# i8run/BigDL-1

Hardware: AMD Instinct MI355X
Metric: images/sec (whole node) ResNet-50 ImageNet-shape sync-SGD at 1/2/4/8 MI355X (higher is better)
Workload: dtype bf16; 1 GPU; model=ResNet-50, global_batch=256, per_gpu_batch=256, image_size=224, classes=1000, parallelism=dp1, optimizer=SGD(lr=0.1,m=0.9,nesterov,wd=1e-4)+L2Reg(1e-4), comm_dtype=fp32, device=cuda, syncbn=False, driver=LocalOptimizer

## Files before the change

bigdl-1_amd/bigdl/nn/fusion.py:

```python
from __future__ import annotations

from ..utils import config
from .containers import Sequential, ConcatTable
from .layers.activation import Threshold
from .layers.conv import SpatialConvolution
from .layers.normalization import BatchNormalization, SpatialBatchNormalization
from .layers.table_ops import CAddTable


def _is_relu(m):
    return isinstance(m, Threshold) and m.threshold == 0.0 and m.value == 0.0


from .layers.conv import SpatialShareConvolution

_PLAIN_CONVS = (SpatialConvolution, SpatialShareConvolution)


def _is_nchw_bn(m):
    return isinstance(m, BatchNormalization) and getattr(m, "dataFormat", "NCHW") == "NCHW"


def _relu_fusable_conv(m):
    return type(m) in _PLAIN_CONVS and m.format == "NCHW" and m._bias_folded_into is None


def _fuse_conv_relu(a, b):
    a._fused_relu = True
    b._passthrough = "mask"


def _fuse_graphs(model, convrelu):
    from .graph import Graph
    for g in model.flattened_modules():
        if not isinstance(g, Graph) or not hasattr(g, "forward_order"):
            continue
        g._plans = None
        for n in g.forward_order:
            if (convrelu and _relu_fusable_conv(n.element) and len(n.next_nodes) == 1
                    and _is_relu(n.next_nodes[0].element) and len(n.next_nodes[0].prev_nodes) == 1
                    and not n.element._fused_relu):
                _fuse_conv_relu(n.element, n.next_nodes[0].element)


def _stackable(a, b):
    from .layers.recurrent import Recurrent, LSTM
    return (type(a) is Recurrent and type(b) is Recurrent and type(a.topology) is LSTM and type(b.topology) is LSTM
            and a.topology.p == 0 and b.topology.p == 0 and not a.maskZero and not b.maskZero
            and b.batchNormParams is None and a._stack_next is None and a._stack_prev is None
            and b._stack_next is None and b._stack_prev is None)


def _link_stack(a, b):
    a._stack_next = b
    b._stack_prev = a


def _fuse_lstm_stacks(model):
    from .graph import Graph
    for s in model.flattened_modules():
        if isinstance(s, Sequential):
            mods = s.modules
            for i in range(len(mods) - 1):
                if _stackable(mods[i], mods[i + 1]):
                    _link_stack(mods[i], mods[i + 1])
        elif isinstance(s, Graph) and hasattr(s, "forward_order"):
            for n in s.forward_order:
                if len(n.next_nodes) != 1:
                    continue
                m = n.next_nodes[0]
                if len(m.prev_nodes) == 1 and _stackable(n.element, m.element):
                    _link_stack(n.element, m.element)


def fuse(model, convbn=None, bnrelu=None, convsum=None, bnbwd=None, convrelu=None):
    if not config.get_property("bigdl.fusion"):
        return model
    if getattr(model, "_fused", False):
        return model
    model._fused = True
    convrelu = config.get_property("bigdl.fusion.convrelu") if convrelu is None else convrelu
    convbn = config.get_property("bigdl.fusion.convbn") if convbn is None else convbn
    bnrelu = config.get_property("bigdl.fusion.bnrelu") if bnrelu is None else bnrelu
    convsum = config.get_property("bigdl.fusion.convsum") if convsum is None else convsum
    bnbwd = config.get_property("bigdl.fusion.bnbwd") if bnbwd is None else bnbwd
    tails, heads = [], []
    for s in model.flattened_modules():
        if not isinstance(s, Sequential):
            continue
        mods = s.modules
        for i in range(len(mods) - 1):
            a, b = mods[i], mods[i + 1]
            if convbn and isinstance(a, SpatialConvolution) and type(a) in (SpatialConvolution,) + tuple(
                    SpatialConvolution.__subclasses__()) and a.format == "NCHW" and a.withBias and _is_nchw_bn(b) \
                    and b._bias_producer is None:
                a._bias_folded_into = b
                b._bias_producer = a
            if convrelu and _relu_fusable_conv(a) and _is_relu(b) and not b._passthrough:
                _fuse_conv_relu(a, b)
            if bnrelu and _is_nchw_bn(a) and _is_relu(b):
                a._fused_relu = True
                b._passthrough = True
                c = mods[i + 2] if i + 2 < len(mods) else None
                if bnbwd and isinstance(c, SpatialConvolution) and c.format == "NCHW" and c.nGroup == 1:
                    c._bn_bwd_target = a
                    if type(c) in _PLAIN_CONVS:
                        a._pro_consumer = c
        if not convsum:
            continue
        for i in range(len(mods) - 1):
            ct, add = mods[i], mods[i + 1]
            if not (isinstance(ct, ConcatTable) and len(ct.modules) == 2 and isinstance(add, CAddTable)):
                continue
            br = ct.modules[0]
            if not (isinstance(br, Sequential) and br.modules and _is_nchw_bn(br.modules[-1])):
                continue
            bn = br.modules[-1]
            if bn._fused_relu:
                continue
            relu = mods[i + 2] if i + 2 < len(mods) and _is_relu(mods[i + 2]) else None
            ct._residual = (br, bn, ct.modules[1], relu is not None)
            sc = ct.modules[1]
            if (config.get_property("bigdl.fusion.shortcutbn") and isinstance(sc, Sequential) and len(sc.modules) >= 2
                    and _is_nchw_bn(sc.modules[-1]) and not sc.modules[-1]._fused_relu):
                sc.modules[-1]._defer_ok = True
            add._passthrough = True
            if relu is not None:
                relu._passthrough = True
                tails.append(bn)
            first = br.modules[0]
            if isinstance(first, SpatialConvolution) and len(br.modules) > 1:
                heads.append(first)
                sc = ct.modules[1]
                sc0 = sc.modules[0] if isinstance(sc, Sequential) and sc.modules else None
                if (isinstance(sc0, SpatialConvolution) and type(sc0) in _PLAIN_CONVS and sc0.format == "NCHW"
                        and sc0.kernelW == 1 and sc0.kernelH == 1 and sc0.padW == 0 and sc0.padH == 0
                        and sc0.nGroup == 1 and (sc0.strideW > 1 or sc0.strideH > 1)):
                    sc0._lazy_strided_ok = True
    if bnbwd and tails:
        for h in heads:
            h._tail_candidates = tails
    _fuse_graphs(model, convrelu)
    if config.get_property("bigdl.fusion.lstmstack"):
        _fuse_lstm_stacks(model)
    return model


def mark_input_no_grad(model):
    from .graph import Graph
    todo, seen = [model], set()
    while todo:
        m = todo.pop()
        if id(m) in seen:
            continue
        seen.add(id(m))
        if isinstance(m, Sequential):
            if m.modules:
                todo.append(m.modules[0])
        elif isinstance(m, Graph) and hasattr(m, "forward_order"):
            for n in m.forward_order:
                if not n.prev_nodes:
                    todo.append(n.element)
        elif isinstance(m, SpatialConvolution):
            m._input_grad_needed = False
    return model


def unfuse(model):
    model._fused = False
    for m in model.flattened_modules():
        if hasattr(m, "_plans"):
            m._plans = None
        if hasattr(m, "_plan"):
            m._plan = None
        if isinstance(m, SpatialConvolution):
            m._bias_folded_into = None
            m._fused_relu = False
            m._bn_bwd_target = None
            m._tail_candidates = None
            m._input_grad_needed = True
            m._lazy_strided_ok = False
        if isinstance(m, BatchNormalization):
            m._bias_producer = None
            m._fused_relu = False
            m._defer_ok = False
            m._pro_consumer = None
            m._pending_stats = None
            m._pending_grad = None
        if isinstance(m, Threshold):
            m._passthrough = False
        if isinstance(m, ConcatTable):
            m._residual = None
        if isinstance(m, CAddTable):
            m._passthrough = False
    return model
```

bigdl-1_amd/bigdl/nn/layers/conv.py:

```python
from __future__ import annotations

import math

import torch
import torch.nn.functional as F

from ... import ops
from ...ops.reference import BNGrad, BNOut, StridedGrad, as_dense
from ...utils.engine import Engine
from ...utils import config
from ..abstractnn import AbstractModule, TensorModule, AutogradModule
from ..initialization_method import RandomUniform, Zeros, VariableFormats
from ...utils import acc_float


def same_padding(in_h, in_w, stride_h, stride_w, k_h, k_w, dil_h=1, dil_w=1):
    out_h = math.ceil(in_h / stride_h)
    out_w = math.ceil(in_w / stride_w)
    ekh = (k_h - 1) * dil_h + 1
    ekw = (k_w - 1) * dil_w + 1
    ph = max((out_h - 1) * stride_h + ekh - in_h, 0)
    pw = max((out_w - 1) * stride_w + ekw - in_w, 0)
    return ph // 2, ph - ph // 2, pw // 2, pw - pw // 2, out_h, out_w


def to_device_layout(x: torch.Tensor) -> torch.Tensor:
    if x.is_cuda and x.dim() == 4:
        dt = Engine.compute_dtype()
        if (dt == torch.bfloat16 and x.dtype in (torch.float32, torch.bfloat16) and x.is_contiguous()
                and not x.is_contiguous(memory_format=torch.channels_last)):
            from ...ops import native as N
            if N.has("nchw_to_nhwc_bf16"):
                y = N.native_ops.nchw_to_nhwc_bf16(x)
                if y is not NotImplemented:
                    return y
        if x.dtype != dt and x.is_floating_point():
            x = x.to(dt)
        if not x.is_contiguous(memory_format=torch.channels_last):
            x = x.contiguous(memory_format=torch.channels_last)
    return x


class SpatialConvolution(TensorModule):
    def __init__(self, n_input_plane, n_output_plane, kernel_w, kernel_h, stride_w=1, stride_h=1, pad_w=0,
                 pad_h=0, n_group=1, propagate_back=True, wRegularizer=None, bRegularizer=None, init_weight=None,
                 init_bias=None, init_grad_weight=None, init_grad_bias=None, with_bias=True, data_format="NCHW",
                 bigdl_type="float"):
        super().__init__()
        if n_output_plane % n_group != 0 or n_input_plane % n_group != 0:
            raise ValueError(f"channels must be multiples of group: in {n_input_plane} out {n_output_plane} g {n_group}")
        if not ((pad_w >= 0 and pad_h >= 0) or (pad_w == -1 and pad_h == -1)):
            raise ValueError(f"Illegal padding configuration (padW: {pad_w}, padH: {pad_h})")
        self.nInputPlane, self.nOutputPlane = n_input_plane, n_output_plane
        self.kernelW, self.kernelH = kernel_w, kernel_h
        self.strideW, self.strideH = stride_w, stride_h
        self.padW, self.padH = pad_w, pad_h
        self.nGroup = n_group
        self.propagateBack = propagate_back
        self.withBias = with_bias
        self.format = data_format
        self.dilationW = self.dilationH = 1
        self.wRegularizer, self.bRegularizer = wRegularizer, bRegularizer
        g = n_group
        shape5 = (g, n_output_plane // g, n_input_plane // g, kernel_h, kernel_w)
        phys = (g, n_output_plane // g, kernel_h, kernel_w, n_input_plane // g)
        w = init_weight if init_weight is not None else torch.zeros(shape5)
        self.register_parameter("weight", torch.as_tensor(w, dtype=torch.float32).reshape(shape5), "gradWeight",
                                layout=(phys, (0, 1, 4, 2, 3)))
        if with_bias:
            b = init_bias if init_bias is not None else torch.zeros(n_output_plane)
            self.register_parameter("bias", torch.as_tensor(b, dtype=torch.float32).reshape(n_output_plane), "gradBias")
        else:
            self.bias = None
            self.gradBias = None
        self._has_init_w = init_weight is not None
        self._has_init_b = init_bias is not None
        stdv = 1.0 / math.sqrt(kernel_w * kernel_h * n_input_plane)
        self._init_weight_method = RandomUniform(-stdv, stdv)
        self._init_bias_method = RandomUniform(-stdv, stdv) if with_bias else Zeros()
        self.reset()

    def reset(self):
        if not self._has_init_w:
            self._init_weight_method.init(self.weight, VariableFormats.GP_OUT_IN_KW_KH)
        if self.withBias and not self._has_init_b:
            self._init_bias_method.init(self.bias, VariableFormats.ONE_D)
        self.zeroGradParameters()
        return self

    def _pads(self, x):
        H, W = x.shape[-2], x.shape[-1]
        if self.padW == -1 and self.padH == -1:
            pt, pb, pl, pr, _, _ = same_padding(H, W, self.strideH, self.strideW, self.kernelH, self.kernelW,
                                                self.dilationH, self.dilationW)
            return pt, pb, pl, pr
        return self.padH, self.padH, self.padW, self.padW

    def _w4(self, w):
        g, og, ig, kh, kw = w.shape
        krsc = w.permute(0, 1, 3, 4, 2)
        if krsc.is_contiguous():
            return krsc.reshape(g * og, kh, kw, ig).permute(0, 3, 1, 2)
        return w.reshape(g * og, ig, kh, kw)

    def _prep(self, input):
        x = input
        batched = x.dim() == 4
        if not batched:
            x = x.unsqueeze(0)
        if self.format == "NHWC":
            x = x.permute(0, 3, 1, 2)
        if (self.nInputPlane <= 3 and self.nGroup == 1 and x.is_cuda and x.dim() == 4 and x.is_contiguous()
                and not x.is_contiguous(memory_format=torch.channels_last) and (self.dilationH, self.dilationW) == (1, 1)
                and Engine.compute_dtype() == torch.bfloat16 and x.dtype in (torch.float32, torch.bfloat16)):
            from ...ops import native as N
            y = N.native_ops.nchw_to_nhwc_padded(x, self._pad_slot_()) if N.has("conv2d_forward") else NotImplemented
            x = to_device_layout(x) if y is NotImplemented else y
        else:
            x = to_device_layout(x)
        pt, pb, pl, pr = self._pads(x)
        if pt != pb or pl != pr:
            x = F.pad(x, (pl, pr, pt, pb))
            pad = (0, 0)
        else:
            pad = (pt, pl)
        return x, pad, batched, (pt, pb, pl, pr)

    _bias_folded_into = None
    _fused_relu = False
    _out_target = None

    _grad_residual = None
    _bn_bwd_target = None
    _tail_candidates = None
    _lazy_strided_ok = False

    def _pad_slot_(self):
        s = self.__dict__.get("_pad_slot")
        if s is None:
            s = self.__dict__["_pad_slot"] = [None]
        return s

    def _tail_target(self, x):
        for bn in self._tail_candidates or ():
            y = bn.output
            if (isinstance(y, torch.Tensor) and y.data_ptr() == x.data_ptr() and y.shape == x.shape and bn.train
                    and getattr(bn, "_last_relu", False)
                    and bn._last_input is not None and bn._last_input.shape == x.shape):
                return bn
        return None

    def _stats_consumer(self, x):
        bn = self._bias_folded_into
        if bn is None or not bn.train or not x.is_cuda:
            return None
        if getattr(bn, "_sync", False) and not config.get_property("bigdl.bn.shiftedStats"):
            return None
        if self.format != "NCHW" or not config.get_property("bigdl.fusion.convstats"):
            return None
        return bn

    def _pro_input(self, input):
        if not (isinstance(input, BNOut) and input.relu and self.format == "NCHW" and self.nGroup == 1
                and input.dim() == 4 and input.is_cuda and self.padW >= 0 and self.padH >= 0):
            return None
        return input.x, input.coef

    def updateOutput(self, input):
        pro = self._pro_input(input)
        if pro is not None:
            y = self._pro_forward(pro[0], pro[1])
            if y is not NotImplemented:
                return y
        if isinstance(input, BNOut):
            input = input.dense()
        x, pad, batched, _ = self._prep(input)
        w4 = self._w4(self.cw("weight"))
        b = self.bias if (self.withBias and self._bias_folded_into is None) else None
        bn = self._stats_consumer(x) if batched else None
        y = NotImplemented
        if bn is not None and ops.native_has("conv2d_forward"):
            shift = bn._stat_shift() if config.get_property("bigdl.bn.shiftedStats") else None
            sums = bn._atomic_sums("fwd", self.nOutputPlane, x.device) if shift is not None else None
            r = ops.native_ops.conv2d_forward_stats(x, w4, b, (self.strideH, self.strideW), pad,
                                                (self.dilationH, self.dilationW), self.nGroup,
                                                pad_slot=self._pad_slot_(), shift=shift, sums=sums)
            if r is not NotImplemented:
                y, part, G = r
                bn._pending_stats = (y.data_ptr(), tuple(y.shape), part, G, shift)
        if y is NotImplemented:
            tgt, self._out_target = self._out_target, None
            if tgt is not None and (not batched or self.format != "NCHW"):
                tgt = None
            y = ops.conv2d_forward(x, w4, b, (self.strideH, self.strideW), pad, (self.dilationH, self.dilationW),
                                   self.nGroup, relu=self._fused_relu, out=tgt,
                                   pad_slot=self._pad_slot_() if (self.train or self.nInputPlane <= 3) else None)
        if self.format == "NHWC":
            y = y.permute(0, 2, 3, 1)
        return y if batched else y.squeeze(0)

    def _pro_forward(self, xb, coef):
        if not ops.native_has("conv2d_forward"):
            return NotImplemented
        pt, pb, pl, pr = self._pads(xb)
        if pt != pb or pl != pr:
            return NotImplemented
        pad = (pt, pl)
        w4 = self._w4(self.cw("weight"))
        b = self.bias if (self.withBias and self._bias_folded_into is None) else None
        st, dl = (self.strideH, self.strideW), (self.dilationH, self.dilationW)
        bn = self._stats_consumer(xb)
        if bn is not None:
            shift = bn._stat_shift() if config.get_property("bigdl.bn.shiftedStats") else None
            sums = bn._atomic_sums("fwd", self.nOutputPlane, xb.device) if shift is not None else None
            r = ops.native_ops.conv2d_forward_stats(xb, w4, b, st, pad, dl, self.nGroup, shift=shift, sums=sums,
                                                    pro=coef) if sums is not None else NotImplemented
            if r is not NotImplemented:
                y, part, G = r
                bn._pending_stats = (y.data_ptr(), tuple(y.shape), part, G, shift)
                return y
            if sums is not None:
                bn._drop_sums((None, None, sums[0], sums[1]), 3)
        return ops.native_ops.conv2d_forward(xb, w4, b, st, pad, dl, self.nGroup, relu=self._fused_relu, pro=coef)

    def _backward(self, input, gradOutput, need_input, acc):
        pro = self._pro_input(input)
        if pro is not None:
            r = self._pro_backward(pro[0], pro[1], gradOutput, need_input, acc)
            if r is not NotImplemented:
                return r
        if isinstance(input, BNOut):
            input = input.dense()
        x, pad, batched, pads = self._prep(input)
        if isinstance(gradOutput, BNGrad):
            own = self.withBias and self._bias_folded_into is None and acc
            if not (batched and self.format == "NCHW" and not own and ops.native_has("conv2d_backward")
                    and ops.native_ops.bngrad_consumable(gradOutput, x, self._w4(self.cw("weight")),
                                                          (self.strideH, self.strideW), pad, self.nGroup)):
                gradOutput = gradOutput.dense()
        if isinstance(gradOutput, BNGrad):
            gy = gradOutput
        else:
            gy = gradOutput if batched else gradOutput.unsqueeze(0)
            if self.format == "NHWC":
                gy = gy.permute(0, 3, 1, 2)
            gy = to_device_layout(gy)
        w4 = self._w4(self.cw("weight"))
        gw = self._w4(self.gradWeight) if acc else None
        same_scale = self.scale_b == self.scale_w
        own_bias = self.withBias and self._bias_folded_into is None
        gb = self.gradBias if (acc and own_bias and same_scale) else None
        res = self._grad_residual if need_input else None
        self._grad_residual = None
        pt, pb, pl, pr = pads
        fuse_res = res is not None and pt == pb and pl == pr and self.format == "NCHW" and batched
        if isinstance(res, StridedGrad) and not (fuse_res and gy.is_cuda):
            res = res.dense()
        bn = self._bn_bwd_target
        bn_fuse = None
        if (bn is not None and need_input and res is None and pt == pb and pl == pr and self.format == "NCHW"
                and batched and gy.is_cuda and bn.train and bn._fused_relu
                and bn._coef is not None and bn._last_input is not None
                and config.get_property("bigdl.fusion.bnbwd")):
            C_ = bn._coef.numel() // 2
            bn_fuse = {"x": bn._last_input, "scale": bn._coef[:C_], "shift": bn._coef[C_:], "mean": bn.saveMean,
                       "sums": bn._atomic_sums("bwd", C_, bn.saveMean.device)}
        elif (fuse_res and self._tail_candidates and gy.is_cuda and config.get_property("bigdl.fusion.bnbwd")):
            bn = self._tail_target(x)
            if bn is not None:
                bn_fuse = {"x": bn._last_input, "mean": bn.saveMean, "mask": bn.output,
                           "bits": getattr(bn, "_relu_bits", None),
                           "sums": bn._atomic_sums("bwd", bn.saveMean.numel(), bn.saveMean.device)}
        lazy = (need_input and self._lazy_strided_ok and res is None and bn_fuse is None and batched
                and self.format == "NCHW" and pt == pb and pl == pr and gy.is_cuda)
        if fuse_res and not isinstance(res, StridedGrad):
            res = to_device_layout(res)
        gi = ops.conv2d_backward(gy, x, w4, (self.strideH, self.strideW), pad, (self.dilationH, self.dilationW),
                                 self.nGroup, need_input, gw, gb, self.scale_w if acc else 0.0,
                                 residual=res if fuse_res else None, bn_fuse=bn_fuse,
                                 pad_slot=self._pad_slot_(), lazy_strided=lazy)
        if isinstance(gi, StridedGrad):
            return gi
        if bn_fuse is not None and "partial" in bn_fuse and gi is not None:
            bn._pending_grad = (gi.data_ptr(), bn_fuse["partial"], bn_fuse["G"])
        if acc and own_bias and not same_scale and self.scale_b != 0:
            self.gradBias.add_(acc_float(gy).sum((0, 2, 3)), alpha=self.scale_b)
        if need_input and gi is not None:
            pt, pb, pl, pr = pads
            if pt != pb or pl != pr:
                gi = gi[:, :, pt:gi.shape[2] - pb, pl:gi.shape[3] - pr]
            if self.format == "NHWC":
                gi = gi.permute(0, 2, 3, 1)
            if not batched:
                gi = gi.squeeze(0)
            if res is not None and not fuse_res:
                gi = gi + as_dense(res)
        return gi

    def _pro_backward(self, xb, coef, gradOutput, need_input, acc):
        if not isinstance(gradOutput, torch.Tensor) or gradOutput.dim() != 4 or not gradOutput.is_cuda:
            return NotImplemented
        pt, pb, pl, pr = self._pads(xb)
        if pt != pb or pl != pr:
            return NotImplemented
        pad = (pt, pl)
        gy = to_device_layout(gradOutput)
        w4 = self._w4(self.cw("weight"))
        gw = self._w4(self.gradWeight) if acc else None
        own_bias = self.withBias and self._bias_folded_into is None
        same_scale = self.scale_b == self.scale_w
        gb = self.gradBias if (acc and own_bias and same_scale) else None
        if self._grad_residual is not None and need_input:
            return NotImplemented
        bn = self._bn_bwd_target
# ... 422 lines not shown
```

bigdl-1_amd/bigdl/nn/layers/normalization.py:

```python
from __future__ import annotations

import math

import torch
import torch.nn.functional as F

from ... import ops
from ..abstractnn import TensorModule, AutogradModule
from ..initialization_method import RandomUniform, Zeros, Ones, VariableFormats
from .conv import to_device_layout
from ...utils import acc_float, config


_SYNCBN_COMM = {}


def _syncbn_comm():
    import torch.distributed as dist
    if not config.get_property("bigdl.syncbn.ownComm") or dist.get_world_size() == 1:
        return None
    key = id(dist.distributed_c10d._get_default_group())
    g = _SYNCBN_COMM.get(key)
    if g is None:
        g = _SYNCBN_COMM[key] = dist.new_group(list(range(dist.get_world_size())))
# ... 6 lines not shown
        super().__init__()
        if n_output <= 0:
            raise ValueError("output feature map number must be greater than zero")
        self.nOutput = n_output
        self.eps = eps
        self.momentum = momentum
        self.affine = affine
        self.register_buffer("runningMean", torch.zeros(n_output))
        self.register_buffer("runningVar", torch.ones(n_output))
        self.saveMean = torch.zeros(n_output)
        self.saveStd = torch.zeros(n_output)
        if affine:
            self.register_parameter("weight", torch.zeros(n_output) if init_weight is None else
                                    torch.as_tensor(init_weight, dtype=torch.float32).reshape(n_output))
            self.register_parameter("bias", torch.zeros(n_output) if init_bias is None else
                                    torch.as_tensor(init_bias, dtype=torch.float32).reshape(n_output))
        else:
            self.weight = self.bias = self.gradWeight = self.gradBias = None
        self._has_init_w = init_weight is not None
        self._has_init_b = init_bias is not None
        self._init_weight_method = RandomUniform(0, 1)
        self._init_bias_method = Zeros()
        self._fused_relu = False
        self._defer_ok = False
        self._pro_consumer = None
        self._sync_group = None
        self._sync = False
        self._sync_force = False
        self.reset()

    def reset(self):
        if self.affine:
            if not self._has_init_w:
                self._init_weight_method.init(self.weight, VariableFormats.ONE_D)
            if not self._has_init_b:
                self._init_bias_method.init(self.bias, VariableFormats.ONE_D)
        self.runningMean.zero_()
        self.runningVar.fill_(1.0)
        self.zeroGradParameters()
        return self

    def setParallism(self, parallism: int):
        self._sync = parallism is not None and parallism > 1
        return self

    def set_sync_group(self, group=None, enabled: bool = True, force: bool = False):
        self._sync = enabled
        self._sync_group = group
        self._sync_force = force
        return self

    def _sync_active(self):
        if not self._sync:
            return False
        import torch.distributed as dist
        pg = dist.distributed_c10d.GroupMember.WORLD if dist.is_available() else None
        token = (id(pg), id(self._sync_group), self._sync_force, config.version())
        c = self.__dict__.get("_sa_cache")
        if c is not None and c[0] == token:
            return c[1]
        on = _dist_ready(self._sync_force)
        if on and config.get_property("bigdl.bn.syncOneRankLocal") and self._sync_world() == 1:
            on = False
        self.__dict__["_sa_cache"] = (token, on)
        return on

    def _sync_world(self):
        import torch.distributed as dist
        grp = self._sync_group
        return dist.get_world_size(grp) if grp is not None else dist.get_world_size()

    def _to_nchw_like(self, x):
        return x

    def _shape_in(self, input):
        return input

    _bias_producer = None
    _pending_stats = None
    _coef = None
    _last_input = None
    _pending_grad = None
    _relu_bits = None

    def _atomic_sums(self, kind, C, device):
        if device.type != "cuda" or config.get_property("bigdl.deterministic"):
            return None
        rep = int(config.get_property("bigdl.bn.statReplicas"))
        if self._sync_active() and not (rep > 0 and config.get_property("bigdl.bn.shiftedStats")):
            return None
        if rep > 0 and (self._sync_active() or not config.get_property("bigdl.bn.atomicStats")):
            rep = min(rep, 512)
            if config.get_property("bigdl.bn.foldFinalize"):
                rep = min(rep, max(4, 16384 // max(C, 1)))
            attr = "_rep_" + kind
            sets = self.__dict__.get(attr)
            if sets is None or sets[0].numel() != 2 * rep * C or sets[0].device != device:
                sets = self.__dict__[attr] = [torch.zeros(2 * rep * C, dtype=torch.float32, device=device)
                                              for _ in range(2)]
                self.__dict__["_repi_" + kind] = 0
            return sets[self.__dict__["_repi_" + kind]], rep
        if not config.get_property("bigdl.bn.atomicStats"):
            return None
        attr = "_sums_" + kind
        buf = self.__dict__.get(attr)
        if buf is None or buf.numel() != 2 * C + 1 or buf.device != device:
            buf = self.__dict__[attr] = torch.zeros(2 * C + 1, dtype=torch.float32, device=device)
        return buf

    def _drop_sums(self, pending, g_index):
        if pending is not None and (pending[g_index] == 0 or self._is_rep(pending[g_index - 1])):
            pending[g_index - 1].zero_()

    def _is_rep(self, part):
        return part is not None and any(part is b for a in ("_rep_fwd", "_rep_bwd") for b in (self.__dict__.get(a) or ()))

    def _rep_next(self, kind, part):
        sets = self.__dict__.get("_rep_" + kind)
        if not sets or not config.get_property("bigdl.bn.foldFinalize"):
            return None
        i = self.__dict__["_repi_" + kind]
        return sets[1 - i] if part is sets[i] else None

    def _rep_flip(self, kind, part):
        sets = self.__dict__.get("_rep_" + kind)
        if sets and part is sets[self.__dict__["_repi_" + kind]]:
            self.__dict__["_repi_" + kind] ^= 1

    def _advance_shift(self, mean):
        kb = self.__dict__.get("_kbuf")
        if kb is None or mean is None:
            return
        i = self.__dict__["_kidx"]
        nxt = kb[1 - i]
        if mean is not nxt:
            nxt.copy_(mean.detach().reshape(nxt.shape))
        self.__dict__["_kidx"] = 1 - i

    def _shift_next(self, shift):
        kb = self.__dict__.get("_kbuf")
        if kb is None or shift is not kb[self.__dict__["_kidx"]]:
            return None
        return kb[1 - self.__dict__["_kidx"]]

    def _stat_shift(self, device=None):
        if not (self._sync_active() or (config.get_property("bigdl.bn.foldFinalize") and self.train)):
            return self.runningMean
        kb = self.__dict__.get("_kbuf")
        rm = self.runningMean
        if kb is None or kb[0].shape != rm.shape or kb[0].device != rm.device:
            kb = self.__dict__["_kbuf"] = [rm.detach().to(torch.float32).clone(), torch.empty_like(rm, dtype=torch.float32)]
            self.__dict__["_kidx"] = 0
        return kb[self.__dict__["_kidx"]]

    def _in_bias(self):
        p = self._bias_producer
        if p is None or not getattr(p, "withBias", False):
            return None
        return p.cw("bias", torch.float32)

    def _pro_deferrable(self, x, relu, residual, coef):
        c = self._pro_consumer
        if (c is None or not relu or residual is not None or not x.is_cuda or x.dtype != torch.float32
                or c._bn_bwd_target is not self or not c.train):
            return False
        if not config.get_property("bigdl.fp32.bnPrologue") or not config.get_property("bigdl.fusion.bnbwd"):
            return False
        from ...ops import fp32x3 as F3
        return F3.pro_ok(x, coef)

    def forward_residual(self, x, residual, relu):
        self._residual_mode = True
        self._res_relu = relu
        try:
            self.output = self._forward_impl(x, residual, relu)
        finally:
            self._residual_mode = False
        return self.output

    def updateOutput(self, input):
        return self._forward_impl(input, None, self._fused_relu)

    def _forward_impl(self, input, residual, relu):
        from ...ops.reference import BNOut
        x = input
        if x.dim() == 1:
            x = x.unsqueeze(0)
        x = to_device_layout(x) if x.dim() == 4 else x
        defer = (self.__dict__.pop("_defer_next", False) and residual is None and not relu and x.is_cuda
                 and x.dtype == torch.bfloat16)
        deferred_res = isinstance(residual, BNOut)
        if deferred_res and not self.train:
            residual, deferred_res = residual.dense(), False
        if residual is not None and not deferred_res and residual.dim() == 4:
            residual = to_device_layout(residual)
        pdt = torch.float64 if x.dtype == torch.float64 else torch.float32
        g = self.cw("weight", pdt) if self.affine else None
        b = self.cw("bias", pdt) if self.affine else None
        ib = self._in_bias()
        self._last_relu = relu
        if self.train:
            if self._sync_active():
                y, mean, invstd = self._sync_forward(x, g, b, relu, residual, ib, defer=defer)
            else:
                r = NotImplemented
                C_ = x.shape[1]
                coef = self._coef
                if coef is None or coef.numel() != 2 * C_ or coef.device != x.device:
                    coef = self._coef = torch.empty(2 * C_, dtype=torch.float32, device=x.device)
                ps, self._pending_stats = self._pending_stats, None
                bits = self._tail_bits(x, relu, residual)
                self._relu_bits = None
                if ps is not None and ps[0] == x.data_ptr() and ps[1] == tuple(x.shape):
                    special = defer or deferred_res
                    pdefer = not special and self._pro_deferrable(x, relu, residual, coef)
                    r = ops.native_ops.batchnorm_forward_train_partials(
                        x, ps[2], ps[3], g, b, self.runningMean, self.runningVar, self.momentum, self.eps,
                        relu=relu, residual=residual, in_bias=ib, coef_out=coef, shift=ps[4],
                        bits_out=None if pdefer else bits,
                        rezero=self._is_rep(ps[2]), zero_next=None if special else self._rep_next("fwd", ps[2]),
                        mean_out=self._shift_next(ps[4]), apply=not (defer or pdefer))
                    if r is not NotImplemented and not special:
                        self._rep_flip("fwd", ps[2])
                if r is NotImplemented:
                    if deferred_res:
                        residual = residual.dense()
                    self._drop_sums(ps, 3)
                    r = ops.batchnorm_forward_train(x, g, b, self.runningMean, self.runningVar,
                                                    self.momentum, self.eps, relu=relu, residual=residual,
                                                    in_bias=ib, coef_out=coef, bits_out=bits)
                self._relu_bits = bits
                y, mean, invstd = r
                if y is None:
                    y = BNOut(x, coef, relu=bool(relu))
                self._advance_shift(mean)
                self._last_input = x
            self.saveMean, self.saveStd = mean, invstd
        else:
            y = ops.batchnorm_forward_infer(x, g, b, self.runningMean, self.runningVar, self.eps, relu=False,
                                            in_bias=ib)
            if residual is not None:
                y = y + residual
            if relu:
                y = torch.relu(y)
        return y.reshape(input.shape) if input.dim() == 1 else y

    def _tail_bits(self, x, relu, residual):
        if not (residual is not None and relu and x.is_cuda and x.dim() == 4 and x.shape[1] % 8 == 0
                and getattr(self, "_residual_mode", False)):
            return None
        n = x.numel() // 8
        bits = self._relu_bits
        if bits is None or bits.numel() != n or bits.device != x.device:
            bits = torch.empty(n, dtype=torch.uint8, device=x.device)
        return bits

    def _lazy_grad_ok(self, input, x):
        prod = self._bias_producer
        if prod is None or input is not x or x.dim() != 4 or not x.is_cuda or x.dtype != torch.bfloat16:
            return False
        mode = int(config.get_property("bigdl.fusion.bnprologue"))
        if mode <= 0 or (mode == 1 and x.shape[1] >= getattr(prod, "nInputPlane", 0)):
            return False
        k = (getattr(prod, "kernelH", 0), getattr(prod, "kernelW", 0), getattr(prod, "strideH", 0),
             getattr(prod, "strideW", 0), getattr(prod, "padH", -1), getattr(prod, "padW", -1),
             getattr(prod, "nGroup", 0))
        return (k == (1, 1, 1, 1, 0, 0, 1) and prod.format == "NCHW" and x.shape[1] % 32 == 0
                and x.is_contiguous(memory_format=torch.channels_last))

    def _sync_allreduce(self, t):
        import torch.distributed as dist
        ws = self.__dict__.get("_sync_ws")
        if ws is None or ws[0] is not self._sync_group:
            grp = self._sync_group if self._sync_group is not None else _syncbn_comm()
            ws = self.__dict__["_sync_ws"] = (self._sync_group, dist.get_world_size(grp), grp)
        if ws[1] > 1:
            dist.all_reduce(t, group=ws[2])

    def _sync_ops(self, x):
        from ...ops import native_ops as NO, reference as R
        if (x.is_cuda and x.dtype == torch.bfloat16 and x.dim() == 4 and x.shape[1] % 8 == 0
                and ops.native_has("batchnorm_forward_train")):
            return NO
        return R

    def _sync_forward(self, x, g, b, relu=False, residual=None, in_bias=None, defer=False):
        from ...ops import reference as R
        impl = self._sync_ops(x)
        C_ = x.shape[1]
        coef = self._coef
        if coef is None or coef.numel() != 2 * C_ or coef.device != x.device:
            coef = self._coef = torch.empty(2 * C_, dtype=torch.float32, device=x.device)
        ps, self._pending_stats = self._pending_stats, None
        bits = self._tail_bits(x, relu, residual) if impl is not R else None
        self._relu_bits = None
        r = NotImplemented
        for m in ((impl, R) if impl is not R else (R,)):
            if m is not R and ps is not None and ps[0] == x.data_ptr() and ps[1] == tuple(x.shape) \
                    and ps[4] is not None:
                shift = ps[4]
                sums = m.bn_local_sums(x, shift, ps[2], ps[3], rezero=self._is_rep(ps[2]))
                ps = None
            else:
                shift = self._stat_shift()
                sums = m.bn_local_sums(x, shift)
            if sums is NotImplemented:
                continue
            self._sync_allreduce(sums)
            kb = self.__dict__.get("_kbuf")
            nxt = kb[1 - self.__dict__["_kidx"]] if (kb is not None and shift is kb[self.__dict__["_kidx"]]) else None
            kw = dict(mean_out=nxt) if (m is not R and nxt is not None) else {}
            r = m.bn_forward_from_sums(x, sums, 0, shift, g, b, self.runningMean, self.runningVar, self.momentum,
                                       self.eps, relu=relu, residual=residual, in_bias=in_bias, coef_out=coef,
                                       bits_out=bits if (m is not R and not defer) else None, apply=not defer, **kw)
            if r is NotImplemented and m is not R:
                m = R
                r = R.bn_forward_from_sums(x, sums, 0, shift, g, b, self.runningMean, self.runningVar,
                                           self.momentum, self.eps, relu=relu, residual=residual, in_bias=in_bias,
                                           coef_out=coef, apply=not defer)
            if r is not NotImplemented:
                if r[0] is None:
                    r = (R.BNOut(x, coef, relu=bool(relu)),) + tuple(r[1:])
                self._relu_bits = bits if m is not R else None
                self._sync_path = "native" if m is not R else "reference"
                self._last_input = x
                if nxt is not None:
                    if r[1] is not nxt:
                        nxt.copy_(r[1])
                    self.__dict__["_kidx"] ^= 1
                break
        self._drop_sums(ps, 3)
        return r

    def _bwd(self, input, gradOutput, need_input, acc, want_gres=False):
        x = input if input.dim() > 1 else input.unsqueeze(0)
        gy = gradOutput if gradOutput.dim() > 1 else gradOutput.unsqueeze(0)
        if x.dim() == 4:
            x = to_device_layout(x)
            gy = to_device_layout(gy)
        relu = getattr(self, "_last_relu", self._fused_relu)
        y = self.output if relu else None
        from ...ops.reference import BNOut
        if isinstance(y, BNOut):
            y = None if (self._pending_grad is not None and self._pending_grad[0] == gy.data_ptr()) else y.dense()
        if y is not None and y.dim() == 1:
            y = y.unsqueeze(0)
        g = self.cw("weight", torch.float64 if x.dtype == torch.float64 else torch.float32) if self.affine else None
        prod = self._bias_producer
        cb = prod.gradBias if (acc and prod is not None and getattr(prod, "withBias", False)) else None
        cbs = prod.scale_b if prod is not None else 0.0
        gres = None
        if self._sync_active() and self.train:
            pg = self._pending_grad
            pre_masked = pg is not None and pg[0] == gy.data_ptr()
            gi, cb_done = self._sync_backward(x, gy, g, y, need_input, acc, relu, cb, cbs)
            if cb is not None and gi is not None and not cb_done:
                cb.add_(acc_float(gi).sum([d for d in range(gi.dim()) if d != 1]), alpha=cbs)
            if want_gres:
                gres = gy * (y > 0).to(gy.dtype) if (relu and not pre_masked) else gy
        else:
            same = self.scale_w == self.scale_b
            pg, self._pending_grad = self._pending_grad, None
            if pg is not None and pg[0] == gy.data_ptr() and relu and same:
                gi = ops.native_ops.batchnorm_backward_partials(
                    gy, x, g, self.saveMean, self.saveStd, pg[1], pg[2], need_input=need_input,
                    gg_acc=self.gradWeight if (acc and self.affine) else None,
                    gb_acc=self.gradBias if (acc and self.affine) else None,
                    scale=self.scale_w if acc else 0.0, cbias_acc=cb, cbias_scale=cbs,
                    lazy=self._lazy_grad_ok(input, x), rezero=self._is_rep(pg[1]),
                    zero_next=self._rep_next("bwd", pg[1]))
                if gi is not NotImplemented:
                    self._rep_flip("bwd", pg[1])
                    if gi is not None and input.dim() == 1:
                        gi = gi.reshape(input.shape)
                    return (gi, gy) if want_gres else gi
            self._drop_sums(pg, 2)
            gi, gres = ops.batchnorm_backward(gy, x, g, self.saveMean, self.saveStd, y=y, relu=relu,
                                              need_input=need_input,
                                              gg_acc=self.gradWeight if (acc and self.affine) else None,
                                              gb_acc=self.gradBias if (acc and self.affine and same) else None,
                                              scale=self.scale_w if acc else 0.0, cbias_acc=cb, cbias_scale=cbs,
                                              want_gres=want_gres)
            if acc and self.affine and not same and self.scale_b != 0:
                gf = acc_float(gy) * ((y > 0).float() if relu else 1.0)
                dims = [d for d in range(gf.dim()) if d != 1]
                self.gradBias.add_(gf.sum(dims), alpha=self.scale_b)
        if gi is not None and input.dim() == 1:
            gi = gi.reshape(input.shape)
        if want_gres:
            return gi, gres
        return gi

    def backward_residual(self, input, gradOutput):
        gi, gres = self._bwd(input, gradOutput, True, True, want_gres=True)
        self.gradInput = gi
        for h in self._grad_ready_hooks:
            h(self)
        return gi, gres

    def _sync_backward(self, x, gy, g, y, need_input, acc, relu=None, cb=None, cbs=0.0):
        from ...ops import reference as R
        relu = self._fused_relu if relu is None else relu
        impl = self._sync_ops(x)
        pg, self._pending_grad = self._pending_grad, None
        C = x.shape[1]
        rows = x.numel() // C
        for m in ((impl, R) if impl is not R else (R,)):
            rl = relu
            both = NotImplemented
            if m is not R and pg is not None and pg[0] == gy.data_ptr() and relu:
                both = m.bn_bwd_partials_sums(pg[1], pg[2], C, x.device, rows=rows, rezero=self._is_rep(pg[1]))
                if both is not NotImplemented:
                    rl = False
                    pg = None
            if both is NotImplemented:
                both = m.bn_bwd_local_sums(gy, x, self.saveMean, y=y, relu=rl)
            if both is NotImplemented:
                continue
            loc, glob = both[:2 * C], both[2 * C:]
            self._sync_allreduce(glob)
            kw = dict(need_input=need_input, gg_acc=self.gradWeight if (acc and self.affine) else None,
                      gb_acc=self.gradBias if (acc and self.affine) else None, scale=self.scale_w if acc else 0.0,
                      cbias_acc=cb, cbias_scale=cbs)
            gi = m.bn_backward_from_sums(gy, x, g, self.saveMean, self.saveStd, loc, glob, 0, y=y, relu=rl, **kw)
            if gi is NotImplemented and m is not R:
                m = R
                gi = R.bn_backward_from_sums(gy, x, g, self.saveMean, self.saveStd, loc, glob, 0, y=y, relu=rl, **kw)
            if gi is NotImplemented:
                raise RuntimeError("SyncBN backward: no implementation accepted the all-reduced sums")
            if acc and self.affine and self.scale_b != self.scale_w:
                self.gradBias.add_(loc[:C], alpha=self.scale_b - self.scale_w)
            self._sync_bwd_path = "native" if m is not R else "reference"
            self._drop_sums(pg, 2)
            return gi, cb is not None
        raise RuntimeError("SyncBN backward: no implementation accepted the input")

    def updateGradInput(self, input, gradOutput):
        gi = self._bwd(input, gradOutput, True, True)
        self._gi_done = True
        return gi

    def accGradParameters(self, input, gradOutput):
        if not getattr(self, "_gi_done", False):
            self._bwd(input, gradOutput, False, True)
        self._gi_done = False

    def set_running_mean(self, v):
        self.runningMean.copy_(torch.as_tensor(v))
        return self

    def set_running_std(self, v):
        self.runningVar.copy_(torch.as_tensor(v))
        return self

    def __repr__(self):
        return f"{type(self).__name__}[{self.get_name()}]({self.nOutput}, {self.eps}, {self.momentum}, {self.affine})"


class SpatialBatchNormalization(BatchNormalization):
    def __init__(self, n_output, eps=1e-5, momentum=0.1, affine=True, init_weight=None, init_bias=None,
                 init_grad_weight=None, init_grad_bias=None, data_format="NCHW", bigdl_type="float"):
        super().__init__(n_output, eps, momentum, affine, init_weight, init_bias, init_grad_weight, init_grad_bias)
        self.dataFormat = data_format

    def updateOutput(self, input):
        if self.dataFormat == "NHWC":
            y = super().updateOutput(input.permute(0, 3, 1, 2))
# ... 188 lines not shown
```

bigdl-1_amd/bigdl/nn/layers/pooling.py:

```python
from __future__ import annotations

import math

import torch
import torch.nn.functional as F

from ... import ops
from ..abstractnn import TensorModule, AutogradModule
from .conv import to_device_layout, same_padding
from ...utils import acc_float


def _pool_pad(x, kh, kw, dh, dw, ph, pw):
    if ph == -1 and pw == -1:
        pt, pb, pl, pr, _, _ = same_padding(x.shape[-2], x.shape[-1], dh, dw, kh, kw)
        return pt, pb, pl, pr
    return ph, ph, pw, pw


class SpatialMaxPooling(TensorModule):
    def __init__(self, kw, kh, dw=None, dh=None, pad_w=0, pad_h=0, to_ceil=False, format="NCHW",
                 bigdl_type="float"):
        super().__init__()
        self.kW, self.kH = kw, kh
        self.dW = dw if dw is not None else kw
        self.dH = dh if dh is not None else kh
        self.padW, self.padH = pad_w, pad_h
        self.ceilMode = to_ceil
        self.format = format

    def ceil(self):
        self.ceilMode = True
        return self

    def floor(self):
        self.ceilMode = False
        return self

    def _prep(self, input):
        x = input
        if self.format == "NHWC":
            x = x.permute(0, 3, 1, 2) if x.dim() == 4 else x.permute(2, 0, 1)
        batched = x.dim() == 4
        if not batched:
            x = x.unsqueeze(0)
        x = to_device_layout(x)
        pt, pb, pl, pr = _pool_pad(x, self.kH, self.kW, self.dH, self.dW, self.padH, self.padW)
        if pt != pb or pl != pr:
            x = F.pad(x, (pl, pr, pt, pb), value=float("-inf"))
            pad = (0, 0)
        else:
            pad = (pt, pl)
        return x, pad, batched, (pt, pb, pl, pr)

    def _post(self, y, batched):
        if not batched:
            y = y.squeeze(0)
        if self.format == "NHWC":
            y = y.permute(0, 2, 3, 1) if y.dim() == 4 else y.permute(1, 2, 0)
        return y

    def _int8_forward(self, input):
        from ...ops import native_ops as NO
        if not (input.is_cuda and input.dim() == 4 and self.format == "NCHW" and not self.train):
            return None
        pt, pb, pl, pr = _pool_pad(input, self.kH, self.kW, self.dH, self.dW, self.padH, self.padW)
        if pt != pb or pl != pr:
            return None
        H, W = input.shape[2], input.shape[3]
        P = NO._pool_out(H, self.kH, self.dH, pt, self.ceilMode)
        Q = NO._pool_out(W, self.kW, self.dW, pl, self.ceilMode)
        y = NO.maxpool_i8(input, self.kH, self.kW, self.dH, self.dW, pt, pl, P, Q)
        return None if y is NotImplemented else y

    def updateOutput(self, input):
        if input.dtype == torch.int8 and getattr(input, "_qscale", None) is not None:
            y = self._int8_forward(input)
            if y is not None:
                return y
            from ..quantized.layers import dequant
            input = dequant(input)
        x, pad, batched, _ = self._prep(input)
        y, idx = ops.maxpool2d_forward(x, (self.kH, self.kW), (self.dH, self.dW), pad, self.ceilMode,
                                       need_indices=bool(self.train))
        self._indices = idx
        return self._post(y, batched)

    def updateGradInput(self, input, gradOutput):
        x, pad, batched, pads = self._prep(input)
        gy = gradOutput
        if self.format == "NHWC":
            gy = gy.permute(0, 3, 1, 2) if gy.dim() == 4 else gy.permute(2, 0, 1)
        if not batched:
            gy = gy.unsqueeze(0)
        gy = to_device_layout(gy)
        if self._indices is None:
            _, self._indices = ops.maxpool2d_forward(x, (self.kH, self.kW), (self.dH, self.dW), pad, self.ceilMode)
        gi = ops.maxpool2d_backward(gy, x, self._indices, (self.kH, self.kW), (self.dH, self.dW), pad, self.ceilMode)
        pt, pb, pl, pr = pads
        if pt != pb or pl != pr:
            gi = gi[:, :, pt:gi.shape[2] - pb, pl:gi.shape[3] - pr]
        return self._post(gi, batched)

    def __repr__(self):
        return f"SpatialMaxPooling[{self.get_name()}]({self.kW}, {self.kH}, {self.dW}, {self.dH}, {self.padW}, {self.padH})"


class SpatialAveragePooling(TensorModule):
    def __init__(self, kw, kh, dw=1, dh=1, pad_w=0, pad_h=0, global_pooling=False, ceil_mode=False,
                 count_include_pad=True, divide=True, format="NCHW", bigdl_type="float"):
        super().__init__()
        self.kW, self.kH, self.dW, self.dH = kw, kh, dw, dh
        self.padW, self.padH = pad_w, pad_h
        self.globalPooling = global_pooling
        self.ceilMode = ceil_mode
        self.countIncludePad = count_include_pad
        self.divide = divide
        self.format = format

    def ceil(self):
        self.ceilMode = True
        return self

    def floor(self):
        self.ceilMode = False
        return self

    def _geom(self, x):
        if self.globalPooling:
            return (x.shape[-2], x.shape[-1]), (1, 1), (0, 0)
        return (self.kH, self.kW), (self.dH, self.dW), None

    def _prep(self, input):
        x = input
        if self.format == "NHWC":
            x = x.permute(0, 3, 1, 2) if x.dim() == 4 else x.permute(2, 0, 1)
        batched = x.dim() == 4
        if not batched:
            x = x.unsqueeze(0)
        x = to_device_layout(x)
        k, s, p = self._geom(x)
        pads = (0, 0, 0, 0)
        if p is None:
            pt, pb, pl, pr = _pool_pad(x, k[0], k[1], s[0], s[1], self.padH, self.padW)
            pads = (pt, pb, pl, pr)
            if pt != pb or pl != pr:
                x = F.pad(x, (pl, pr, pt, pb))
                p = (0, 0)
            else:
                p = (pt, pl)
        divisor = None if self.divide else 1
        return x, k, s, p, batched, pads, divisor

    def _post(self, y, batched):
        if not batched:
            y = y.squeeze(0)
        if self.format == "NHWC":
            y = y.permute(0, 2, 3, 1) if y.dim() == 4 else y.permute(1, 2, 0)
        return y

    def updateOutput(self, input):
        x, k, s, p, batched, _, divisor = self._prep(input)
        y = ops.avgpool2d_forward(x, k, s, p, self.ceilMode, self.countIncludePad, divisor)
        return self._post(y, batched)

    def updateGradInput(self, input, gradOutput):
        x, k, s, p, batched, pads, divisor = self._prep(input)
        gy = gradOutput
        if self.format == "NHWC":
            gy = gy.permute(0, 3, 1, 2) if gy.dim() == 4 else gy.permute(2, 0, 1)
        if not batched:
# ... 228 lines not shown
```

bigdl-1_amd/bigdl/ops/csrc/batchnorm.hip:

```cpp
#include "common.h"

struct BnGeom {
  int C, CG, RPI, tpr;
};

__device__ __forceinline__ BnGeom bn_geom(int C) {
  BnGeom g;
  g.C = C;
  g.CG = C >> 3;
  int cg_eff = g.CG < 256 ? g.CG : 256;
  g.RPI = 256 / cg_eff;
  g.tpr = cg_eff;
  return g;
}

__global__ void __launch_bounds__(256) k_bn_stats(const bf16_t* __restrict__ x, long long M, int C,
                                                  long long rows_per_block, float* __restrict__ partial, int G,
                                                  const float* __restrict__ kshift = nullptr) {
  extern __shared__ __attribute__((aligned(16))) float smem[];
  BnGeom g = bn_geom(C);
  const int t = threadIdx.x;
  const int cg_local = t % g.tpr;
  const int r_off = t / g.tpr;
  const long long r0 = (long long)blockIdx.x * rows_per_block;
// ... 300 lines not shown
      b += partial[(size_t)(G + g) * C + c];
    }
  }
  red[0][ty][tx] = a;
  red[1][ty][tx] = b;
  __syncthreads();
  if (ty == 0 && c < C) {
    out[(size_t)blockIdx.y * C + c] = red[0][0][tx] + red[0][1][tx] + red[0][2][tx] + red[0][3][tx];
    out[(size_t)(S + blockIdx.y) * C + c] = red[1][0][tx] + red[1][1][tx] + red[1][2][tx] + red[1][3][tx];
  }
}

static constexpr int kFoldRows = 128;

BIGDL_EXPORT long long bigdl_bn_fold_scratch(int G, int C) {
  if (G <= 512) return 0;
  const int S = (G + kFoldRows - 1) / kFoldRows;
  return 4LL * S * C;
}

static bool maybe_fold(const float* partial, int& G, int C, float* scratch, hipStream_t s) {
  if (G <= 512 || !scratch) return false;
  const int S = (G + kFoldRows - 1) / kFoldRows;
  hipLaunchKernelGGL(k_bn_fold_partials, dim3((C + 63) / 64, S), dim3(256), 0, s, partial, G, C, kFoldRows, S,
                     (double*)scratch);
  G = S;
  return true;
}

BIGDL_EXPORT int bigdl_bn_fwd_train_partials2(const void* x, const void* res, const float* rcoef, void* y, long long M,
                                              int C, const float* gamma, const float* beta, const float* in_bias,
                                              float* run_mean, float* run_var, float momentum, float eps,
                                              float* save_mean, float* save_invstd, const float* partial, int G,
                                              const float* kshift, float* coef, int relu, float* scratch, void* bits,
                                              int rezero, hipStream_t s);

BIGDL_EXPORT int bigdl_bn_fwd_train_partials(const void* x, const void* res, void* y, long long M, int C,
                                             const float* gamma, const float* beta, const float* in_bias,
                                             float* run_mean, float* run_var, float momentum, float eps,
                                             float* save_mean, float* save_invstd, const float* partial, int G,
                                             const float* kshift, float* coef, int relu, float* scratch, void* bits,
                                             int rezero, hipStream_t s) {
  if (!y) return (int)hipErrorInvalidValue;
  return bigdl_bn_fwd_train_partials2(x, res, nullptr, y, M, C, gamma, beta, in_bias, run_mean, run_var, momentum, eps,
                                      save_mean, save_invstd, partial, G, kshift, coef, relu, scratch, bits, rezero, s);
}

BIGDL_EXPORT int bigdl_bn_fwd_train_partials2(const void* x, const void* res, const float* rcoef, void* y, long long M,
                                              int C, const float* gamma, const float* beta, const float* in_bias,
                                              float* run_mean, float* run_var, float momentum, float eps,
                                              float* save_mean, float* save_invstd, const float* partial, int G,
                                              const float* kshift, float* coef, int relu, float* scratch, void* bits,
                                              int rezero, hipStream_t s) {
  if (rcoef && !res) return (int)hipErrorInvalidValue;
  if (C % 8 || M <= 0 || G <= 0 || (bits && !relu) || (rezero && G > 512)) return (int)hipErrorInvalidValue;
  if (!rezero && maybe_fold(partial, G, C, scratch, s))
    hipLaunchKernelGGL(k_bn_finalize<double>, dim3((C + 31) / 32), dim3(32 * kFinRG), 0, s, (const bf16_t*)nullptr, kshift,
                       (const double*)scratch, G, M, C, gamma, beta, in_bias, run_mean, run_var, momentum, eps, save_mean,
                       save_invstd, coef, coef + C);
  else
    hipLaunchKernelGGL(k_bn_finalize<float>, dim3((C + 31) / 32), dim3(32 * kFinRG), 0, s, (const bf16_t*)nullptr, kshift,
                       partial, G, M, C, gamma, beta, in_bias, run_mean, run_var, momentum, eps, save_mean, save_invstd,
                       coef, coef + C, nullptr, rezero ? const_cast<float*>(partial) : nullptr);
  if (y) launch_apply(x, res, y, M, C, coef, relu, bits, s, rcoef);
  BIGDL_CHECK_LAUNCH();
}

BIGDL_EXPORT int bigdl_bn_fwd_infer(const void* x, void* y, long long M, int C, const float* gamma, const float* beta,
                                    const float* run_mean, const float* run_var, const float* in_bias, float eps,
                                    float* coef, int relu, hipStream_t s) {
  if (C % 8 || M <= 0) return (int)hipErrorInvalidValue;
  hipLaunchKernelGGL(k_bn_infer_coef, dim3((C + 255) / 256), dim3(256), 0, s, C, gamma, beta, run_mean, run_var,
                     in_bias, eps, coef, coef + C);
  int grid = apply_grid(M, C);
  if (relu)
    hipLaunchKernelGGL((k_bn_apply<false, true>), dim3(grid), dim3(256), 0, s, (const bf16_t*)x, nullptr, (bf16_t*)y,
                       M, C, coef, coef + C);
  else
    hipLaunchKernelGGL((k_bn_apply<false, false>), dim3(grid), dim3(256), 0, s, (const bf16_t*)x, nullptr,
                       (bf16_t*)y, M, C, coef, coef + C);
  BIGDL_CHECK_LAUNCH();
}

template <bool RELU>
__global__ void __launch_bounds__(256) k_bn_bwd_reduce(const bf16_t* __restrict__ gy, const bf16_t* __restrict__ x,
                                                       const bf16_t* __restrict__ y, long long M, int C,
                                                       long long rows_per_block, const float* __restrict__ mean,
                                                       float* __restrict__ partial, int G) {
  extern __shared__ __attribute__((aligned(16))) float smem[];
  BnGeom g = bn_geom(C);
  const int t = threadIdx.x;
  const int cg_local = t % g.tpr;
  const int r_off = t / g.tpr;
  const long long r0 = (long long)blockIdx.x * rows_per_block;
  long long r1 = r0 + rows_per_block;
  if (r1 > M) r1 = M;
  float* s_a = smem;
  float* s_b = smem + g.RPI * C;
  for (int cg = cg_local; cg < g.CG; cg += g.tpr) {
    if (r_off >= g.RPI) break;
    float mu[8], a[8], b[8];
#pragma unroll
    for (int k = 0; k < 8; ++k) { mu[k] = mean[cg * 8 + k]; a[k] = 0.f; b[k] = 0.f; }
    for (long long r = r0 + r_off; r < r1; r += g.RPI) {
      size_t off = (size_t)r * C + (size_t)cg * 8;
      float gv[8], xv[8];
      load8_nt(gy + off, gv);
      load8_nt(x + off, xv);
      if (RELU) {
        float yv[8];
        load8_nt(y + off, yv);
#pragma unroll
        for (int k = 0; k < 8; ++k) gv[k] = yv[k] > 0.f ? gv[k] : 0.f;
      }
#pragma unroll
      for (int k = 0; k < 8; ++k) {
        a[k] += gv[k];
        b[k] = fmaf(gv[k], xv[k] - mu[k], b[k]);
      }
    }
#pragma unroll
    for (int k = 0; k < 8; ++k) {
      s_a[r_off * C + cg * 8 + k] = a[k];
      s_b[r_off * C + cg * 8 + k] = b[k];
    }
  }
  __syncthreads();
  for (int c = t; c < C; c += 256) {
    float a = 0.f, b = 0.f;
    for (int i = 0; i < g.RPI; ++i) {
      a += s_a[i * C + c];
      b += s_b[i * C + c];
    }
    partial[(size_t)blockIdx.x * C + c] = a;
    partial[(size_t)(G + blockIdx.x) * C + c] = b;
  }
}

template <typename T>
__global__ void __launch_bounds__(32 * kFinRG) k_bn_bwd_finalize(const T* __restrict__ partial, int G, long long M,
                                                          int C, const float* __restrict__ gamma,
                                                          const float* __restrict__ mean,
                                                          const float* __restrict__ invstd,
                                                          float* __restrict__ ggamma, float* __restrict__ gbeta,
                                                          float gscale, float* __restrict__ cbias, float cbscale,
                                                          float* __restrict__ coef, const float* __restrict__ dM = nullptr,
                                                          float* rezero = nullptr) {
  __shared__ double lds[kFinRG][2][33];
  double ad, bd;
  reduce_partials(partial, G, C, blockIdx.x * 32, lds, ad, bd, rezero);
  const int c = blockIdx.x * 32 + (threadIdx.x & 31);
  if ((threadIdx.x >> 5) != 0 || c >= C) return;
  const float a = (float)ad, b = (float)bd;
  float is = invstd[c];
  float dbeta = a;
  float dgamma = b * is;
  if (ggamma) ggamma[c] += gscale * dgamma;
  if (gbeta) gbeta[c] += gscale * dbeta;
  float gm = gamma ? gamma[c] : 1.f;
  float A = gm * is;
  const float Mf = dM ? *dM : (float)M;
  float B = -gm * is * is * dgamma / Mf;
  float Cc = -gm * is * dbeta / Mf - B * mean[c];
  coef[c] = A;
  coef[C + c] = B;
  coef[2 * C + c] = Cc;
  if (cbias) cbias[c] += cbscale * (A * dbeta + B * Mf * mean[c] + Mf * Cc);
}

template <bool RELU, bool GRES, int kApplyUnroll>
__device__ __forceinline__ void bn_bwd_apply_rows(const bf16_t* __restrict__ gy, const bf16_t* __restrict__ x,
                                                  const bf16_t* __restrict__ y, bf16_t* __restrict__ gx,
                                                  bf16_t* __restrict__ gres, long long M, int C, const float* coef) {
  BnGeom g = bn_geom(C);
  const int t = threadIdx.x;
  const int cg_local = t % g.tpr;
  const int r_off = t / g.tpr;
  if (r_off >= g.RPI) return;
  const long long rstride = (long long)gridDim.x * g.RPI;
  for (int cg = cg_local; cg < g.CG; cg += g.tpr) {
    float A[8], B[8], Cc[8];
#pragma unroll
    for (int k = 0; k < 8; ++k) {
      A[k] = coef[cg * 8 + k];
      B[k] = coef[C + cg * 8 + k];
      Cc[k] = coef[2 * C + cg * 8 + k];
    }
    long long r = (long long)blockIdx.x * g.RPI + r_off;
    for (; r < M; r += kApplyUnroll * rstride) {
      bigdl_u32x4 gq[kApplyUnroll], xq[kApplyUnroll], yq[kApplyUnroll];
#pragma unroll
      for (int u = 0; u < kApplyUnroll; ++u) {
        const long long ru = r + u * rstride;
        const size_t off = (size_t)(ru < M ? ru : r) * C + (size_t)cg * 8;
        gq[u] = __builtin_nontemporal_load(reinterpret_cast<const bigdl_u32x4*>(gy + off));
        xq[u] = __builtin_nontemporal_load(reinterpret_cast<const bigdl_u32x4*>(x + off));
        if (RELU) yq[u] = __builtin_nontemporal_load(reinterpret_cast<const bigdl_u32x4*>(y + off));
      }
#pragma unroll
      for (int u = 0; u < kApplyUnroll; ++u) {
        const long long ru = r + u * rstride;
        if (ru >= M) break;
        const size_t off = (size_t)ru * C + (size_t)cg * 8;
        float gv[8], xv[8];
        unpack8(make_uint4(gq[u][0], gq[u][1], gq[u][2], gq[u][3]), gv);
        unpack8(make_uint4(xq[u][0], xq[u][1], xq[u][2], xq[u][3]), xv);
        if (RELU) {
          float yv[8];
          unpack8(make_uint4(yq[u][0], yq[u][1], yq[u][2], yq[u][3]), yv);
#pragma unroll
          for (int k = 0; k < 8; ++k) gv[k] = yv[k] > 0.f ? gv[k] : 0.f;
        }
        if (GRES) store8(gres + off, gv);
#pragma unroll
        for (int k = 0; k < 8; ++k) xv[k] = fmaf(A[k], gv[k], fmaf(B[k], xv[k], Cc[k]));
        store8(gx + off, xv);
      }
    }
  }
}

template <bool RELU, bool GRES, int kApplyUnroll = 4>
__global__ void __launch_bounds__(256) k_bn_bwd_apply(const bf16_t* __restrict__ gy, const bf16_t* __restrict__ x,
                                                      const bf16_t* __restrict__ y, bf16_t* __restrict__ gx,
                                                      bf16_t* __restrict__ gres, long long M, int C,
                                                      const float* __restrict__ coef) {
  bn_bwd_apply_rows<RELU, GRES, kApplyUnroll>(gy, x, y, gx, gres, M, C, coef);
}

BIGDL_EXPORT int bigdl_bn_bwd(const void* gy, const void* x, const void* y, void* gx, void* gres, long long M, int C,
                              const float* gamma, const float* mean, const float* invstd, float* ggamma,
                              float* gbeta, float gscale, float* cbias, float cbscale, float* ws, float* coef,
                              int relu, hipStream_t s) {
  if (C % 8 || M <= 0) return (int)hipErrorInvalidValue;
  int G = bigdl_bn_num_partials(M, C);
  long long rpb = (M + G - 1) / G;
  size_t sm = stats_smem(C);
  if (relu)
    hipLaunchKernelGGL(k_bn_bwd_reduce<true>, dim3(G), dim3(256), sm, s, (const bf16_t*)gy, (const bf16_t*)x,
                       (const bf16_t*)y, M, C, rpb, mean, ws, G);
  else
    hipLaunchKernelGGL(k_bn_bwd_reduce<false>, dim3(G), dim3(256), sm, s, (const bf16_t*)gy, (const bf16_t*)x,
                       (const bf16_t*)y, M, C, rpb, mean, ws, G);
  hipLaunchKernelGGL(k_bn_bwd_finalize<float>, dim3((C + 31) / 32), dim3(32 * kFinRG), 0, s, (const float*)ws, G, M, C, gamma,
                     mean, invstd, ggamma, gbeta, gscale, cbias, cbscale, coef);
  if (gx) {
    int grid = apply_grid(M, C);
    const bf16_t *g_ = (const bf16_t*)gy, *x_ = (const bf16_t*)x, *y_ = (const bf16_t*)y;
    bf16_t *gx_ = (bf16_t*)gx, *gr_ = (bf16_t*)gres;
    if (relu && gres) hipLaunchKernelGGL((k_bn_bwd_apply<true, true>), dim3(grid), dim3(256), 0, s, g_, x_, y_, gx_, gr_, M, C, coef);
    else if (relu) hipLaunchKernelGGL((apply_unroll1() ? k_bn_bwd_apply<true, false, 1> : k_bn_bwd_apply<true, false, 4>), dim3(grid), dim3(256), 0, s, g_, x_, y_, gx_, gr_, M, C, coef);
    else if (gres) hipLaunchKernelGGL((k_bn_bwd_apply<false, true>), dim3(grid), dim3(256), 0, s, g_, x_, y_, gx_, gr_, M, C, coef);
    else hipLaunchKernelGGL((apply_unroll1() ? k_bn_bwd_apply<false, false, 1> : k_bn_bwd_apply<false, false, 4>), dim3(grid), dim3(256), 0, s, g_, x_, y_, gx_, gr_, M, C, coef);
  }
  BIGDL_CHECK_LAUNCH();
}

BIGDL_EXPORT int bigdl_bn_bwd_partials(const void* gm, const void* x, void* gx, long long M, int C, const float* gamma,
                                       const float* mean, const float* invstd, float* ggamma, float* gbeta,
                                       float gscale, float* cbias, float cbscale, const float* partial, int G,
                                       float* coef, float* scratch, int rezero, hipStream_t s) {
  if (C % 8 || M <= 0 || G <= 0 || (rezero && G > 512)) return (int)hipErrorInvalidValue;
  if (!rezero && maybe_fold(partial, G, C, scratch, s))
    hipLaunchKernelGGL(k_bn_bwd_finalize<double>, dim3((C + 31) / 32), dim3(32 * kFinRG), 0, s, (const double*)scratch, G, M,
                       C, gamma, mean, invstd, ggamma, gbeta, gscale, cbias, cbscale, coef);
  else
    hipLaunchKernelGGL(k_bn_bwd_finalize<float>, dim3((C + 31) / 32), dim3(32 * kFinRG), 0, s, partial, G, M, C, gamma, mean,
                       invstd, ggamma, gbeta, gscale, cbias, cbscale, coef, nullptr,
                       rezero ? const_cast<float*>(partial) : nullptr);
  if (gx) {
    int grid = apply_grid(M, C);
    hipLaunchKernelGGL((apply_unroll1() ? k_bn_bwd_apply<false, false, 1> : k_bn_bwd_apply<false, false, 4>), dim3(grid), dim3(256), 0, s, (const bf16_t*)gm,
                       (const bf16_t*)x, (const bf16_t*)nullptr, (bf16_t*)gx, (bf16_t*)nullptr, M, C, coef);
  }
  BIGDL_CHECK_LAUNCH();
}

BIGDL_EXPORT int bigdl_bn_bwd_apply_coef(const void* gm, const void* x, void* gx, long long M, int C,
                                         const float* coef, hipStream_t s) {
  if (C % 8 || M <= 0 || !gm || !x || !gx || !coef) return (int)hipErrorInvalidValue;
  hipLaunchKernelGGL((apply_unroll1() ? k_bn_bwd_apply<false, false, 1> : k_bn_bwd_apply<false, false, 4>),
                     dim3(apply_grid(M, C)), dim3(256), 0, s, (const bf16_t*)gm, (const bf16_t*)x,
                     (const bf16_t*)nullptr, (bf16_t*)gx, (bf16_t*)nullptr, M, C, coef);
  BIGDL_CHECK_LAUNCH();
}

struct BnFwdFin {
  float* sums;
  const float* kshift;
  const float* gamma;
  const float* beta;
  const float* in_bias;
  float* run_mean;
  float* run_var;
  float* save_mean;
  float* save_invstd;
  float* coef;
  double M;
  float momentum, eps;
  const float* dM;
  unsigned* ticket;
  int keep;
  int early;
  const float* rep;
  int R;
  float* zero_next;
};

__device__ __forceinline__ void fin_fwd_sums(const BnFwdFin& f, int C, int c, double& s, double& q) {
  if (f.rep) {
    s = 0.0;
    q = 0.0;
    for (int r = 0; r < f.R; ++r) {
      s += (double)f.rep[(size_t)r * C + c];
      q += (double)f.rep[((size_t)f.R + r) * C + c];
    }
  } else {
    s = (double)f.sums[c];
    q = (double)f.sums[C + c];
  }
}

__device__ __forceinline__ void block_zero(float* p, long long n) {
  for (long long i = (long long)threadIdx.x * 4; i < n; i += (long long)blockDim.x * 4)
    *reinterpret_cast<float4*>(p + i) = make_float4(0.f, 0.f, 0.f, 0.f);
}

__device__ __forceinline__ void fin_fwd_coef(const BnFwdFin& f, int C, int c, float& mean, float& var, float& invstd,
                                             float& sc, float& sh) {
  const double Mg = f.dM ? (double)*f.dM : f.M;
  double s1, s2;
  fin_fwd_sums(f, C, c, s1, s2);
  const double dm = s1 / Mg;
  var = (float)fmax(s2 / Mg - dm * dm, 0.0);
  mean = (f.kshift ? f.kshift[c] : 0.f) + (float)dm;
  invstd = rsqrtf(var + f.eps);
  sc = (f.gamma ? f.gamma[c] : 1.f) * invstd;
  sh = (f.beta ? f.beta[c] : 0.f) - mean * sc;
}

__device__ __forceinline__ bool last_arriver(unsigned* cnt) {
  __shared__ int last;
  __syncthreads();
  if (threadIdx.x == 0) last = atomicAdd(cnt, 1u) == gridDim.x - 1 ? 1 : 0;
  __syncthreads();
  return last != 0;
}

constexpr int kTicketLeaves = 16;
__device__ __forceinline__ bool last_arriver_tree(unsigned* cnt) {
  __shared__ int last;
  __syncthreads();
  if (threadIdx.x == 0) {
    const unsigned nb = gridDim.x, leaf = blockIdx.x % kTicketLeaves;
    const unsigned in_leaf = (nb - leaf + kTicketLeaves - 1) / kTicketLeaves;
    const unsigned leaves = nb < (unsigned)kTicketLeaves ? nb : (unsigned)kTicketLeaves;
    int l = 0;
    if (atomicAdd(&cnt[1 + leaf], 1u) == in_leaf - 1) {
      atomicExch(&cnt[1 + leaf], 0u);
      if (atomicAdd(&cnt[0], 1u) == leaves - 1) {
        atomicExch(&cnt[0], 0u);
        l = 1;
      }
    }
    last = l;
  }
// ... 283 lines not shown
                                         const float* kshift, float* coef, int relu, void* bits, unsigned* ticket,
                                         hipStream_t s) {
  if (C % 8 || M <= 0 || count < 0 || (bits && !relu) || (rcoef && !res) || (!y && (res || bits)))
    return (int)hipErrorInvalidValue;
  if (ticket && C <= 8192 && y && !rcoef) {
    BnFwdFin f{const_cast<float*>(sums), kshift, gamma, beta, in_bias, run_mean, run_var, save_mean, save_invstd, coef,
               (double)count, momentum, eps, count == 0 ? sums + 2 * C : nullptr, ticket, 1,
               (kshift != run_mean && kshift != save_mean) ? 1 : 0};
    const int grid = apply_grid(M, C);
    const bf16_t* xr = (const bf16_t*)x;
    const bf16_t* rr = (const bf16_t*)res;
    bf16_t* yr = (bf16_t*)y;
    uint8_t* br = (uint8_t*)bits;
    if (relu && bits && res) hipLaunchKernelGGL((k_bn_apply_fin<true, true, true>), dim3(grid), dim3(256), 8 * C, s, xr, rr, yr, M, C, f, br);
    else if (relu && bits) hipLaunchKernelGGL((k_bn_apply_fin<false, true, true>), dim3(grid), dim3(256), 8 * C, s, xr, rr, yr, M, C, f, br);
    else if (res && relu) hipLaunchKernelGGL((k_bn_apply_fin<true, true, false>), dim3(grid), dim3(256), 8 * C, s, xr, rr, yr, M, C, f, br);
    else if (res) hipLaunchKernelGGL((k_bn_apply_fin<true, false, false>), dim3(grid), dim3(256), 8 * C, s, xr, rr, yr, M, C, f, br);
    else if (relu) hipLaunchKernelGGL((k_bn_apply_fin<false, true, false>), dim3(grid), dim3(256), 8 * C, s, xr, rr, yr, M, C, f, br);
    else hipLaunchKernelGGL((k_bn_apply_fin<false, false, false>), dim3(grid), dim3(256), 8 * C, s, xr, rr, yr, M, C, f, br);
    BIGDL_CHECK_LAUNCH();
  }
  hipLaunchKernelGGL(k_bn_finalize<float>, dim3((C + 31) / 32), dim3(32 * kFinRG), 0, s, (const bf16_t*)nullptr, kshift, sums,
                     1, count, C, gamma, beta, in_bias, run_mean, run_var, momentum, eps, save_mean, save_invstd, coef,
                     coef + C, count == 0 ? sums + 2 * C : nullptr);
  if (y) launch_apply(x, res, y, M, C, coef, relu, bits, s, rcoef);
  BIGDL_CHECK_LAUNCH();
}

BIGDL_EXPORT int bigdl_bn_bwd_sums(const void* gy, const void* x, const void* y, long long M, int C, const float* mean,
                                   float* ws, float* scratch, float* out, int relu, float cnt, hipStream_t s) {
  if (C % 8 || M <= 0) return (int)hipErrorInvalidValue;
  int G = bigdl_bn_num_partials(M, C);
  long long rpb = (M + G - 1) / G;
  size_t sm = stats_smem(C);
  if (relu)
    hipLaunchKernelGGL(k_bn_bwd_reduce<true>, dim3(G), dim3(256), sm, s, (const bf16_t*)gy, (const bf16_t*)x,
                       (const bf16_t*)y, M, C, rpb, mean, ws, G);
  else
    hipLaunchKernelGGL(k_bn_bwd_reduce<false>, dim3(G), dim3(256), sm, s, (const bf16_t*)gy, (const bf16_t*)x,
                       (const bf16_t*)y, M, C, rpb, mean, ws, G);
  sum_rows(ws, G, C, scratch, out, s, out + 2 * C, cnt);
  BIGDL_CHECK_LAUNCH();
}

__global__ void __launch_bounds__(256) k_bn_cbias_sync(const float* __restrict__ local_sums,
                                                       const float* __restrict__ coef, const float* __restrict__ mean,
                                                       long long M, int C, float* __restrict__ cbias, float cbscale) {
  const int c = blockIdx.x * 256 + threadIdx.x;
  if (c >= C) return;
  const float A = coef[c], B = coef[C + c], Cc = coef[2 * C + c];
  cbias[c] += cbscale * (A * local_sums[c] + (float)M * (B * mean[c] + Cc));
}

BIGDL_EXPORT int bigdl_bn_bwd_apply_sums(const void* gy, const void* x, const void* y, void* gx, long long M,
                                         long long count, int C, const float* gamma, const float* mean,
                                         const float* invstd, float* ggamma, float* gbeta, float gscale,
                                         const float* local_sums, const float* global_sums, float* coef,
                                         float* coef_scratch, int relu, float* cbias, float cbscale, unsigned* ticket,
                                         hipStream_t s) {
  if (C % 8 || M <= 0 || count < 0) return (int)hipErrorInvalidValue;
  const float* dM = count == 0 ? global_sums + 2 * C : nullptr;
  if (ticket && !relu && C <= 4096) {
    BnBwdFin f{const_cast<float*>(global_sums), gamma, mean, invstd, ggamma, gbeta, gscale, cbias, cbscale, nullptr,
               (float)count, local_sums, (float)M, dM, ticket, 1, 1};
    const int grid = gx ? apply_grid(M, C) : 1;
    hipLaunchKernelGGL(k_bn_bwd_apply_fin, dim3(grid), dim3(256), gx ? 12 * C : 0, s, (const bf16_t*)gy,
                       (const bf16_t*)x, (bf16_t*)gx, M, C, f);
    BIGDL_CHECK_LAUNCH();
  }
  if (ggamma || gbeta)
    hipLaunchKernelGGL(k_bn_bwd_finalize<float>, dim3((C + 31) / 32), dim3(32 * kFinRG), 0, s, local_sums, 1, count, C, gamma,
                       mean, invstd, ggamma, gbeta, gscale, (float*)nullptr, 0.f, coef_scratch, dM);
  hipLaunchKernelGGL(k_bn_bwd_finalize<float>, dim3((C + 31) / 32), dim3(32 * kFinRG), 0, s, global_sums, 1, count, C, gamma,
                     mean, invstd, (float*)nullptr, (float*)nullptr, 0.f, (float*)nullptr, 0.f, coef, dM);
  if (cbias)
    hipLaunchKernelGGL(k_bn_cbias_sync, dim3((C + 255) / 256), dim3(256), 0, s, local_sums, coef, mean, M, C, cbias,
                       cbscale);
  if (gx) {
    int grid = apply_grid(M, C);
    const bf16_t *g_ = (const bf16_t*)gy, *x_ = (const bf16_t*)x, *y_ = (const bf16_t*)y;
    bf16_t* gx_ = (bf16_t*)gx;
    if (relu)
      hipLaunchKernelGGL((apply_unroll1() ? k_bn_bwd_apply<true, false, 1> : k_bn_bwd_apply<true, false, 4>), dim3(grid), dim3(256), 0, s, g_, x_, y_, gx_, (bf16_t*)nullptr, M, C,
                         coef);
    else
      hipLaunchKernelGGL((apply_unroll1() ? k_bn_bwd_apply<false, false, 1> : k_bn_bwd_apply<false, false, 4>), dim3(grid), dim3(256), 0, s, g_, x_, y_, gx_, (bf16_t*)nullptr, M,
                         C, coef);
  }
  BIGDL_CHECK_LAUNCH();
}

__device__ __forceinline__ void ld8f(const float* __restrict__ p, float (&v)[8]) {
  const float4 a = *reinterpret_cast<const float4*>(p), b = *reinterpret_cast<const float4*>(p + 4);
  v[0] = a.x; v[1] = a.y; v[2] = a.z; v[3] = a.w; v[4] = b.x; v[5] = b.y; v[6] = b.z; v[7] = b.w;
}
__device__ __forceinline__ void st8f(float* __restrict__ p, const float (&v)[8]) {
  *reinterpret_cast<float4*>(p) = make_float4(v[0], v[1], v[2], v[3]);
  *reinterpret_cast<float4*>(p + 4) = make_float4(v[4], v[5], v[6], v[7]);
}

template <int MODE, bool RELU>
__global__ void __launch_bounds__(256) k_bn32_reduce(const float* __restrict__ x, const float* __restrict__ gy,
                                                     const float* __restrict__ y, long long M, int C,
                                                     long long rows_per_block, const float* __restrict__ ref,
                                                     float* __restrict__ partial, int G,
                                                     const uint8_t* __restrict__ mbits = nullptr) {
  extern __shared__ __attribute__((aligned(16))) float smem[];
  BnGeom g = bn_geom(C);
  const int t = threadIdx.x;
  const int cg_local = t % g.tpr;
  const int r_off = t / g.tpr;
  const long long r0 = (long long)blockIdx.x * rows_per_block;
  long long r1 = r0 + rows_per_block;
  if (r1 > M) r1 = M;
  float* s_a = smem;
  float* s_b = smem + g.RPI * C;
  for (int cg = cg_local; cg < g.CG; cg += g.tpr) {
    float K[8], a[8], b[8];
#pragma unroll
    for (int k = 0; k < 8; ++k) { K[k] = ref[cg * 8 + k]; a[k] = 0.f; b[k] = 0.f; }
    if (r_off < g.RPI) {
      for (long long r = r0 + r_off; r < r1; r += g.RPI) {
        const size_t off = (size_t)r * C + (size_t)cg * 8;
        float xv[8];
        ld8f(x + off, xv);
        if (MODE == 0) {
#pragma unroll
          for (int k = 0; k < 8; ++k) {
            const float d = xv[k] - K[k];
            a[k] += d;
            b[k] = fmaf(d, d, b[k]);
          }
        } else {
          float gv[8];
          ld8f(gy + off, gv);
          if (RELU) {
            if (mbits) {
              const unsigned mb = mbits[(size_t)r * (C >> 3) + cg];
#pragma unroll
              for (int k = 0; k < 8; ++k) gv[k] = (mb >> k) & 1u ? gv[k] : 0.f;
            } else {
              float yv[8];
              ld8f(y + off, yv);
#pragma unroll
              for (int k = 0; k < 8; ++k) gv[k] = yv[k] > 0.f ? gv[k] : 0.f;
            }
          }
#pragma unroll
          for (int k = 0; k < 8; ++k) {
            a[k] += gv[k];
            b[k] = fmaf(gv[k], xv[k] - K[k], b[k]);
          }
        }
      }
#pragma unroll
      for (int k = 0; k < 8; ++k) {
        s_a[r_off * C + cg * 8 + k] = a[k];
        s_b[r_off * C + cg * 8 + k] = b[k];
      }
    }
  }
  __syncthreads();
  for (int c = t; c < C; c += 256) {
    float a = 0.f, b = 0.f;
    for (int i = 0; i < g.RPI; ++i) {
      a += s_a[i * C + c];
      b += s_b[i * C + c];
    }
    partial[(size_t)blockIdx.x * C + c] = a;
    partial[(size_t)(G + blockIdx.x) * C + c] = b;
// ... 230 lines not shown
```

bigdl-1_amd/bigdl/ops/csrc/pooling.hip:

```cpp
#include "common.h"

struct PoolGeom {
  int N, H, W, C, P, Q, kh, kw, sh, sw, ph, pw;
};

__device__ __forceinline__ void pld8(const bf16_t* p, float* o) { load8(p, o); }
__device__ __forceinline__ void pld8(const float* p, float* o) {
  const float4 a = *reinterpret_cast<const float4*>(p), b = *reinterpret_cast<const float4*>(p + 4);
  o[0] = a.x; o[1] = a.y; o[2] = a.z; o[3] = a.w; o[4] = b.x; o[5] = b.y; o[6] = b.z; o[7] = b.w;
}
__device__ __forceinline__ void pst8(bf16_t* p, const float* o) { store8(p, o); }
__device__ __forceinline__ void pst8(float* p, const float* o) {
  *reinterpret_cast<float4*>(p) = make_float4(o[0], o[1], o[2], o[3]);
  *reinterpret_cast<float4*>(p + 4) = make_float4(o[4], o[5], o[6], o[7]);
}

template <typename IT, typename T = bf16_t>
__global__ void __launch_bounds__(256) k_maxpool_fwd(const T* __restrict__ x, T* __restrict__ y,
                                                     int8_t* __restrict__ idx, PoolGeom g) {
  const int CG = g.C >> 3;
  const IT total = (IT)g.N * g.P * g.Q * CG;
  for (IT t = blockIdx.x * (IT)blockDim.x + threadIdx.x; t < total; t += (IT)gridDim.x * blockDim.x) {
    const int cg = (int)(t % CG);
    IT pix = t / CG;
    const int q = (int)(pix % g.Q);
    pix /= g.Q;
    const int p = (int)(pix % g.P);
    const int n = (int)(pix / g.P);
    float best[8];
    int arg[8];
#pragma unroll
    for (int e = 0; e < 8; ++e) { best[e] = -INFINITY; arg[e] = 0; }
    const int h0 = p * g.sh - g.ph, w0 = q * g.sw - g.pw;
    for (int i = 0; i < g.kh; ++i) {
      const int h = h0 + i;
      if ((unsigned)h >= (unsigned)g.H) continue;
      for (int j = 0; j < g.kw; ++j) {
        const int w = w0 + j;
        if ((unsigned)w >= (unsigned)g.W) continue;
        float v[8];
        pld8(x + (((size_t)n * g.H + h) * g.W + w) * g.C + cg * 8, v);
#pragma unroll
        for (int e = 0; e < 8; ++e) {
          if (v[e] > best[e] || v[e] != v[e]) {
            best[e] = v[e];
            arg[e] = i * g.kw + j;
          }
        }
      }
    }
    const size_t o = (((size_t)n * g.P + p) * g.Q + q) * g.C + cg * 8;
    pst8(y + o, best);
    if (!idx) continue;
    uint32_t lo = 0, hi = 0;
#pragma unroll
    for (int e = 0; e < 4; ++e) lo |= (uint32_t)(arg[e] & 0xFF) << (8 * e);
#pragma unroll
    for (int e = 0; e < 4; ++e) hi |= (uint32_t)(arg[4 + e] & 0xFF) << (8 * e);
    *reinterpret_cast<uint2*>(idx + o) = make_uint2(lo, hi);
  }
}

template <typename IT, typename T = bf16_t>
__global__ void __launch_bounds__(256) k_maxpool_fwd_k3s2(const T* __restrict__ x, T* __restrict__ y,
                                                          int8_t* __restrict__ idx, PoolGeom g) {
  const int CG = g.C >> 3;
  const IT total = (IT)g.N * g.P * g.Q * CG;
  for (IT t = blockIdx.x * (IT)blockDim.x + threadIdx.x; t < total; t += (IT)gridDim.x * blockDim.x) {
    const int cg = (int)(t % CG);
    IT pix = t / CG;
    const int q = (int)(pix % g.Q);
    pix /= g.Q;
    const int p = (int)(pix % g.P);
    const int n = (int)(pix / g.P);
    const int h0 = p * 2 - g.ph, w0 = q * 2 - g.pw;
    const int hc = min(max(h0 + 1, 0), g.H - 1), wc = min(max(w0 + 1, 0), g.W - 1);
    float v[9][8];
    bool ok[9];
#pragma unroll
    for (int i = 0; i < 3; ++i)
#pragma unroll
      for (int j = 0; j < 3; ++j) {
        const int h = h0 + i, w = w0 + j;
        ok[3 * i + j] = (unsigned)h < (unsigned)g.H && (unsigned)w < (unsigned)g.W;
        const int hh = ok[3 * i + j] ? h : hc, ww = ok[3 * i + j] ? w : wc;
        pld8(x + (((size_t)n * g.H + hh) * g.W + ww) * g.C + cg * 8, v[3 * i + j]);
      }
    float best[8];
    int arg[8];
#pragma unroll
    for (int e = 0; e < 8; ++e) { best[e] = -INFINITY; arg[e] = 0; }
#pragma unroll
    for (int k = 0; k < 9; ++k)
#pragma unroll
      for (int e = 0; e < 8; ++e)
        if (ok[k] && (v[k][e] > best[e] || v[k][e] != v[k][e])) {
          best[e] = v[k][e];
          arg[e] = k;
        }
    const size_t o = (((size_t)n * g.P + p) * g.Q + q) * g.C + cg * 8;
    pst8(y + o, best);
    if (!idx) continue;
    uint32_t lo = 0, hi = 0;
#pragma unroll
    for (int e = 0; e < 4; ++e) lo |= (uint32_t)(arg[e] & 0xFF) << (8 * e);
#pragma unroll
    for (int e = 0; e < 4; ++e) hi |= (uint32_t)(arg[4 + e] & 0xFF) << (8 * e);
    *reinterpret_cast<uint2*>(idx + o) = make_uint2(lo, hi);
  }
}

template <typename IT, typename T = bf16_t>
__global__ void __launch_bounds__(256) k_maxpool_bwd(const T* __restrict__ gy, const int8_t* __restrict__ idx,
                                                     T* __restrict__ gx, PoolGeom g) {
  const int CG = g.C >> 3;
  const IT total = (IT)g.N * g.H * g.W * CG;
  for (IT t = blockIdx.x * (IT)blockDim.x + threadIdx.x; t < total; t += (IT)gridDim.x * blockDim.x) {
    const int cg = (int)(t % CG);
    IT pix = t / CG;
    const int w = (int)(pix % g.W);
    pix /= g.W;
    const int h = (int)(pix % g.H);
    const int n = (int)(pix / g.H);
    float acc[8];
#pragma unroll
    for (int e = 0; e < 8; ++e) acc[e] = 0.f;
    const int hp = h + g.ph, wp = w + g.pw;
    int p_lo = hp - g.kh + 1;
    p_lo = p_lo <= 0 ? 0 : (p_lo + g.sh - 1) / g.sh;
    int p_hi = hp / g.sh;
    if (p_hi > g.P - 1) p_hi = g.P - 1;
    int q_lo = wp - g.kw + 1;
    q_lo = q_lo <= 0 ? 0 : (q_lo + g.sw - 1) / g.sw;
    int q_hi = wp / g.sw;
    if (q_hi > g.Q - 1) q_hi = g.Q - 1;
    for (int p = p_lo; p <= p_hi; ++p) {
      const int i = hp - p * g.sh;
      for (int q = q_lo; q <= q_hi; ++q) {
        const int j = wp - q * g.sw;
        const int8_t me = (int8_t)(i * g.kw + j);
        const size_t o = (((size_t)n * g.P + p) * g.Q + q) * g.C + cg * 8;
        const uint2 a = *reinterpret_cast<const uint2*>(idx + o);
        float gv[8];
        pld8(gy + o, gv);
        const uint32_t aw[2] = {a.x, a.y};
#pragma unroll
        for (int e = 0; e < 8; ++e) {
          const int8_t ae = (int8_t)((aw[e >> 2] >> (8 * (e & 3))) & 0xFF);
          if (ae == me) acc[e] += gv[e];
        }
      }
    }
    pst8(gx + (((size_t)n * g.H + h) * g.W + w) * g.C + cg * 8, acc);
  }
}

template <typename IT, typename T = bf16_t>
__global__ void __launch_bounds__(256) k_maxpool_bwd_k3s2(const T* __restrict__ gy, const int8_t* __restrict__ idx,
                                                          T* __restrict__ gx, PoolGeom g) {
  const int CG = g.C >> 3;
  const IT total = (IT)g.N * g.H * g.W * CG;
  for (IT t = blockIdx.x * (IT)blockDim.x + threadIdx.x; t < total; t += (IT)gridDim.x * blockDim.x) {
    const int cg = (int)(t % CG);
    IT pix = t / CG;
    const int w = (int)(pix % g.W);
    pix /= g.W;
    const int h = (int)(pix % g.H);
    const int n = (int)(pix / g.H);
    const int hp = h + g.ph, wp = w + g.pw;
    const int pa = hp / 2 - 1, qa = wp / 2 - 1;
    uint2 a[4];
    float gv[4][8];
    bool ok[4];
    int8_t me[4];
#pragma unroll
    for (int u = 0; u < 2; ++u)
#pragma unroll
      for (int v2 = 0; v2 < 2; ++v2) {
        const int p = pa + u, q = qa + v2, k = 2 * u + v2;
        const int i = hp - 2 * p, j = wp - 2 * q;
        ok[k] = p >= 0 && p < g.P && q >= 0 && q < g.Q && i <= 2 && j <= 2;
        me[k] = (int8_t)(i * 3 + j);
        const int pp = ok[k] ? p : 0, qq = ok[k] ? q : 0;
        const size_t o = (((size_t)n * g.P + pp) * g.Q + qq) * g.C + cg * 8;
// ... 97 lines not shown
#pragma unroll
          for (int e = 0; e < 8; ++e) best[j][e] = (rm[e] > best[j][e] || rm[e] != rm[e]) ? rm[e] : best[j][e];
        }
      }
    }
#pragma unroll
    for (int j = 0; j < MP_ROWS; ++j)
      if (j < np) store8(y + (((size_t)n * g.P + p0 + j) * g.Q + q) * g.C + cg * 8, best[j]);
  }
}

template <typename T = bf16_t>
__global__ void __launch_bounds__(256) k_maxpool_bwd_c1(const T* __restrict__ gy, const int8_t* __restrict__ idx,
                                                        T* __restrict__ gx, PoolGeom g, long long total) {
  for (long long t = blockIdx.x * (long long)blockDim.x + threadIdx.x; t < total; t += (long long)gridDim.x * blockDim.x) {
    const int c = (int)(t % g.C);
    long long pix = t / g.C;
    const int w = (int)(pix % g.W);
    pix /= g.W;
    const int h = (int)(pix % g.H);
    const int n = (int)(pix / g.H);
    const int hp = h + g.ph, wp = w + g.pw;
    int p_lo = hp - g.kh + 1;
    p_lo = p_lo <= 0 ? 0 : (p_lo + g.sh - 1) / g.sh;
    const int p_hi = min(hp / g.sh, g.P - 1);
    int q_lo = wp - g.kw + 1;
    q_lo = q_lo <= 0 ? 0 : (q_lo + g.sw - 1) / g.sw;
    const int q_hi = min(wp / g.sw, g.Q - 1);
    float acc = 0.f;
    for (int p = p_lo; p <= p_hi; ++p)
      for (int q = q_lo; q <= q_hi; ++q) {
        const size_t o = (((size_t)n * g.P + p) * g.Q + q) * g.C + c;
        if (idx[o] == (int8_t)((hp - p * g.sh) * g.kw + (wp - q * g.sw))) acc += pld1(gy + o);
      }
    pst1(gx + t, acc);
  }
}

static PoolGeom make_geom(int N, int H, int W, int C, int P, int Q, int kh, int kw, int sh, int sw, int ph, int pw) {
  PoolGeom g;
  g.N = N; g.H = H; g.W = W; g.C = C; g.P = P; g.Q = Q;
  g.kh = kh; g.kw = kw; g.sh = sh; g.sw = sw; g.ph = ph; g.pw = pw;
  return g;
}

BIGDL_EXPORT int bigdl_maxpool_fwd(const void* x, void* y, void* idx, int N, int H, int W, int C, int P, int Q, int kh,
                                   int kw, int sh, int sw, int ph, int pw, hipStream_t s) {
  if (kh * kw > 127 || N <= 0 || P <= 0 || Q <= 0 || C <= 0) return (int)hipErrorInvalidValue;
  PoolGeom g = make_geom(N, H, W, C, P, Q, kh, kw, sh, sw, ph, pw);
  if (C % 8) {
    const long long te = (long long)N * P * Q * C;
    hipLaunchKernelGGL(k_maxpool_fwd_c1<bf16_t>, dim3(bigdl_grid(te, 256, 16384)), dim3(256), 0, s, (const bf16_t*)x, (bf16_t*)y,
                       (int8_t*)idx, g, te);
    BIGDL_CHECK_LAUNCH();
  }
  const bool k3s2 = kh == 3 && kw == 3 && sh == 2 && sw == 2 && ph <= 1 && pw <= 1;
  if (!idx && k3s2 && (long long)N * P * Q * (C / 8) < 0x7fffffffLL) {
    const long long total = (long long)N * P * Q * (C / 8);
    hipLaunchKernelGGL(k_maxpool_fwd_k3s2<uint32_t>, dim3(bigdl_grid(total, 256, 16384)), dim3(256), 0, s,
                       (const bf16_t*)x, (bf16_t*)y, (int8_t*)nullptr, g);
    BIGDL_CHECK_LAUNCH();
  }
  if (!idx) {
    const long long rows = (long long)N * ((P + MP_ROWS - 1) / MP_ROWS) * Q * (C / 8);
    if (rows < 0x7fffffffLL - 65536LL * 256)
      hipLaunchKernelGGL(k_maxpool_fwd_rows<uint32_t>, dim3(bigdl_grid(rows, 256, 16384)), dim3(256), 0, s,
                         (const bf16_t*)x, (bf16_t*)y, g);
    else
      hipLaunchKernelGGL(k_maxpool_fwd_rows<long long>, dim3(bigdl_grid(rows, 256, 16384)), dim3(256), 0, s,
                         (const bf16_t*)x, (bf16_t*)y, g);
    BIGDL_CHECK_LAUNCH();
  }
  const long long total = (long long)N * P * Q * (C / 8);
  const int grid = bigdl_grid(total, 256, 16384);
  if (total < 0x7fffffffLL) {
    if (k3s2) hipLaunchKernelGGL(k_maxpool_fwd_k3s2<uint32_t>, dim3(grid), dim3(256), 0, s, (const bf16_t*)x, (bf16_t*)y, (int8_t*)idx, g);
    else hipLaunchKernelGGL(k_maxpool_fwd<uint32_t>, dim3(grid), dim3(256), 0, s, (const bf16_t*)x, (bf16_t*)y, (int8_t*)idx, g);
  } else {
    hipLaunchKernelGGL(k_maxpool_fwd<long long>, dim3(grid), dim3(256), 0, s, (const bf16_t*)x, (bf16_t*)y, (int8_t*)idx, g);
  }
  BIGDL_CHECK_LAUNCH();
}

BIGDL_EXPORT int bigdl_maxpool_bwd(const void* gy, const void* idx, void* gx, int N, int H, int W, int C, int P, int Q,
                                   int kh, int kw, int sh, int sw, int ph, int pw, hipStream_t s) {
  if (kh * kw > 127 || N <= 0 || C <= 0) return (int)hipErrorInvalidValue;
  PoolGeom g = make_geom(N, H, W, C, P, Q, kh, kw, sh, sw, ph, pw);
  if (C % 8) {
    const long long te = (long long)N * H * W * C;
    hipLaunchKernelGGL(k_maxpool_bwd_c1<bf16_t>, dim3(bigdl_grid(te, 256, 16384)), dim3(256), 0, s, (const bf16_t*)gy,
                       (const int8_t*)idx, (bf16_t*)gx, g, te);
    BIGDL_CHECK_LAUNCH();
  }
  const long long total = (long long)N * H * W * (C / 8);
  const int grid = bigdl_grid(total, 256, 16384);
  const bool k3s2 = kh == 3 && kw == 3 && sh == 2 && sw == 2 && ph <= 1 && pw <= 1;
  if (total < 0x7fffffffLL && k3s2)
    hipLaunchKernelGGL(k_maxpool_bwd_k3s2<uint32_t>, dim3(grid), dim3(256), 0, s, (const bf16_t*)gy, (const int8_t*)idx,
                       (bf16_t*)gx, g);
  else if (total < 0x7fffffffLL)
    hipLaunchKernelGGL(k_maxpool_bwd<uint32_t>, dim3(grid), dim3(256), 0, s, (const bf16_t*)gy, (const int8_t*)idx,
                       (bf16_t*)gx, g);
  else
    hipLaunchKernelGGL(k_maxpool_bwd<long long>, dim3(grid), dim3(256), 0, s, (const bf16_t*)gy, (const int8_t*)idx,
                       (bf16_t*)gx, g);
  BIGDL_CHECK_LAUNCH();
}

__device__ __forceinline__ float avg_count(const PoolGeom& g, int p, int q, int cip, int divisor) {
  if (divisor > 0) return (float)divisor;
  int hs = p * g.sh - g.ph, ws = q * g.sw - g.pw;
  int he = min(hs + g.kh, g.H + g.ph), we = min(ws + g.kw, g.W + g.pw);
  if (cip) return (float)((he - hs) * (we - ws));
  hs = max(hs, 0); ws = max(ws, 0);
  he = min(he, g.H); we = min(we, g.W);
  return (float)((he - hs) * (we - ws));
}

template <typename IT, typename T = bf16_t>
__global__ void __launch_bounds__(256) k_avgpool_fwd(const T* __restrict__ x, T* __restrict__ y, PoolGeom g,
                                                     int cip, int divisor) {
  const int CG = g.C >> 3;
  const IT total = (IT)g.N * g.P * g.Q * CG;
  for (IT t = blockIdx.x * (IT)blockDim.x + threadIdx.x; t < total; t += (IT)gridDim.x * blockDim.x) {
    const int cg = (int)(t % CG);
    IT pix = t / CG;
    const int q = (int)(pix % g.Q);
    pix /= g.Q;
    const int p = (int)(pix % g.P);
    const int n = (int)(pix / g.P);
    float acc[8] = {0.f, 0.f, 0.f, 0.f, 0.f, 0.f, 0.f, 0.f};
    const int h0 = p * g.sh - g.ph, w0 = q * g.sw - g.pw;
    const int hb = max(h0, 0), he = min(h0 + g.kh, g.H), wb = max(w0, 0), we = min(w0 + g.kw, g.W);
    for (int h = hb; h < he; ++h)
      for (int w = wb; w < we; ++w) {
        float v[8];
        pld8(x + (((size_t)n * g.H + h) * g.W + w) * g.C + cg * 8, v);
#pragma unroll
        for (int e = 0; e < 8; ++e) acc[e] += v[e];
      }
    const float inv = 1.f / fmaxf(avg_count(g, p, q, cip, divisor), 1.f);
#pragma unroll
    for (int e = 0; e < 8; ++e) acc[e] *= inv;
    pst8(y + (((size_t)n * g.P + p) * g.Q + q) * g.C + cg * 8, acc);
  }
}

template <typename IT, typename T = bf16_t>
__global__ void __launch_bounds__(256) k_avgpool_bwd(const T* __restrict__ gy, T* __restrict__ gx, PoolGeom g,
                                                     int cip, int divisor) {
  const int CG = g.C >> 3;
  const IT total = (IT)g.N * g.H * g.W * CG;
  for (IT t = blockIdx.x * (IT)blockDim.x + threadIdx.x; t < total; t += (IT)gridDim.x * blockDim.x) {
    const int cg = (int)(t % CG);
    IT pix = t / CG;
    const int w = (int)(pix % g.W);
    pix /= g.W;
    const int h = (int)(pix % g.H);
    const int n = (int)(pix / g.H);
    const int hp = h + g.ph, wp = w + g.pw;
    const int p_lo = hp < g.kh ? 0 : (hp - g.kh) / g.sh + 1, p_hi = min(hp / g.sh, g.P - 1);
    const int q_lo = wp < g.kw ? 0 : (wp - g.kw) / g.sw + 1, q_hi = min(wp / g.sw, g.Q - 1);
    float acc[8] = {0.f, 0.f, 0.f, 0.f, 0.f, 0.f, 0.f, 0.f};
    for (int p = p_lo; p <= p_hi; ++p)
      for (int q = q_lo; q <= q_hi; ++q) {
        float v[8];
// ... 121 lines not shown
```

bigdl-1_amd/bigdl/ops/native_ops.py:

```python
from __future__ import annotations

import contextlib
import ctypes as C
from typing import Optional

import torch

from . import native as N
from . import reference as R_
from . import fp32x3 as F3
from ..utils import config
from .native import register, ptr, stream_ptr, check
from .lars_table import LarsTable

_bf16 = torch.bfloat16
_f32 = torch.float32


def _al16(t: Optional[torch.Tensor]) -> bool:
    return t is None or t.data_ptr() % 16 == 0


def _dense(t: torch.Tensor) -> bool:
    if t.dim() == 4:
# ... 380 lines not shown
    y = torch.empty_like(x) if apply else None
    check(_lib().bigdl_bn_fwd_train_sums(ptr(x), ptr(residual), ptr(rcoef), ptr(y), _ll(M), _ll(count), C.c_int(C_), ptr(gamma),
                                         ptr(beta), ptr(in_bias), ptr(running_mean), ptr(running_var), _f(momentum),
                                         _f(eps), ptr(mean), ptr(invstd), ptr(sums), ptr(shift), ptr(coef),
                                         C.c_int(1 if relu else 0), ptr(bits_out if relu else None),
                                         ptr(_ticket(x.device)), _s()),
          "bn_fwd_train_sums")
    return y, mean, invstd


def bn_bwd_local_sums(gy, x, save_mean, y=None, relu=False):
    rc = _rows_c(x)
    if rc is None:
        return NotImplemented
    M, C_ = rc
    if not _bn_ok(x, C_) or gy.dtype != _bf16 or gy.shape != x.shape or gy.stride() != x.stride() or not _al16(gy):
        return NotImplemented
    if relu and (y is None or y.dtype != _bf16 or y.stride() != x.stride() or not _al16(y)):
        return NotImplemented
    lib = _lib()
    G = lib.bigdl_bn_num_partials(_ll(M), C.c_int(C_))
    ws = torch.empty(2 * G * C_, dtype=_f32, device=x.device)
    out = torch.empty(4 * C_ + 1, dtype=_f32, device=x.device)
    check(lib.bigdl_bn_bwd_sums(ptr(gy), ptr(x), ptr(y if relu else None), _ll(M), C.c_int(C_), ptr(save_mean), ptr(ws),
                                ptr(_fold_scratch(G, C_, x.device)), ptr(out), C.c_int(1 if relu else 0), _f(M), _s()),
          "bn_bwd_sums")
    return out


def bn_bwd_partials_sums(partial, G, C_, dev, rows=None, rezero=False):
    if partial is None or partial.dtype != _f32 or partial.numel() != 2 * G * C_ or rows is None:
        return NotImplemented
    out = torch.empty(4 * C_ + 1, dtype=_f32, device=dev)
    check(_lib().bigdl_bn_partials_sums2(ptr(partial), C.c_int(G), C.c_int(C_), ptr(_fold_scratch(G, C_, dev)),
                                         ptr(out), ptr(out[2 * C_:]), _f(rows), C.c_int(1 if rezero else 0), _s()), "bn_partials_sums2")
    return out


def bn_backward_from_sums(gy, x, gamma, save_mean, save_invstd, local_sums, global_sums, count, y=None, relu=False,
                          need_input=True, gg_acc=None, gb_acc=None, scale=1.0, cbias_acc=None, cbias_scale=1.0):
    rc = _rows_c(x)
    if rc is None:
        return NotImplemented
    M, C_ = rc
    if not all(_f32vec(t, C_) for t in (gamma, save_mean, save_invstd, gg_acc, gb_acc, cbias_acc)):
        return NotImplemented
    coef = torch.empty(3 * C_, dtype=_f32, device=x.device)
    scratch = torch.empty(3 * C_, dtype=_f32, device=x.device)
    gx = torch.empty_like(x) if need_input else None
    check(_lib().bigdl_bn_bwd_apply_sums(ptr(gy), ptr(x), ptr(y if relu else None), ptr(gx), _ll(M), _ll(count),
                                         C.c_int(C_), ptr(gamma), ptr(save_mean), ptr(save_invstd),
                                         ptr(gg_acc if scale != 0 else None), ptr(gb_acc if scale != 0 else None),
                                         _f(scale), ptr(local_sums), ptr(global_sums), ptr(coef), ptr(scratch),
                                         C.c_int(1 if relu else 0), ptr(cbias_acc if cbias_scale != 0 else None),
                                         _f(cbias_scale), ptr(_ticket(x.device)), _s()), "bn_bwd_apply_sums")
    return gx


@register("batchnorm_forward_infer")
def batchnorm_forward_infer(x, gamma, beta, running_mean, running_var, eps, relu=False, in_bias=None):
    rc = _rows_c(x)
    if rc is None:
        return NotImplemented
    M, C_ = rc
    if _bn32_ok(x, C_) and all(_f32vec(t, C_) for t in (gamma, beta, running_mean, running_var, in_bias)):
        coef = torch.empty(2 * C_, dtype=_f32, device=x.device)
        y = torch.empty_like(x)
        check(_lib().bigdl_bn32_fwd_infer(ptr(x), ptr(y), _ll(M), C.c_int(C_), ptr(gamma), ptr(beta),
                                          ptr(running_mean), ptr(running_var), ptr(in_bias), _f(eps), ptr(coef),
                                          C.c_int(1 if relu else 0), _s()), "bn32_fwd_infer")
        return y
    if not _bn_ok(x, C_) or not all(_f32vec(t, C_) for t in (gamma, beta, running_mean, running_var, in_bias)):
        return NotImplemented
    coef = torch.empty(2 * C_, dtype=_f32, device=x.device)
    y = torch.empty_like(x)
    check(_lib().bigdl_bn_fwd_infer(ptr(x), ptr(y), _ll(M), C.c_int(C_), ptr(gamma), ptr(beta), ptr(running_mean),
                                    ptr(running_var), ptr(in_bias), _f(eps), ptr(coef), C.c_int(1 if relu else 0),
                                    _s()), "bn_fwd_infer")
    return y


@register("batchnorm_backward")
def batchnorm_backward(gy, x, gamma, save_mean, save_invstd, y=None, relu=False, need_input=True, gg_acc=None,
                       gb_acc=None, scale=1.0, cbias_acc=None, cbias_scale=1.0, want_gres=False):
    rc = _rows_c(x)
    if rc is None:
        return NotImplemented
    M, C_ = rc
    mb = F3.producer_bits(y) if relu else None
    if (_bn32_ok(x, C_, gy, y if relu and mb is None else None) and (y is not None or not relu)
            and all(_f32vec(t, C_) for t in (gamma, save_mean, save_invstd, gg_acc, gb_acc, cbias_acc))):
        G = _lib().bigdl_bn_num_partials(_ll(M), C.c_int(C_))
        ws = torch.empty(2 * G * C_, dtype=_f32, device=x.device)
        coef = torch.empty(3 * C_, dtype=_f32, device=x.device)
        gx = torch.empty_like(x) if need_input else None
        gres = torch.empty_like(x) if want_gres else None
        sp = F3.split_buffer(M, C_, x.device) if need_input else None
        check(_lib().bigdl_bn32_bwd(ptr(gy), ptr(x), ptr(y if relu else None), ptr(gx), ptr(gres), _ll(M), C.c_int(C_),
                                    ptr(gamma), ptr(save_mean), ptr(save_invstd), ptr(gg_acc), ptr(gb_acc), _f(scale),
                                    ptr(cbias_acc), _f(cbias_scale), ptr(ws), ptr(coef), C.c_int(1 if relu else 0),
                                    ptr(sp), ptr(mb), _s()), "bn32_bwd")
        F3.note_split(gx, sp)
        return gx, gres
    if not _bn_ok(x, C_) or gy.dtype != _bf16 or gy.shape != x.shape or gy.stride() != x.stride() or not _al16(gy):
        return NotImplemented
    if relu and (y is None or y.dtype != _bf16 or y.stride() != x.stride() or not _al16(y)):
        return NotImplemented
    if not all(_f32vec(t, C_) for t in (gamma, save_mean, save_invstd, gg_acc, gb_acc, cbias_acc)):
        return NotImplemented
    lib = _lib()
    G = lib.bigdl_bn_num_partials(_ll(M), C.c_int(C_))
    ws = torch.empty(2 * G * C_, dtype=_f32, device=x.device)
    coef = torch.empty(3 * C_, dtype=_f32, device=x.device)
    gx = torch.empty_like(x) if need_input else None
    gres = torch.empty_like(x) if want_gres else None
    check(lib.bigdl_bn_bwd(ptr(gy), ptr(x), ptr(y if relu else None), ptr(gx), ptr(gres), _ll(M), C.c_int(C_),
                           ptr(gamma), ptr(save_mean), ptr(save_invstd), ptr(gg_acc), ptr(gb_acc), _f(scale),
                           ptr(cbias_acc), _f(cbias_scale), ptr(ws), ptr(coef), C.c_int(1 if relu else 0), _s()),
          "bn_bwd")
    return gx, gres


def _targets_i32(target_1b, B):
    t = target_1b.reshape(-1)
    if t.numel() != B:
        return None
    return t.to(torch.int32).contiguous()


@register("cross_entropy_fused")
def cross_entropy_fused(x, target_1b, weights=None, size_average=True, padding_value=-1):
    if x.dim() != 2 or not x.is_contiguous() or x.dtype not in (_bf16, _f32):
        return NotImplemented
    B, K = x.shape
    tf = target_1b.reshape(-1) if target_1b.dtype == _f32 and target_1b.device == x.device else None
    if tf is not None and (tf.numel() != B or not tf.is_contiguous() or not hasattr(_lib(), "bigdl_cross_entropy_ft")):
        tf = None
    t = None if tf is not None else _targets_i32(target_1b.to(x.device), B)
    if tf is None and t is None:
        return NotImplemented
    w = None
    if weights is not None:
        w = weights.to(x.device, _f32).contiguous()
        if w.numel() != K:
            return NotImplemented
    ws = torch.empty(3 * B, dtype=_f32, device=x.device)
    out = torch.empty(2, dtype=_f32, device=x.device)
    gx = torch.empty_like(x)
    fn = _lib().bigdl_cross_entropy_ft if tf is not None else _lib().bigdl_cross_entropy
    check(fn(ptr(x), ptr(tf if tf is not None else t), ptr(w), ptr(gx), _ll(B), C.c_int(K), C.c_int(int(padding_value)),
             C.c_int(1 if size_average else 0), C.c_int(1 if x.dtype == _bf16 else 0),
             ptr(ws), ptr(out), _s()), "cross_entropy")
    return out[0], gx


@register("log_softmax_forward")
def log_softmax_forward(x):
    if not x.is_contiguous() or x.dtype not in (_bf16, _f32) or x.dim() < 1 or x.numel() == 0:
        return NotImplemented
    K = x.shape[-1]
    rows = x.numel() // K
    y = torch.empty_like(x)
    check(_lib().bigdl_logsoftmax(ptr(x), ptr(None), ptr(y), _ll(rows), C.c_int(K), C.c_int(0),
                                  C.c_int(1 if x.dtype == _bf16 else 0), _s()), "logsoftmax")
    return y


@register("log_softmax_backward")
def log_softmax_backward(gy, y):
    if not (gy.is_contiguous() and y.is_contiguous()) or gy.dtype != y.dtype or y.dtype not in (_bf16, _f32) \
            or gy.shape != y.shape:
# ... 1331 lines not shown
    check(_lib().bigdl_gemm_i8_ex(ptr(qa), ptr(qb), C.c_int(M), C.c_int(N), C.c_int(Kp), None, C.c_float(sa0), ptr(sb),
                                  ptr(b), ptr(out), C.c_int(1 if out_dtype == _bf16 else 0), C.c_int(1 if relu else 0),
                                  C.c_float(out_scale if out_scale is not None else 0.0),
                                  C.c_int(1 if (out_scale is not None and out_u8) else 0), C.c_int(splits), ptr(work),
                                  _s()), "gemm_i8_ex")
    if out_scale is not None:
        _tag(out, out_scale, out_u8)
        out._qtail = False
    return out


@register("image_crop_flip_norm")
def image_crop_flip_norm(src, oy, ox, flip, out_h, out_w, mean, std, to_rgb, out_dtype=torch.float32):
    if src.dim() != 4 or src.dtype not in (torch.uint8, _f32) or not src.is_contiguous():
        return NotImplemented
    if out_dtype not in (_f32, _bf16):
        return NotImplemented
    B, H, W, Cc = src.shape
    if Cc > 4:
        return NotImplemented
    oy_c, ox_c, fl_c = (torch.as_tensor(v).reshape(-1).cpu().int() for v in (oy, ox, flip))
    if len(oy_c) != B or len(ox_c) != B or len(fl_c) != B:
        return NotImplemented
    if int(oy_c.max()) + out_h > H or int(ox_c.max()) + out_w > W or int(oy_c.min()) < 0 or int(ox_c.min()) < 0:
        raise ValueError("crop window outside the image")
    dev = src.device
    oy_d, ox_d, fl_d = (t.to(dev, non_blocking=True) for t in (oy_c, ox_c, fl_c))
    mean_f = (C.c_float * 4)(*[float(v) for v in list(mean)[:Cc]])
    std_f = (C.c_float * 4)(*[float(v) for v in list(std)[:Cc]])
    out = torch.empty((B, Cc, out_h, out_w), dtype=out_dtype, device=dev, memory_format=torch.channels_last)
    check(_lib().bigdl_image_crop_flip_norm(ptr(src), C.c_int(1 if src.dtype == torch.uint8 else 0), C.c_int(B),
                                            C.c_int(H), C.c_int(W), C.c_int(Cc), ptr(oy_d), ptr(ox_d), ptr(fl_d),
                                            C.c_int(out_h), C.c_int(out_w), mean_f, std_f,
                                            C.c_int(1 if to_rgb else 0), ptr(out),
                                            C.c_int(1 if out_dtype == _bf16 else 0), _s()), "image_crop_flip_norm")
    return out


def _pool_out(size, k, s, p, ceil_mode):
    if ceil_mode:
        o = -(-(size + 2 * p - k) // s) + 1
        if (o - 1) * s >= size + p:
            o -= 1
    else:
        o = (size + 2 * p - k) // s + 1
    return o


class _Int8Idx:
    __slots__ = ("t",)

    def __init__(self, t):
        self.t = t


@register("maxpool2d_forward")
def maxpool2d_forward(x, k, s, p, ceil_mode, need_indices=True):
    if (x.dim() == 4 and x.dtype == _f32 and x.is_contiguous(memory_format=torch.channels_last)
            and k[0] * k[1] <= 127 and p[0] * 2 <= k[0] and p[1] * 2 <= k[1]):
        N_, C_, H, W = x.shape
        P = _pool_out(H, k[0], s[0], p[0], ceil_mode)
        Q = _pool_out(W, k[1], s[1], p[1], ceil_mode)
        if P > 0 and Q > 0:
            y = torch.empty((N_, C_, P, Q), dtype=_f32, device=x.device, memory_format=torch.channels_last)
            idx = torch.empty((N_, P, Q, C_), dtype=torch.int8, device=x.device) if need_indices else None
            check(_lib().bigdl_maxpool32_fwd(ptr(x), ptr(y), ptr(idx), N_, H, W, C_, P, Q, k[0], k[1], s[0], s[1],
                                             p[0], p[1], _s()), "maxpool32_fwd")
            return y, (_Int8Idx(idx) if need_indices else None)
    if x.dim() != 4 or x.dtype != _bf16 or not x.is_contiguous(memory_format=torch.channels_last) or not _al16(x):
        return NotImplemented
    N_, C_, H, W = x.shape
    if k[0] * k[1] > 127 or p[0] * 2 > k[0] or p[1] * 2 > k[1] or (C_ % 8 and not x.is_contiguous(
            memory_format=torch.channels_last)):
        return NotImplemented
    P = _pool_out(H, k[0], s[0], p[0], ceil_mode)
    Q = _pool_out(W, k[1], s[1], p[1], ceil_mode)
    y = torch.empty((N_, C_, P, Q), dtype=_bf16, device=x.device, memory_format=torch.channels_last)
    idx = torch.empty((N_, P, Q, C_), dtype=torch.int8, device=x.device) if need_indices else None
    check(_lib().bigdl_maxpool_fwd(ptr(x), ptr(y), ptr(idx), N_, H, W, C_, P, Q, k[0], k[1], s[0], s[1], p[0], p[1],
                                   _s()), "maxpool_fwd")
    return y, (_Int8Idx(idx) if need_indices else None)


@register("maxpool2d_backward")
def maxpool2d_backward(gy, x, idx, k, s, p, ceil_mode):
    if not isinstance(idx, _Int8Idx):
        return NotImplemented
    N_, C_, H, W = x.shape
    P, Q = gy.shape[2], gy.shape[3]
    if x.dtype == _f32:
        gy = gy.float().contiguous(memory_format=torch.channels_last)
        gx = torch.empty((N_, C_, H, W), dtype=_f32, device=x.device, memory_format=torch.channels_last)
        check(_lib().bigdl_maxpool32_bwd(ptr(gy), ptr(idx.t), ptr(gx), N_, H, W, C_, P, Q, k[0], k[1], s[0], s[1],
                                         p[0], p[1], _s()), "maxpool32_bwd")
        return gx
    if gy.dtype != _bf16:
        gy = gy.to(_bf16)
    gy = gy.contiguous(memory_format=torch.channels_last)
    gx = torch.empty((N_, C_, H, W), dtype=_bf16, device=x.device, memory_format=torch.channels_last)
    check(_lib().bigdl_maxpool_bwd(ptr(gy), ptr(idx.t), ptr(gx), N_, H, W, C_, P, Q, k[0], k[1], s[0], s[1], p[0],
                                   p[1], _s()), "maxpool_bwd")
    return gx


def _lrn_ok(x, size):
    return (x.dim() == 4 and x.dtype in (_bf16, _f32) and x.is_contiguous(memory_format=torch.channels_last)
            and _al16(x) and x.shape[1] % 8 == 0 and size % 2 == 1 and x.numel() > 0)


@register("lrn_forward")
def lrn_forward(x, size, alpha, beta, k):
    if x.dim() == 4 and x.dtype == _f32 and not x.is_contiguous(memory_format=torch.channels_last):
        x = x.contiguous(memory_format=torch.channels_last)
    if not _lrn_ok(x, size) or size > 17:
        return NotImplemented
    y = torch.empty_like(x, memory_format=torch.channels_last)
    n, c, h, w = x.shape
    fn = _lib().bigdl_lrn_fwd_f32 if x.dtype == _f32 else _lib().bigdl_lrn_fwd
    check(fn(ptr(x), ptr(y), _ll(n * h * w), c, size, C.c_float(alpha), C.c_float(beta), C.c_float(k), _s()),
          "lrn_fwd")
    return y


@register("lrn_backward")
def lrn_backward(gy, x, size, alpha, beta, k):
    if x.dim() == 4 and x.dtype == _f32 and not x.is_contiguous(memory_format=torch.channels_last):
        x = x.contiguous(memory_format=torch.channels_last)
    if not _lrn_ok(x, size) or size > 9:
        return NotImplemented
    gy = gy.to(x.dtype).contiguous(memory_format=torch.channels_last)
    if gy.shape != x.shape or not _al16(gy):
        return NotImplemented
    gx = torch.empty_like(x, memory_format=torch.channels_last)
    n, c, h, w = x.shape
    fn = _lib().bigdl_lrn_bwd_f32 if x.dtype == _f32 else _lib().bigdl_lrn_bwd
    check(fn(ptr(x), ptr(gy), ptr(gx), _ll(n * h * w), c, size, C.c_float(alpha), C.c_float(beta), C.c_float(k),
             _s()), "lrn_bwd")
    return gx


class _DropMask:
    __slots__ = ("seed", "cl", "shape", "dev")

    def __init__(self, seed, cl, shape, dev=None):
        self.seed, self.cl, self.shape, self.dev = seed, cl, shape, dev


_DEV_SEED = {}


def _device_seed(device) -> torch.Tensor:
    t = _DEV_SEED.get(device)
    if t is None:
        t = torch.tensor([int(torch.randint(0, 2 ** 62, (1,)))], dtype=torch.int64, device=device)
        _DEV_SEED[device] = t
    return t


def _dense_layout(t):
    if t.is_contiguous():
        return False
    if t.dim() == 4 and t.is_contiguous(memory_format=torch.channels_last):
        return True
    return None


# ... 1228 lines not shown
```

bigdl-1_amd/bigdl/ops/reference.py:

```python
from __future__ import annotations

import ctypes
import math
from typing import Optional, Tuple

import torch
import torch.nn.functional as F
from ..utils import acc_float

aten = torch.ops.aten


def zero_fill(t: torch.Tensor):
    return t.zero_()


def cast_copy(dst: torch.Tensor, src: torch.Tensor):
    dst.copy_(src.reshape(dst.shape) if src.shape != dst.shape else src)
    return dst


def relu_forward(x: torch.Tensor, threshold: float = 0.0, value: float = 0.0, inplace=False):
    if threshold == 0.0 and value == 0.0:
        return torch.relu_(x) if inplace else torch.relu(x)
    y = torch.where(x > threshold, x, torch.full_like(x, value))
    if inplace:
        x.copy_(y)
        return x
    return y


def relu_backward(gy: torch.Tensor, y_or_x: torch.Tensor, threshold: float = 0.0):
    return gy * (y_or_x > threshold).to(gy.dtype)


def conv2d_forward(x, w4, b, stride, pad, dilation=(1, 1), groups=1, relu=False, out=None, res=None, pad_slot=None):
    y = F.conv2d(x, w4.to(x.dtype), None if b is None else b.to(x.dtype), stride, pad, dilation, groups)
    if res is not None:
        y = y + res.to(y.dtype)
    if relu:
        y = torch.relu(y)
    if out is not None:
        out.copy_(y)
        return out
    return y


def conv2d_backward(gy, x, w4, stride, pad, dilation=(1, 1), groups=1, need_input=True, gw_acc=None,
                    gb_acc=None, scale=1.0, residual=None, bn_fuse=None, pad_slot=None, lazy_strided=False):
    gy = gy.to(x.dtype)
    need_w = gw_acc is not None and scale != 0
    need_b = gb_acc is not None and scale != 0
    gi, gw, gb = aten.convolution_backward(gy, x, w4.to(x.dtype), [w4.shape[0]] if need_b else None,
                                           list(stride), list(pad), list(dilation), False, [0, 0], groups,
                                           [need_input, need_w, need_b])
    if need_w:
        gw_acc.add_(acc_float(gw), alpha=scale)
    if need_b:
        gb_acc.add_(acc_float(gb), alpha=scale)
    if residual is not None and gi is not None:
        gi = gi + as_dense(residual).to(gi.dtype)
    return gi


class StridedGrad:
    __slots__ = ("t", "stride", "shape")

    def __init__(self, t, stride, shape):
        self.t, self.stride, self.shape = t, tuple(stride), tuple(shape)

    def dense(self):
        fmt = torch.channels_last if self.t.is_contiguous(memory_format=torch.channels_last) else \
            torch.contiguous_format
        out = torch.empty(self.shape, dtype=self.t.dtype, device=self.t.device, memory_format=fmt).zero_()
        out[:, :, ::self.stride[0], ::self.stride[1]] = self.t
        return out


class BNOut:
    __slots__ = ("x", "coef", "shape", "relu")

    def __init__(self, x, coef, relu=False):
        self.x, self.coef, self.shape, self.relu = x, coef, tuple(x.shape), relu

    @property
    def dtype(self):
        return self.x.dtype

    @property
    def is_cuda(self):
        return self.x.is_cuda

    @property
    def device(self):
        return self.x.device

    def dim(self):
        return self.x.dim()

    def dense(self):
        C = self.shape[1]
        sc = self.coef[:C].view(1, C, *([1] * (self.x.dim() - 2)))
        sh = self.coef[C:2 * C].view(1, C, *([1] * (self.x.dim() - 2)))
        y = torch.addcmul(sh, self.x.float(), sc)
        if self.relu:
            y = torch.relu(y)
        return y.to(self.x.dtype).contiguous(memory_format=torch.channels_last) if self.x.dim() == 4 \
            else y.to(self.x.dtype)


class BNGrad:
    __slots__ = ("g", "x", "coef", "shape")

    def __init__(self, g, x, coef):
        self.g, self.x, self.coef, self.shape = g, x, coef, tuple(x.shape)

    @property
    def dtype(self):
        return self.g.dtype

    @property
    def is_cuda(self):
        return self.g.is_cuda

    def dense(self):
        from . import native as N
        if self.g.is_cuda and N.has("batchnorm_backward"):
            M, C = self.g.numel() // self.shape[1], self.shape[1]
            gx = torch.empty_like(self.g)
            N.check(N.lib().bigdl_bn_bwd_apply_coef(N.ptr(self.g), N.ptr(self.x), N.ptr(gx), ctypes.c_longlong(M),
                                                    ctypes.c_int(C), N.ptr(self.coef),
                                                    ctypes.c_void_p(N.stream_ptr())), "bn_bwd_apply_coef")
            return gx
        C = self.shape[1]
        sh = [1, C] + [1] * (len(self.shape) - 2)
        a, b, c = (self.coef[i * C:(i + 1) * C].view(sh) for i in range(3))
        return (a * self.g.float() + b * self.x.float() + c).to(self.g.dtype)


def as_dense(g):
    return g.dense() if isinstance(g, (StridedGrad, BNGrad)) else g


def conv_transpose2d_forward(x, w4, b, stride, pad, adj, dilation=(1, 1), groups=1):
    return F.conv_transpose2d(x, w4.to(x.dtype), None if b is None else b.to(x.dtype), stride, pad, adj, groups,
                              dilation)


def _resize_axis(n_in, n_out, align, device):
    scale = (n_in - 1) / (n_out - 1) if (align and n_out > 1) else n_in / n_out
    src = torch.arange(n_out, dtype=torch.float32, device=device) * torch.tensor(scale, dtype=torch.float32)
    lo = src.to(torch.int64).clamp_max(n_in - 1)
    hi = (lo + 1).clamp_max(n_in - 1)
    return lo, hi, src - lo.to(torch.float32)


def resize_bilinear(x, oh, ow, align=False):
    y0, y1, ly = _resize_axis(x.shape[2], oh, align, x.device)
    x0, x1, lx = _resize_axis(x.shape[3], ow, align, x.device)
    xf = x if x.dtype == torch.float64 else x.float()
    top, bot = xf.index_select(2, y0), xf.index_select(2, y1)
    lx_, ly_ = lx.to(xf.dtype).view(1, 1, 1, -1), ly.to(xf.dtype).view(1, 1, -1, 1)
    t = top.index_select(3, x0) + (top.index_select(3, x1) - top.index_select(3, x0)) * lx_
    b = bot.index_select(3, x0) + (bot.index_select(3, x1) - bot.index_select(3, x0)) * lx_
    return (t + (b - t) * ly_).to(x.dtype)


def batchnorm_forward_train(x, gamma, beta, running_mean, running_var, momentum, eps, relu=False, residual=None,
                            in_bias=None, coef_out=None, bits_out=None):
    C = x.shape[1]
    dims = [d for d in range(x.dim()) if d != 1]
    xf = acc_float(x)
    n = x.numel() // C
    mean = xf.mean(dim=dims)
    var = xf.var(dim=dims, unbiased=False)
    invstd = torch.rsqrt(var + eps)
    if running_mean is not None:
        with torch.no_grad():
            unbiased = var * (n / max(n - 1, 1))
            true_mean = mean if in_bias is None else mean + acc_float(in_bias)
            running_mean.mul_(1 - momentum).add_(true_mean, alpha=momentum)
            running_var.mul_(1 - momentum).add_(unbiased, alpha=momentum)
    shape = [1, C] + [1] * (x.dim() - 2)
    g = acc_float(gamma).view(shape) if gamma is not None else 1.0
    bb = acc_float(beta).view(shape) if beta is not None else 0.0
    if coef_out is not None:
        sc = invstd * (acc_float(gamma) if gamma is not None else 1.0)
        coef_out[:C].copy_(sc)
        coef_out[C:2 * C].copy_((acc_float(beta) if beta is not None else 0.0) - mean * sc)
    y = (xf - mean.view(shape)) * invstd.view(shape) * g + bb
    if residual is not None:
        y = y + acc_float(residual)
    if relu:
        y = torch.relu(y)
    y = y.to(x.dtype)
    if bits_out is not None and relu and x.dim() == 4 and C % 8 == 0:
        pos = (y.permute(0, 2, 3, 1).reshape(-1, 8) > 0).to(torch.int32)
        w = (2 ** torch.arange(8, device=y.device, dtype=torch.int32)).view(1, 8)
        bits_out.copy_((pos * w).sum(1).to(torch.uint8))
    return y, mean, invstd


def batchnorm_forward_infer(x, gamma, beta, running_mean, running_var, eps, relu=False, in_bias=None):
    C = x.shape[1]
    shape = [1, C] + [1] * (x.dim() - 2)
    invstd = torch.rsqrt(acc_float(running_var) + eps)
    scale = invstd * (acc_float(gamma) if gamma is not None else 1.0)
    rm = acc_float(running_mean) - (acc_float(in_bias) if in_bias is not None else 0.0)
    shift = (acc_float(beta) if beta is not None else 0.0) - rm * scale
    y = acc_float(x) * scale.view(shape) + shift.view(shape)
    if relu:
        y = torch.relu(y)
    return y.to(x.dtype)


def batchnorm_backward(gy, x, gamma, save_mean, save_invstd, y=None, relu=False, need_input=True, gg_acc=None,
                       gb_acc=None, scale=1.0, cbias_acc=None, cbias_scale=1.0, want_gres=False):
    C = x.shape[1]
    dims = [d for d in range(x.dim()) if d != 1]
    shape = [1, C] + [1] * (x.dim() - 2)
    g = acc_float(gy)
    if relu:
        g = g * (y > 0).float()
    xhat = (acc_float(x) - save_mean.view(shape)) * save_invstd.view(shape)
    dbeta = g.sum(dim=dims)
    dgamma = (g * xhat).sum(dim=dims)
    gi = None
    if need_input or cbias_acc is not None:
        n = x.numel() // C
        gam = acc_float(gamma).view(shape) if gamma is not None else 1.0
        gif = (gam * save_invstd.view(shape) / n) * (n * g - dbeta.view(shape) - xhat * dgamma.view(shape))
        if cbias_acc is not None and cbias_scale != 0:
            cbias_acc.add_(gif.sum(dim=dims), alpha=cbias_scale)
        gi = gif.to(x.dtype) if need_input else None
    if gg_acc is not None and scale != 0:
        gg_acc.add_(dgamma, alpha=scale)
    if gb_acc is not None and scale != 0:
        gb_acc.add_(dbeta, alpha=scale)
    return gi, (g.to(gy.dtype) if want_gres else None)


def _bn_dims(x):
    return [d for d in range(x.dim()) if d != 1], [1, x.shape[1]] + [1] * (x.dim() - 2)


def bn_local_sums(x, shift, partial=None, G=0, rezero=False):
    C = x.shape[1]
    dims, shape = _bn_dims(x)
    if partial is not None:
        p = partial.view(2, G, C).sum(1)
        out = torch.cat([p.reshape(-1), p.new_tensor([float(x.numel() // C)])])
        if rezero:
            partial.zero_()
        return out
    xf = acc_float(x).double() - acc_float(shift).double().view(shape)
    out = torch.cat([xf.sum(dims), (xf * xf).sum(dims), xf.new_tensor([float(x.numel() // C)])])
    return out.to(acc_float(x).dtype if acc_float(x).dtype != torch.float64 else torch.float64)


def bn_forward_from_sums(x, sums, count, shift, gamma, beta, running_mean, running_var, momentum, eps, relu=False,
                         residual=None, in_bias=None, coef_out=None, bits_out=None, apply=True):
    C = x.shape[1]
    dims, shape = _bn_dims(x)
    n = sums[2 * C].double() if count == 0 else torch.tensor(float(count), dtype=torch.float64, device=x.device)
    dm = sums[:C].double() / n
    var = (sums[C:2 * C].double() / n - dm * dm).clamp_min(0)
    fd = acc_float(x).dtype
    mean = (acc_float(shift).double() + dm).to(fd)
    var = var.to(fd)
    invstd = torch.rsqrt(var + eps)
    if running_mean is not None:
        with torch.no_grad():
            unb = (var.double() * n / (n - 1).clamp_min(1)).to(fd)
            tm = mean if in_bias is None else mean + acc_float(in_bias)
            running_mean.mul_(1 - momentum).add_(tm, alpha=momentum)
            running_var.mul_(1 - momentum).add_(unb, alpha=momentum)
    sc = invstd * (acc_float(gamma) if gamma is not None else 1.0)
    sh = (acc_float(beta) if beta is not None else 0.0) - mean * sc
    if coef_out is not None:
        coef_out[:C].copy_(sc)
        coef_out[C:2 * C].copy_(sh)
    if not apply:
        return None, mean, invstd
    y = acc_float(x) * sc.view(shape) + sh.view(shape)
    if isinstance(residual, BNOut):
        residual = residual.dense()
    if residual is not None:
        y = y + acc_float(residual)
    if relu:
        y = torch.relu(y)
    return y.to(x.dtype), mean, invstd


def bn_bwd_local_sums(gy, x, save_mean, y=None, relu=False):
    C = x.shape[1]
    dims, shape = _bn_dims(x)
    g = acc_float(gy)
    if relu:
        g = g * (y > 0).float()
    xc = acc_float(x) - save_mean.view(shape)
    loc = torch.cat([g.sum(dims), (g * xc).sum(dims)])
    return torch.cat([loc, loc, loc.new_tensor([float(x.numel() // C)])])


def bn_bwd_partials_sums(partial, G, C_, dev, rows=None, rezero=False):
    p = partial.view(2, G, C_).sum(1).reshape(-1)
    out = torch.cat([p, p, p.new_tensor([float(rows)])])
    if rezero:
        partial.zero_()
    return out


def bn_backward_from_sums(gy, x, gamma, save_mean, save_invstd, local_sums, global_sums, count, y=None, relu=False,
                          need_input=True, gg_acc=None, gb_acc=None, scale=1.0, cbias_acc=None, cbias_scale=1.0):
    C = x.shape[1]
    dims, shape = _bn_dims(x)
    n = global_sums[2 * C] if count == 0 else torch.tensor(float(count), device=x.device)
    is_ = save_invstd
    if gg_acc is not None and scale != 0:
        gg_acc.add_(local_sums[C:2 * C] * is_, alpha=scale)
    if gb_acc is not None and scale != 0:
        gb_acc.add_(local_sums[:C], alpha=scale)
    gm = acc_float(gamma) if gamma is not None else torch.ones_like(is_)
    db, dgc = global_sums[:C], global_sums[C:2 * C]
    A = gm * is_
    B = -gm * is_ * is_ * (dgc * is_) / n
    Cc = -gm * is_ * db / n - B * save_mean
    if cbias_acc is not None and cbias_scale != 0:
        m_loc = float(x.numel() // C)
        cbias_acc.add_(A * local_sums[:C] + m_loc * (B * save_mean + Cc), alpha=cbias_scale)
    if not need_input:
        return None
    g = acc_float(gy)
    if relu:
        g = g * (y > 0).float()
    gx = A.view(shape) * g + B.view(shape) * acc_float(x) + Cc.view(shape)
    return gx.to(x.dtype)


def maxpool2d_forward(x, k, s, p, ceil_mode, need_indices=True):
    if not need_indices:
        return F.max_pool2d(x, k, s, p, 1, ceil_mode), None
    y, idx = F.max_pool2d(x, k, s, p, 1, ceil_mode, return_indices=True)
    return y, idx


def maxpool2d_backward(gy, x, idx, k, s, p, ceil_mode):
    if hasattr(idx, "t") and not isinstance(idx, torch.Tensor):
        _, idx = maxpool2d_forward(x, k, s, p, ceil_mode)
    return aten.max_pool2d_with_indices_backward(gy, x, list(k), list(s), list(p), [1, 1], ceil_mode, idx)


def avgpool2d_forward(x, k, s, p, ceil_mode, count_include_pad, divisor=None):
    return F.avg_pool2d(x, k, s, p, ceil_mode, count_include_pad, divisor)


def avgpool2d_backward(gy, x, k, s, p, ceil_mode, count_include_pad, divisor=None):
    if (x.dim() == 4 and tuple(k) == tuple(x.shape[-2:]) and tuple(p) == (0, 0) and tuple(gy.shape[-2:]) == (1, 1)):
        fmt = torch.channels_last if x.is_contiguous(memory_format=torch.channels_last) and not x.is_contiguous() \
            else torch.contiguous_format
        g = torch.div(gy, float(divisor or x.shape[-2] * x.shape[-1]))
        return g.expand(x.shape).contiguous(memory_format=fmt)
    return aten.avg_pool2d_backward(gy, x, list(k), list(s), list(p), ceil_mode, count_include_pad, divisor)


def linear_forward(x, w, b):
    y = x @ w.to(x.dtype).t()
    if b is not None:
        y = y + b.to(y.dtype)
    return y


def linear_backward(gy, x, w, need_input=True, gw_acc=None, gb_acc=None, scale=1.0):
    gi = gy @ w.to(gy.dtype) if need_input else None
    if gw_acc is not None and scale != 0:
        gw_acc.add_(acc_float(gy).t() @ acc_float(x), alpha=scale)
    if gb_acc is not None and scale != 0:
        gb_acc.add_(acc_float(gy).sum(0), alpha=scale)
    return gi


def log_softmax_forward(x):
    return torch.log_softmax(acc_float(x), dim=-1).to(x.dtype)


def log_softmax_backward(gy, y):
    gyf = acc_float(gy)
    return (gyf - torch.exp(acc_float(y)) * gyf.sum(-1, keepdim=True)).to(y.dtype)


def softmax_forward(x):
    return torch.softmax(acc_float(x), dim=-1).to(x.dtype)


def softmax_backward(gy, y):
    gyf, yf = acc_float(gy), acc_float(y)
    return (yf * (gyf - (gyf * yf).sum(-1, keepdim=True))).to(y.dtype)


def class_nll_forward(logp, target_1b, weights=None, size_average=True, padding_value=-1):
    if logp.dim() == 1:
        logp = logp.unsqueeze(0)
        target_1b = target_1b.reshape(1)
    t = target_1b.long().reshape(-1)
    valid = t != padding_value
    idx = torch.where(valid, t - 1, torch.zeros_like(t))
    picked = acc_float(logp).gather(1, idx.unsqueeze(1)).squeeze(1)
    w = acc_float(weights)[idx] if weights is not None else torch.ones_like(picked)
    w = w * acc_float(valid)
    total = -(picked * w).sum()
    if size_average:
        denom = w.sum()
        total = total / torch.clamp(denom, min=1e-12) if weights is not None else total / torch.clamp(acc_float(valid).sum(), min=1)
    return total


def class_nll_backward(logp, target_1b, weights=None, size_average=True, padding_value=-1):
    squeeze = logp.dim() == 1
    lp = logp.unsqueeze(0) if squeeze else logp
    t = target_1b.long().reshape(-1)
    valid = t != padding_value
    idx = torch.where(valid, t - 1, torch.zeros_like(t))
    w = acc_float(weights)[idx] if weights is not None else torch.ones(t.shape[0], device=lp.device)
    w = w * acc_float(valid)
    if size_average:
        denom = w.sum() if weights is not None else acc_float(valid).sum()
        w = w / torch.clamp(denom, min=1e-12 if weights is not None else 1)
    g = torch.zeros(lp.shape, dtype=torch.float32, device=lp.device)
    g.scatter_(1, idx.unsqueeze(1), (-w).unsqueeze(1))
    g = g.to(logp.dtype)
    return g.squeeze(0) if squeeze else g


def cross_entropy_fused(x, target_1b, weights=None, size_average=True, padding_value=-1):
    logp = torch.log_softmax(acc_float(x), dim=-1)
# ... 299 lines not shown
```

bigdl-1_amd/bigdl/utils/config.py:

```python
from __future__ import annotations

import os
import threading

_lock = threading.Lock()

_REGISTRY = {
    "bigdl.localMode": (bool, False, "run without a process group"),
    "bigdl.coreNumber": (int, 0, "host threads for CPU ops (0 = auto)"),
    "bigdl.engineType": (str, "hip", "kept for compatibility: 'mklblas'/'mkldnn' map to the native engine"),
    "bigdl.multiModels": (bool, False, "compat flag (one replica per GPU here)"),
    "bigdl.utils.Engine.defaultPoolSize": (int, 0, "host pool size"),
    "bigdl.check.singleton": (bool, False, "compat"),
    "bigdl.failure.retryTimes": (int, 5, "optimizer retry budget"),
    "bigdl.graph.capture": (bool, False, "LocalOptimizer on a GPU: capture the training step into a HIP graph"),
    "bigdl.comm.timeout": (float, 600.0, "collective watchdog: seconds before a hung RCCL/gloo collective raises"),
    "bigdl.failure.retryTimeInterval": (int, 120, "retry window seconds"),
    "bigdl.failure.resume": (bool, False, "resume from the latest checkpoint at optimize() start (automatic after a launcher restart)"),
    "bigdl.embedding.syncCheck": (bool, False, "check LookupTable ids synchronously after every GPU lookup (debug; default: the out-of-range flag is read back asynchronously and raised at the next lookup)"),
    "bigdl.straggler.window": (int, 20, "iterations between straggler checks (all-gather of per-rank step times)"),
    "bigdl.straggler.factor": (float, 1.5, "a rank is slow when its step time exceeds factor x the kthLargest threshold"),
    "bigdl.Parameter.syncPoolSize": (int, 4, "compat"),
    "bigdl.Parameter.computePoolSize": (int, 0, "compat"),
    "bigdl.parallelOptimizer.parameterBlocks": (int, 10, "number of gradient buckets for overlap mode"),
    "bigdl.compute.dtype": (str, "auto", "auto (bf16 on a GPU, fp32 on the host) | fp32 | bf16 compute dtype"),
    "bigdl.comm.dtype": (str, "fp32", "fp32 | bf16 | bf16_truncate wire format for gradient reduction"),
    "bigdl.comm.bucketMB": (float, 32.0, "gradient bucket size for RCCL collectives"),
    "bigdl.comm.overlap": (bool, True, "overlap gradient reduce-scatter with backward"),
    "bigdl.comm.sharded": (bool, True, "reduce-scatter + sharded update + all-gather (ZeRO-1)"),
    "bigdl.comm.channels": (int, 0, "RCCL channel cap (NCCL_MIN/MAX_NCHANNELS, set by the launcher before any GPU call; 0 = RCCL default): bounds the CUs collectives take from compute"),
    "bigdl.comm.streamPriority": (int, -1, "priority of the comm-side stream that runs the shard update + all-gather (-1 = high, 0 = normal)"),
    "bigdl.comm.aliasWorld1": (bool, True, "sharded mode with one rank: the shard tensors alias the parameter arena and the identity reduce-scatter / all-gather are skipped"),
    "bigdl.comm.earlyUpdate": (bool, True, "sharded mode on a GPU: issue each bucket's shard update + all-gather on the comm-side stream as soon as its reduce-scatter is launched (overlaps the rest of backward)"),
    "bigdl.metrics.jsonPath": (str, "", "per-rank JSON metrics stream: one line per iteration to <path>.rank<r>.jsonl ('' = off)"),
    "bigdl.metrics.deviceTimers": (bool, False, "time the distributed phases with HIP events (adds no host sync)"),
    "bigdl.bn.atomicStats": (bool, False, "conv epilogues ADD the BN statistics into a [2C] buffer with fp32 atomics and the BN runs as ONE finalize+apply launch (forward and backward); off (or bigdl.deterministic) = per-tile partial rows + fold/finalize kernels, bit-reproducible. Off by default: the same-address atomics from thousands of tiles cost more conv time than the fold launches they remove (25.04 vs 23.09 ms/step, profiles/r4_bn_atomic_ab.txt)"),
    "bigdl.syncbn.ownComm": (bool, True, "SyncBN statistics all-reduces run over a communicator of their own (own RCCL stream), not the one the gradient buckets use"),
    "bigdl.bn.statReplicas": (int, 32, "R > 0 (with atomicStats off): conv epilogues ADD the BN statistics into R replicas (tile tm → replica tm % R) of a zeroed buffer — R-fold less same-address atomic contention than atomicStats, and the BN finalizes from R rows with no fold pass; 0 = per-tile partial rows. Default 32: 22.50 vs 22.94 ms/step (profiles/r4_bn_replicas_ab.txt)"),
    "bigdl.bn.foldFinalize": (bool, False, "training BN from a conv's replicated statistics in ONE launch per pass: every apply block reduces the replicas itself (no finalize kernel), block 0 updates the running statistics and clears the other of two alternating replica sets; the statistics shift is the previous step's batch mean (a two-buffer ring), so no block reads what block 0 writes. Off: 22.45 vs 21.05 ms/step — re-reducing the R·C replica rows in each of ~1000 apply blocks costs more than the finalize launches it removes (profiles/r5_bn_fold_ab.txt)"),
    "bigdl.bn.syncOneRankLocal": (bool, True, "a SyncBN whose sync group has ONE rank (also the forced world-size-1 rehearsal) runs the local BN kernels: the all-reduce is the identity there, so the compaction of the statistics replicas and the one-launch global finalize+apply are skipped; False rehearses the multi-rank kernels at one rank"),
    "bigdl.bn.shiftedStats": (bool, True, "conv-epilogue BN statistics as Σ(y−K), Σ(y−K)² with K = the BN running mean"),
    "bigdl.checkpoint.async": (bool, True, "trigger-driven checkpoints: host snapshot on the training thread, serialise + write on a writer thread"),
    "bigdl.predict.compiled": (bool, True, "LocalPredictor / Predictor / PredictionService on a GPU: lower the model through the IR (BN fold, conv+sum+ReLU), plan each batch shape once and replay its forward as a HIP graph (the reference's predictors always convert, LocalPredictor.scala:66)"),
    "bigdl.compile.lower": (bool, True, "nn.compiled.compile (inference phase): lower the model through the IR first (utils/intermediate.ConversionUtils: BN folded into convs / Linears, conv+sum+ReLU epilogues)"),
    "bigdl.roctx": (bool, False, "emit roctx ranges around forward / backward / reduce-scatter / update / all-gather"),
    "bigdl.native.require": (bool, True, "fail loudly on a GPU if the HIP extension is missing"),
    "bigdl.native.strict": (bool, False, "raise instead of warning when a device-tensor op falls back to the torch reference"),
    "bigdl.step.overlapMinMs": (float, 8.0, "enable the high-priority step stream and async wgrad once the measured step period is at least this long (GPU-bound steps; launch-bound ones lose to the extra host work)"),
    "bigdl.step.maxInflight": (int, 2, "GPU training iterations the host may queue ahead of the device (0 = unbounded): a host far ahead of a GPU-bound step piles up cross-stream events and fresh allocations (blocks still read by the wgrad side stream cannot be recycled) and was measured to stall for seconds (profiles/r6_fp32_runahead.txt)"),
    "bigdl.step.highPriority": (bool, True, "run each GPU training iteration on a high-priority HIP stream (the critical path outranks side-stream wgrad work)"),
    "bigdl.fp32.native": (bool, True, "fp32 compute on a GPU: convolutions and Linear run the bf16x3 split on the MFMA kernels (ops/fp32x3.py; ≤2^-16 relative per product) instead of torch/MIOpen fp32"),
    "bigdl.fp32.twoPart": (bool, True, "fp32 compute: activation splits stored as [hi | lo] and read by the conv kernels as [hi | hi | lo] (ConvParams::cdup); false = the three-part [hi | hi | lo] buffers"),
    "bigdl.fp32.producerSplit": (bool, True, "fp32 compute: the BN apply passes also write the [hi | lo] split of their output for the consuming conv (forward input, backward dY), so the conv skips its own split pass"),
    "bigdl.fp32.bnPrologue": (bool, True, "fp32 compute: a training BN + ReLU whose only consumer is a conv hands its output over deferred (ops.reference.BNOut); the conv applies relu(x·scale + shift) in its forward B-operand and weight-gradient X-operand prologues (conv_x3 / conv_wgrad PRO) and its dgrad epilogue recomputes the ReLU mask — the BN output is never written or read"),
    "bigdl.fp32.stemC4": (bool, True, "fp32 compute: a conv with ≤ 4 input channels (the RGB stem) reads a 4-channel NHWC copy of its input and gathers 8 taps × 4 channels per k-tile (conv_x3.hip MODE 2, conv_wgrad.hip C4 F32): 224 reduction indices for the 7×7 stem instead of the space-to-depth image's 512"),
    "bigdl.fp32.direct": (bool, True, "fp32 compute: convolutions with C % 32 == 0 read the fp32 activations and gradients directly (csrc/conv_x3.hip: hi / lo split while reading the MFMA fragments; conv_wgrad.hip F32: split between load and LDS store) — no [hi | lo] split is materialised and the BN passes write fp32 only"),
    "bigdl.fp32.convStats": (bool, True, "fp32 compute: a conv followed by a training BN adds the BN statistics into the BN's replicated buffer from its fp32 epilogue (the BN skips its statistics pass)"),
    "bigdl.compile.trainAutotune": (bool, True, "training compile phase: the first GPU training iteration records its conv launches (forward, backward-data, weight-gradient) and pins the fastest kernel candidate per geometry"),
    "bigdl.compile.autotune": (bool, True, "nn.compiled.compile on a GPU (inference): time every implicit-GEMM conv tile candidate per conv geometry and pin the fastest (kernel selection)"),
    "bigdl.conv.asyncWgrad": (bool, True, "inside optimizer steps run conv backward-weight kernels on a second HIP stream, overlapping the backward-data / BatchNorm chain"),
    "bigdl.deterministic": (bool, False, "bit-reproducible kernels: single-writer reductions instead of split-K float atomics (slower wgrad / embedding backward)"),
    "bigdl.native.enable": (bool, True, "False routes device tensors to the torch reference ops (debug/A-B only)"),
    "bigdl.profile.sync": (bool, False, "synchronize the device around per-module timers"),
    "bigdl.profile.deviceTimers": (bool, False, "per-module HIP-event forward/backward timers (resolved lazily by getDeviceTimes)"),
    "bigdl.optim.foldRegularizers": (bool, True, "apply pure-L2 layer regularizers inside the fused SGD update"),
    "bigdl.lars.fused": (bool, True, "LarsSGD methods with device weights run as one LarsPlan (layer-norm kernels + one fused update, no host sync) under the LocalOptimizer and in replicated mode; sharded mode always uses the plan"),
    "bigdl.int8.calibration": (str, "p99.999", "static int8 activation scale rule of quantize() after calcScales: max (max|x|, the reference's) or p99.9 / p99.99 / p99.999 (that percentile of |x|)"),
    "bigdl.int8.unsignedActivations": (bool, True, "a quantised conv whose ReLU is fused writes its non-negative int8 output as unsigned 8-bit (offset -128, scale clip/255); the consumer corrects the offset with per-tap weight sums"),
    "bigdl.int8.foldBN": (bool, True, "quantize() folds evaluation BatchNorms into the preceding convolution before quantising its weights (the reference's int8 conv + BN fusion)"),
    "bigdl.int8.residual": (bool, True, "quantize() turns ConcatTable(branch, shortcut) + CAddTable + ReLU blocks into int8 residual blocks (conv + sum epilogue, int8 block outputs chained to the next block)"),
    "bigdl.int8.quantizeLinear": (bool, True, "quantize() converts Linear layers too (int8 GEMM, per-row dynamic input scales); False keeps them in the compute dtype"),
    "bigdl.fusion": (bool, True, "enable layer fusion"),
    "bigdl.fusion.convbn": (bool, True, "fold BN into conv for inference"),
    "bigdl.fusion.bnrelu": (bool, True, "fuse BN + ReLU"),
    "bigdl.fusion.convrelu": (bool, True, "fuse conv + ReLU"),
    "bigdl.fusion.lstmstack": (bool, True, "run two stacked Recurrent(LSTM) layers on the layer wavefront"),
    "bigdl.fusion.convsum": (bool, True, "fuse residual add"),
    "bigdl.fusion.convstats": (bool, True, "conv epilogue emits the following training BN's statistics"),
    "bigdl.fusion.shortcutbn": (bool, True, "a ResNet block's conv->BN shortcut hands its BN output to the fused tail deferred (input + coefficients), applied inside the tail's pass"),
    "bigdl.fusion.bnbwd": (bool, True, "dgrad epilogue applies the producing BN's ReLU mask and its backward reductions"),
    "bigdl.fusion.bnprologue": (int, 0, "a BN whose producer is a 1x1 stride-1 conv hands it the input gradient "
                                         "deferred (A*g + B*x + C applied in the conv's dgrad / wgrad operand loads): "
                                         "0 off, 1 when the BN is narrower than the conv input, 2 always "
                                         "(profiles/r3_bn_prologue_ab.txt)"),
    "bigdl.utils.LoggerFilter.disable": (bool, False, "disable log redirect"),
    "bigdl.utils.LoggerFilter.logFile": (str, "bigdl.log", "log file"),
    "bigdl.utils.LoggerFilter.enableSparkLog": (bool, True, "compat"),
}

_overrides: dict = {}
_listeners: dict = {}


def on_change(key: str, fn):
    _listeners.setdefault(key, []).append(fn)


def _env_name(key: str) -> str:
    return "BIGDL_" + key.replace("bigdl.", "", 1).replace(".", "_").upper()


def _coerce(typ, v):
    if typ is bool:
        if isinstance(v, bool):
            return v
        return str(v).strip().lower() in ("1", "true", "yes", "on")
    return typ(v)


def get_property(key: str, default=None):
    with _lock:
        if key in _overrides:
            return _overrides[key]
    typ, dflt, _ = _REGISTRY.get(key, (str, default, ""))
    env = os.environ.get(_env_name(key))
    if env is not None:
        return _coerce(typ, env)
    sysprop = os.environ.get(key)
    if sysprop is not None:
        return _coerce(typ, sysprop)
    return dflt if default is None else default


_VERSION = [0]


def version() -> int:
    return _VERSION[0]


def set_property(key: str, value):
    typ = _REGISTRY.get(key, (type(value), None, ""))[0]
    with _lock:
        _overrides[key] = _coerce(typ, value)
        _VERSION[0] += 1
    for fn in _listeners.get(key, ()):
        fn(get_property(key))


def clear_property(key: str):
    with _lock:
        _overrides.pop(key, None)
        _VERSION[0] += 1
    for fn in _listeners.get(key, ()):
        fn(get_property(key))


def describe() -> dict:
    return {k: get_property(k) for k in _REGISTRY}
```

Baseline: 12360 images/sec.

## Fuse stem BN+ReLU into max-pool forward and pool-gradient gather into BN backward

Adds a bnpool fusion for the ResNet stem: a training BN+ReLU that feeds a 3x3 stride-2 max-pool hands over its input and coefficients deferred. The pool kernel applies BN and ReLU to its window taps on load, and the BN backward gathers the pool gradient through int8 argmax indices, so the dense BN output and dense pool gradient are never materialised. The BN backward can also take the ReLU mask from the coefficients or bit-packed masks instead of the dense output. This targets memory traffic at the largest activation in the network, at the cost of extra index arithmetic and new kernels with many fallback conditions.

```diff
diff --git a/bigdl-1_amd/bigdl/nn/fusion.py b/bigdl-1_amd/bigdl/nn/fusion.py
--- a/bigdl-1_amd/bigdl/nn/fusion.py
+++ b/bigdl-1_amd/bigdl/nn/fusion.py
@@ -5,6 +5,7 @@
 from .layers.activation import Threshold
 from .layers.conv import SpatialConvolution
 from .layers.normalization import BatchNormalization, SpatialBatchNormalization
+from .layers.pooling import SpatialMaxPooling
 from .layers.table_ops import CAddTable
 
 
@@ -73,7 +74,7 @@
                     _link_stack(n.element, m.element)
 
 
-def fuse(model, convbn=None, bnrelu=None, convsum=None, bnbwd=None, convrelu=None):
+def fuse(model, convbn=None, bnrelu=None, convsum=None, bnbwd=None, convrelu=None, bnpool=None):
     if not config.get_property("bigdl.fusion"):
         return model
     if getattr(model, "_fused", False):
@@ -84,6 +85,7 @@
     bnrelu = config.get_property("bigdl.fusion.bnrelu") if bnrelu is None else bnrelu
     convsum = config.get_property("bigdl.fusion.convsum") if convsum is None else convsum
     bnbwd = config.get_property("bigdl.fusion.bnbwd") if bnbwd is None else bnbwd
+    bnpool = config.get_property("bigdl.fusion.bnpool") if bnpool is None else bnpool
     tails, heads = [], []
     for s in model.flattened_modules():
         if not isinstance(s, Sequential):
@@ -106,6 +108,10 @@
                     c._bn_bwd_target = a
                     if type(c) in _PLAIN_CONVS:
                         a._pro_consumer = c
+                if (bnpool and type(c) is SpatialMaxPooling and c._bnpool_ok() and a._pool_consumer is None
+                        and c._bn_producer is None):
+                    a._pool_consumer = c
+                    c._bn_producer = a
         if not convsum:
             continue
         for i in range(len(mods) - 1):
@@ -185,8 +191,12 @@
             m._fused_relu = False
             m._defer_ok = False
             m._pro_consumer = None
+            m._pool_consumer = None
             m._pending_stats = None
             m._pending_grad = None
+        if isinstance(m, SpatialMaxPooling):
+            m._bn_producer = None
+            m._bn_in = None
         if isinstance(m, Threshold):
             m._passthrough = False
         if isinstance(m, ConcatTable):
diff --git a/bigdl-1_amd/bigdl/nn/layers/conv.py b/bigdl-1_amd/bigdl/nn/layers/conv.py
--- a/bigdl-1_amd/bigdl/nn/layers/conv.py
+++ b/bigdl-1_amd/bigdl/nn/layers/conv.py
@@ -6,7 +6,7 @@
 import torch.nn.functional as F
 
 from ... import ops
-from ...ops.reference import BNGrad, BNOut, StridedGrad, as_dense
+from ...ops.reference import BNGrad, BNOut, DeferredBN, StridedGrad, as_dense
 from ...utils.engine import Engine
 from ...utils import config
 from ..abstractnn import AbstractModule, TensorModule, AutogradModule
@@ -172,7 +172,7 @@
             y = self._pro_forward(pro[0], pro[1])
             if y is not NotImplemented:
                 return y
-        if isinstance(input, BNOut):
+        if isinstance(input, DeferredBN):
             input = input.dense()
         x, pad, batched, _ = self._prep(input)
         w4 = self._w4(self.cw("weight"))
@@ -229,7 +229,7 @@
             r = self._pro_backward(pro[0], pro[1], gradOutput, need_input, acc)
             if r is not NotImplemented:
                 return r
-        if isinstance(input, BNOut):
+        if isinstance(input, DeferredBN):
             input = input.dense()
         x, pad, batched, pads = self._prep(input)
         if isinstance(gradOutput, BNGrad):
diff --git a/bigdl-1_amd/bigdl/nn/layers/normalization.py b/bigdl-1_amd/bigdl/nn/layers/normalization.py
--- a/bigdl-1_amd/bigdl/nn/layers/normalization.py
+++ b/bigdl-1_amd/bigdl/nn/layers/normalization.py
@@ -112,6 +112,8 @@
     _last_input = None
     _pending_grad = None
     _relu_bits = None
+    _pool_consumer = None
+    _last_res = False
 
     def _atomic_sums(self, kind, C, device):
         if device.type != "cuda" or config.get_property("bigdl.deterministic"):
@@ -199,6 +201,13 @@
         from ...ops import fp32x3 as F3
         return F3.pro_ok(x, coef)
 
+    def _pool_deferrable(self, x, relu, residual):
+        c = self._pool_consumer
+        return (c is not None and relu and residual is None and x.is_cuda and x.dtype == torch.bfloat16
+                and x.dim() == 4 and x.shape[1] % 8 == 0 and x.is_contiguous(memory_format=torch.channels_last)
+                and c._bn_producer is self and c.train and c._bnpool_ok()
+                and bool(config.get_property("bigdl.fusion.bnpool")) and ops.native_has("maxpool2d_forward"))
+
     def forward_residual(self, x, residual, relu):
         self._residual_mode = True
         self._res_relu = relu
@@ -212,7 +221,7 @@
         return self._forward_impl(input, None, self._fused_relu)
 
     def _forward_impl(self, input, residual, relu):
-        from ...ops.reference import BNOut
+        from ...ops.reference import BNOut, BNPoolOut
         x = input
         if x.dim() == 1:
             x = x.unsqueeze(0)
@@ -229,6 +238,7 @@
         b = self.cw("bias", pdt) if self.affine else None
         ib = self._in_bias()
         self._last_relu = relu
+        self._last_res = residual is not None
         if self.train:
             if self._sync_active():
                 y, mean, invstd = self._sync_forward(x, g, b, relu, residual, ib, defer=defer)
@@ -241,15 +251,17 @@
                 ps, self._pending_stats = self._pending_stats, None
                 bits = self._tail_bits(x, relu, residual)
                 self._relu_bits = None
+                pooldefer = False
                 if ps is not None and ps[0] == x.data_ptr() and ps[1] == tuple(x.shape):
-                    special = defer or deferred_res
+                    pooldefer = not (defer or deferred_res) and self._pool_deferrable(x, relu, residual)
+                    special = defer or deferred_res or pooldefer
                     pdefer = not special and self._pro_deferrable(x, relu, residual, coef)
                     r = ops.native_ops.batchnorm_forward_train_partials(
                         x, ps[2], ps[3], g, b, self.runningMean, self.runningVar, self.momentum, self.eps,
                         relu=relu, residual=residual, in_bias=ib, coef_out=coef, shift=ps[4],
-                        bits_out=None if pdefer else bits,
+                        bits_out=None if (pdefer or pooldefer) else bits,
                         rezero=self._is_rep(ps[2]), zero_next=None if special else self._rep_next("fwd", ps[2]),
-                        mean_out=self._shift_next(ps[4]), apply=not (defer or pdefer))
+                        mean_out=self._shift_next(ps[4]), apply=not (defer or pdefer or pooldefer))
                     if r is not NotImplemented and not special:
                         self._rep_flip("fwd", ps[2])
                 if r is NotImplemented:
@@ -262,7 +274,7 @@
                 self._relu_bits = bits
                 y, mean, invstd = r
                 if y is None:
-                    y = BNOut(x, coef, relu=bool(relu))
+                    y = BNPoolOut(x, coef, relu=True) if pooldefer else BNOut(x, coef, relu=bool(relu))
                 self._advance_shift(mean)
                 self._last_input = x
             self.saveMean, self.saveStd = mean, invstd
@@ -362,7 +374,57 @@
         self._drop_sums(ps, 3)
         return r
 
+    def _bwd_pool(self, input, pg, need_input, acc):
+        out = self.output
+        if (pg.src is not out or not self.train or self._sync_active() or self.scale_w != self.scale_b
+                or input.dim() != 4 or not getattr(self, "_last_relu", False) or self._last_res):
+            return NotImplemented
+        x = to_device_layout(input)
+        if x is not out.x and x.data_ptr() != out.x.data_ptr():
+            return NotImplemented
+        impl = ops.native_ops if (x.is_cuda and ops.native_has("batchnorm_backward")) else ops.reference
+        if x.is_cuda and impl is ops.reference:
+            return NotImplemented
+        g = self.cw("weight", torch.float64 if x.dtype == torch.float64 else torch.float32) if self.affine else None
+        prod = self._bias_producer
+        cb = prod.gradBias if (acc and prod is not None and getattr(prod, "withBias", False)) else None
+        cbs = prod.scale_b if prod is not None else 0.0
+        self._drop_sums(self._pending_grad, 2)
+        self._pending_grad = None
+        return impl.batchnorm_backward_pool(pg, x, g, self.saveMean, self.saveStd, fcoef=out.coef,
+                                            need_input=need_input,
+                                            gg_acc=self.gradWeight if (acc and self.affine) else None,
+                                            gb_acc=self.gradBias if (acc and self.affine) else None,
+                                            scale=self.scale_w if acc else 0.0, cbias_acc=cb, cbias_scale=cbs)
+
+    def _same_input(self, x):
+        li = self._last_input
+        return li is not None and (li is x or (li.data_ptr() == x.data_ptr() and li.shape == x.shape
+                                               and li.stride() == x.stride()))
+
+    def _mask_source(self, x, y, relu):
+        from ...ops.reference import DeferredBN as BNOut
+        if not (relu and self.train and x.is_cuda and x.dtype == torch.bfloat16 and x.dim() == 4
+                and x.shape[1] % 8 == 0 and self._same_input(x) and ops.native_has("batchnorm_backward")):
+            return (y.dense() if isinstance(y, BNOut) else y), None, None
+        C_ = x.shape[1]
+        if not self._last_res:
+            coef = y.coef if isinstance(y, BNOut) else self._coef
+            if coef is not None and coef.numel() == 2 * C_ and coef.device == x.device:
+                return None, coef, None
+        elif not isinstance(y, BNOut):
+            bits = self._relu_bits
+            if bits is not None and bits.numel() == x.numel() // 8 and bits.device == x.device:
+                return None, None, bits
+        return (y.dense() if isinstance(y, BNOut) else y), None, None
+
     def _bwd(self, input, gradOutput, need_input, acc, want_gres=False):
+        from ...ops.reference import PoolGrad
+        if isinstance(gradOutput, PoolGrad):
+            gi = self._bwd_pool(input, gradOutput, need_input, acc)
+            if gi is not NotImplemented:
+                return (gi, None) if want_gres else gi
+            gradOutput = gradOutput.dense()
         x = input if input.dim() > 1 else input.unsqueeze(0)
         gy = gradOutput if gradOutput.dim() > 1 else gradOutput.unsqueeze(0)
         if x.dim() == 4:
@@ -370,10 +432,13 @@
             gy = to_device_layout(gy)
         relu = getattr(self, "_last_relu", self._fused_relu)
         y = self.output if relu else None
-        from ...ops.reference import BNOut
+        from ...ops.reference import DeferredBN as BNOut
         if isinstance(y, BNOut):
-            y = None if (self._pending_grad is not None and self._pending_grad[0] == gy.data_ptr()) else y.dense()
-        if y is not None and y.dim() == 1:
+            if self._pending_grad is not None and self._pending_grad[0] == gy.data_ptr():
+                y = None
+            elif self._sync_active() and self.train:
+                y = y.dense()
+        if isinstance(y, torch.Tensor) and y.dim() == 1:
             y = y.unsqueeze(0)
         g = self.cw("weight", torch.float64 if x.dtype == torch.float64 else torch.float32) if self.affine else None
         prod = self._bias_producer
@@ -405,14 +470,16 @@
                         gi = gi.reshape(input.shape)
                     return (gi, gy) if want_gres else gi
             self._drop_sums(pg, 2)
+            y, fcoef, mbits = self._mask_source(x, y, relu)
+            mkw = {} if (fcoef is None and mbits is None) else dict(fcoef=fcoef, mask_bits=mbits)
             gi, gres = ops.batchnorm_backward(gy, x, g, self.saveMean, self.saveStd, y=y, relu=relu,
-                                              need_input=need_input,
+                                              need_input=need_input, **mkw,
                                               gg_acc=self.gradWeight if (acc and self.affine) else None,
                                               gb_acc=self.gradBias if (acc and self.affine and same) else None,
                                               scale=self.scale_w if acc else 0.0, cbias_acc=cb, cbias_scale=cbs,
                                               want_gres=want_gres)
             if acc and self.affine and not same and self.scale_b != 0:
-                gf = acc_float(gy) * ((y > 0).float() if relu else 1.0)
+                gf = acc_float(gy) * (ops.reference.relu_mask(x, y, fcoef, mbits).float() if relu else 1.0)
                 dims = [d for d in range(gf.dim()) if d != 1]
                 self.gradBias.add_(gf.sum(dims), alpha=self.scale_b)
         if gi is not None and input.dim() == 1:
diff --git a/bigdl-1_amd/bigdl/nn/layers/pooling.py b/bigdl-1_amd/bigdl/nn/layers/pooling.py
--- a/bigdl-1_amd/bigdl/nn/layers/pooling.py
+++ b/bigdl-1_amd/bigdl/nn/layers/pooling.py
@@ -73,7 +73,37 @@
         y = NO.maxpool_i8(input, self.kH, self.kW, self.dH, self.dW, pt, pl, P, Q)
         return None if y is NotImplemented else y
 
+    _bn_producer = None
+    _bn_in = None
+
+    def _bnpool_ok(self):
+        return (self.format == "NCHW" and not self.ceilMode and (self.kW, self.kH, self.dW, self.dH) == (3, 3, 2, 2)
+                and self.padW in (0, 1) and self.padH in (0, 1))
+
+    def _bnpool_forward(self, bnout):
+        if not (self._bnpool_ok() and bnout.dim() == 4 and self.train):
+            return None
+        k, s, p = (self.kH, self.kW), (self.dH, self.dW), (self.padH, self.padW)
+        if bnout.is_cuda:
+            if not ops.native_has("maxpool2d_forward"):
+                return None
+            r = ops.native_ops.bn_maxpool_forward(bnout, k, s, p, False, need_indices=True)
+        else:
+            r = ops.reference.bn_maxpool_forward(bnout, k, s, p, False, need_indices=True)
+        if r is NotImplemented:
+            return None
+        self._indices = r[1]
+        self._bn_in = bnout
+        return r[0]
+
     def updateOutput(self, input):
+        from ...ops.reference import DeferredBN
+        self._bn_in = None
+        if isinstance(input, DeferredBN):
+            y = self._bnpool_forward(input)
+            if y is not None:
+                return y
+            input = input.dense()
         if input.dtype == torch.int8 and getattr(input, "_qscale", None) is not None:
             y = self._int8_forward(input)
             if y is not None:
@@ -87,6 +117,16 @@
         return self._post(y, batched)
 
     def updateGradInput(self, input, gradOutput):
+        from ...ops.reference import DeferredBN, PoolGrad, as_dense
+        gradOutput = as_dense(gradOutput)
+        if isinstance(input, DeferredBN):
+            if input is self._bn_in and self._indices is not None:
+                gy = to_device_layout(gradOutput)
+                if gy.dtype != input.dtype:
+                    gy = gy.to(input.dtype)
+                return PoolGrad(gy, self._indices, (self.kH, self.kW), (self.dH, self.dW), (self.padH, self.padW),
+                                input)
+            input = input.dense()
         x, pad, batched, pads = self._prep(input)
         gy = gradOutput
         if self.format == "NHWC":
diff --git a/bigdl-1_amd/bigdl/ops/csrc/batchnorm.hip b/bigdl-1_amd/bigdl/ops/csrc/batchnorm.hip
--- a/bigdl-1_amd/bigdl/ops/csrc/batchnorm.hip
+++ b/bigdl-1_amd/bigdl/ops/csrc/batchnorm.hip
@@ -406,11 +406,103 @@
   BIGDL_CHECK_LAUNCH();
 }
 
-template <bool RELU>
+enum { kMaskNone = 0, kMaskY = 1, kMaskCoef = 2, kMaskBits = 3 };
+
+struct BnPoolSrc {
+  const int8_t* idx;
+  int H, W, P, Q, ph, pw;
+};
+
+template <int MASK, bool GATHER>
+struct BnBwdRow {
+  static constexpr int NG = GATHER ? 4 : 1;
+  bigdl_u32x4 g[NG], xq, yq;
+  uint2 a[NG];
+  uint32_t me;
+  uint32_t bits;
+
+  __device__ __forceinline__ void issue(const bf16_t* __restrict__ gy, const bf16_t* __restrict__ x,
+                                        const void* __restrict__ msk, const BnPoolSrc& ps, long long r, int C,
+                                        int cg) {
+    const size_t off = (size_t)r * C + (size_t)cg * 8;
+    xq = __builtin_nontemporal_load(reinterpret_cast<const bigdl_u32x4*>(x + off));
+    if (MASK == kMaskY)
+      yq = __builtin_nontemporal_load(reinterpret_cast<const bigdl_u32x4*>(static_cast<const bf16_t*>(msk) + off));
+    if (MASK == kMaskBits) bits = static_cast<const uint8_t*>(msk)[off >> 3];
+    if (!GATHER) {
+      g[0] = __builtin_nontemporal_load(reinterpret_cast<const bigdl_u32x4*>(gy + off));
+      return;
+    }
+    const unsigned ru = (unsigned)r, HW = (unsigned)ps.H * (unsigned)ps.W;
+    const unsigned n = ru / HW, rem = ru - n * HW;
+    const int h = (int)(rem / (unsigned)ps.W), w = (int)(rem - (unsigned)h * (unsigned)ps.W);
+    const int hp = h + ps.ph, wp = w + ps.pw;
+    const int pa = hp / 2 - 1, qa = wp / 2 - 1;
+    me = 0;
+#pragma unroll
+    for (int u = 0; u < 2; ++u)
+#pragma unroll
+      for (int v2 = 0; v2 < 2; ++v2) {
+        const int p = pa + u, q = qa + v2, k = 2 * u + v2;
+        const int i = hp - 2 * p, j = wp - 2 * q;
+        const bool ok = p >= 0 && p < ps.P && q >= 0 && q < ps.Q && i <= 2 && j <= 2;
+        me |= (ok ? (uint32_t)(i * 3 + j) : 0xFFu) << (8 * k);
+        const int pp = ok ? p : 0, qq = ok ? q : 0;
+        const size_t o = (((size_t)n * ps.P + pp) * ps.Q + qq) * C + (size_t)cg * 8;
+        a[k] = *reinterpret_cast<const uint2*>(ps.idx + o);
+        g[k] = *reinterpret_cast<const bigdl_u32x4*>(gy + o);
+      }
+  }
+
+  __device__ __forceinline__ void get(const float* fsc, const float* fsh, float* gv, float* xv) const {
+    unpack8(make_uint4(xq[0], xq[1], xq[2], xq[3]), xv);
+    if (!GATHER) {
+      unpack8(make_uint4(g[0][0], g[0][1], g[0][2], g[0][3]), gv);
+    } else {
+#pragma unroll
+      for (int e = 0; e < 8; ++e) gv[e] = 0.f;
+#pragma unroll
+      for (int k = 0; k < NG; ++k) {
+        float t[8];
+        unpack8(make_uint4(g[k][0], g[k][1], g[k][2], g[k][3]), t);
+        const uint32_t aw[2] = {a[k].x, a[k].y};
+        const uint32_t mk = (me >> (8 * k)) & 0xFFu;
+#pragma unroll
+        for (int e = 0; e < 8; ++e)
+          if (((aw[e >> 2] >> (8 * (e & 3))) & 0xFFu) == mk) gv[e] += t[e];
+      }
+    }
+    if (MASK == kMaskY) {
+      float yv[8];
+      unpack8(make_uint4(yq[0], yq[1], yq[2], yq[3]), yv);
+#pragma unroll
+      for (int k = 0; k < 8; ++k) gv[k] = yv[k] > 0.f ? gv[k] : 0.f;
+    }
+    if (MASK == kMaskCoef) {
+#pragma unroll
+      for (int k = 0; k < 8; ++k) gv[k] = fmaf(xv[k], fsc[k], fsh[k]) > 0.f ? gv[k] : 0.f;
+    }
+    if (MASK == kMaskBits) {
+#pragma unroll
+      for (int k = 0; k < 8; ++k) gv[k] = ((bits >> k) & 1u) ? gv[k] : 0.f;
+    }
+  }
+};
+
+template <int MASK>
+__device__ __forceinline__ void bn_bwd_fcoef(const void* msk, int C, int cg, float* fsc, float* fsh) {
+#pragma unroll
+  for (int k = 0; k < 8; ++k) {
+    fsc[k] = MASK == kMaskCoef ? static_cast<const float*>(msk)[cg * 8 + k] : 0.f;
+    fsh[k] = MASK == kMaskCoef ? static_cast<const float*>(msk)[C + cg * 8 + k] : 0.f;
+  }
+}
+
+template <int MASK, bool GATHER = false>
 __global__ void __launch_bounds__(256) k_bn_bwd_reduce(const bf16_t* __restrict__ gy, const bf16_t* __restrict__ x,
-                                                       const bf16_t* __restrict__ y, long long M, int C,
+                                                       const void* __restrict__ msk, long long M, int C,
                                                        long long rows_per_block, const float* __restrict__ mean,
-                                                       float* __restrict__ partial, int G) {
+                                                       float* __restrict__ partial, int G, BnPoolSrc ps = BnPoolSrc()) {
   extern __shared__ __attribute__((aligned(16))) float smem[];
   BnGeom g = bn_geom(C);
   const int t = threadIdx.x;
@@ -421,26 +513,30 @@
   if (r1 > M) r1 = M;
   float* s_a = smem;
   float* s_b = smem + g.RPI * C;
+  constexpr int U = GATHER ? 4 : 1;
   for (int cg = cg_local; cg < g.CG; cg += g.tpr) {
     if (r_off >= g.RPI) break;
-    float mu[8], a[8], b[8];
+    float mu[8], a[8], b[8], fsc[8], fsh[8];
 #pragma unroll
     for (int k = 0; k < 8; ++k) { mu[k] = mean[cg * 8 + k]; a[k] = 0.f; b[k] = 0.f; }
-    for (long long r = r0 + r_off; r < r1; r += g.RPI) {
-      size_t off = (size_t)r * C + (size_t)cg * 8;
-      float gv[8], xv[8];
-      load8_nt(gy + off, gv);
-      load8_nt(x + off, xv);
-      if (RELU) {
-        float yv[8];
-        load8_nt(y + off, yv);
-#pragma unroll
-        for (int k = 0; k < 8; ++k) gv[k] = yv[k] > 0.f ? gv[k] : 0.f;
+    bn_bwd_fcoef<MASK>(msk, C, cg, fsc, fsh);
+    for (long long r = r0 + r_off; r < r1; r += (long long)U * g.RPI) {
+      BnBwdRow<MASK, GATHER> row[U];
+#pragma unroll
+      for (int u = 0; u < U; ++u) {
+        const long long ru = r + (long long)u * g.RPI;
+        row[u].issue(gy, x, msk, ps, ru < r1 ? ru : r, C, cg);
       }
 #pragma unroll
-      for (int k = 0; k < 8; ++k) {
-        a[k] += gv[k];
-        b[k] = fmaf(gv[k], xv[k] - mu[k], b[k]);
+      for (int u = 0; u < U; ++u) {
+        if (r + (long long)u * g.RPI >= r1) break;
+        float gv[8], xv[8];
+        row[u].get(fsc, fsh, gv, xv);
+#pragma unroll
+        for (int k = 0; k < 8; ++k) {
+          a[k] += gv[k];
+          b[k] = fmaf(gv[k], xv[k] - mu[k], b[k]);
+        }
       }
     }
 #pragma unroll
@@ -492,10 +588,11 @@
   if (cbias) cbias[c] += cbscale * (A * dbeta + B * Mf * mean[c] + Mf * Cc);
 }
 
-template <bool RELU, bool GRES, int kApplyUnroll>
+template <int MASK, bool GRES, int kApplyUnroll, bool GATHER = false>
 __device__ __forceinline__ void bn_bwd_apply_rows(const bf16_t* __restrict__ gy, const bf16_t* __restrict__ x,
-                                                  const bf16_t* __restrict__ y, bf16_t* __restrict__ gx,
-                                                  bf16_t* __restrict__ gres, long long M, int C, const float* coef) {
+                                                  const void* __restrict__ msk, bf16_t* __restrict__ gx,
+                                                  bf16_t* __restrict__ gres, long long M, int C, const float* coef,
+                                                  const BnPoolSrc& ps = BnPoolSrc()) {
   BnGeom g = bn_geom(C);
   const int t = threadIdx.x;
   const int cg_local = t % g.tpr;
@@ -503,23 +600,21 @@
   if (r_off >= g.RPI) return;
   const long long rstride = (long long)gridDim.x * g.RPI;
   for (int cg = cg_local; cg < g.CG; cg += g.tpr) {
-    float A[8], B[8], Cc[8];
+    float A[8], B[8], Cc[8], fsc[8], fsh[8];
 #pragma unroll
     for (int k = 0; k < 8; ++k) {
       A[k] = coef[cg * 8 + k];
       B[k] = coef[C + cg * 8 + k];
       Cc[k] = coef[2 * C + cg * 8 + k];
     }
+    bn_bwd_fcoef<MASK>(msk, C, cg, fsc, fsh);
     long long r = (long long)blockIdx.x * g.RPI + r_off;
     for (; r < M; r += kApplyUnroll * rstride) {
-      bigdl_u32x4 gq[kApplyUnroll], xq[kApplyUnroll], yq[kApplyUnroll];
+      BnBwdRow<MASK, GATHER> row[kApplyUnroll];
 #pragma unroll
       for (int u = 0; u < kApplyUnroll; ++u) {
         const long long ru = r + u * rstride;
-        const size_t off = (size_t)(ru < M ? ru : r) * C + (size_t)cg * 8;
-        gq[u] = __builtin_nontemporal_load(reinterpret_cast<const bigdl_u32x4*>(gy + off));
-        xq[u] = __builtin_nontemporal_load(reinterpret_cast<const bigdl_u32x4*>(x + off));
-        if (RELU) yq[u] = __builtin_nontemporal_load(reinterpret_cast<const bigdl_u32x4*>(y + off));
+        row[u].issue(gy, x, msk, ps, ru < M ? ru : r, C, cg);
       }
 #pragma unroll
       for (int u = 0; u < kApplyUnroll; ++u) {
@@ -527,14 +622,7 @@
         if (ru >= M) break;
         const size_t off = (size_t)ru * C + (size_t)cg * 8;
         float gv[8], xv[8];
-        unpack8(make_uint4(gq[u][0], gq[u][1], gq[u][2], gq[u][3]), gv);
-        unpack8(make_uint4(xq[u][0], xq[u][1], xq[u][2], xq[u][3]), xv);
-        if (RELU) {
-          float yv[8];
-          unpack8(make_uint4(yq[u][0], yq[u][1], yq[u][2], yq[u][3]), yv);
-#pragma unroll
-          for (int k = 0; k < 8; ++k) gv[k] = yv[k] > 0.f ? gv[k] : 0.f;
-        }
+        row[u].get(fsc, fsh, gv, xv);
         if (GRES) store8(gres + off, gv);
 #pragma unroll
         for (int k = 0; k < 8; ++k) xv[k] = fmaf(A[k], gv[k], fmaf(B[k], xv[k], Cc[k]));
@@ -544,12 +632,12 @@
   }
 }
 
-template <bool RELU, bool GRES, int kApplyUnroll = 4>
+template <int MASK, bool GRES, int kApplyUnroll = 4, bool GATHER = false>
 __global__ void __launch_bounds__(256) k_bn_bwd_apply(const bf16_t* __restrict__ gy, const bf16_t* __restrict__ x,
-                                                      const bf16_t* __restrict__ y, bf16_t* __restrict__ gx,
+                                                      const void* __restrict__ msk, bf16_t* __restrict__ gx,
                                                       bf16_t* __restrict__ gres, long long M, int C,
-                                                      const float* __restrict__ coef) {
-  bn_bwd_apply_rows<RELU, GRES, kApplyUnroll>(gy, x, y, gx, gres, M, C, coef);
+                                                      const float* __restrict__ coef, BnPoolSrc ps = BnPoolSrc()) {
+  bn_bwd_apply_rows<MASK, GRES, kApplyUnroll, GATHER>(gy, x, msk, gx, gres, M, C, coef, ps);
 }
 
 BIGDL_EXPORT int bigdl_bn_bwd(const void* gy, const void* x, const void* y, void* gx, void* gres, long long M, int C,
@@ -572,11 +660,75 @@
     int grid = apply_grid(M, C);
     const bf16_t *g_ = (const bf16_t*)gy, *x_ = (const bf16_t*)x, *y_ = (const bf16_t*)y;
     bf16_t *gx_ = (bf16_t*)gx, *gr_ = (bf16_t*)gres;
-    if (relu && gres) hipLaunchKernelGGL((k_bn_bwd_apply<true, true>), dim3(grid), dim3(256), 0, s, g_, x_, y_, gx_, gr_, M, C, coef);
-    else if (relu) hipLaunchKernelGGL((apply_unroll1() ? k_bn_bwd_apply<true, false, 1> : k_bn_bwd_apply<true, false, 4>), dim3(grid), dim3(256), 0, s, g_, x_, y_, gx_, gr_, M, C, coef);
-    else if (gres) hipLaunchKernelGGL((k_bn_bwd_apply<false, true>), dim3(grid), dim3(256), 0, s, g_, x_, y_, gx_, gr_, M, C, coef);
-    else hipLaunchKernelGGL((apply_unroll1() ? k_bn_bwd_apply<false, false, 1> : k_bn_bwd_apply<false, false, 4>), dim3(grid), dim3(256), 0, s, g_, x_, y_, gx_, gr_, M, C, coef);
-  }
+    if (relu && gres) hipLaunchKernelGGL((k_bn_bwd_apply<true, true>), dim3(grid), dim3(256), 0, s, g_, x_, y_, gx_, gr_, M, C, coef, BnPoolSrc());
+    else if (relu) hipLaunchKernelGGL((apply_unroll1() ? k_bn_bwd_apply<true, false, 1> : k_bn_bwd_apply<true, false, 4>), dim3(grid), dim3(256), 0, s, g_, x_, y_, gx_, gr_, M, C, coef, BnPoolSrc());
+    else if (gres) hipLaunchKernelGGL((k_bn_bwd_apply<false, true>), dim3(grid), dim3(256), 0, s, g_, x_, y_, gx_, gr_, M, C, coef, BnPoolSrc());
+    else hipLaunchKernelGGL((apply_unroll1() ? k_bn_bwd_apply<false, false, 1> : k_bn_bwd_apply<false, false, 4>), dim3(grid), dim3(256), 0, s, g_, x_, y_, gx_, gr_, M, C, coef, BnPoolSrc());
+  }
+  BIGDL_CHECK_LAUNCH();
+}
+
+template <int MASK, bool GATHER, bool GRES>
+static void launch_bwd_src(const void* gy, const void* x, const void* msk, void* gx, void* gres, long long M, int C,
+                           const float* gamma, const float* mean, const float* invstd, float* ggamma, float* gbeta,
+                           float gscale, float* cbias, float cbscale, float* ws, float* coef, const BnPoolSrc& ps,
+                           hipStream_t s) {
+  const int G = bigdl_bn_num_partials(M, C);
+  const long long rpb = (M + G - 1) / G;
+  hipLaunchKernelGGL((k_bn_bwd_reduce<MASK, GATHER>), dim3(G), dim3(256), stats_smem(C), s, (const bf16_t*)gy,
+                     (const bf16_t*)x, msk, M, C, rpb, mean, ws, G, ps);
+  hipLaunchKernelGGL(k_bn_bwd_finalize<float>, dim3((C + 31) / 32), dim3(32 * kFinRG), 0, s, (const float*)ws, G, M, C,
+                     gamma, mean, invstd, ggamma, gbeta, gscale, cbias, cbscale, coef);
+  if (!gx) return;
+  constexpr int U = GATHER ? 2 : 4;
+  hipLaunchKernelGGL((k_bn_bwd_apply<MASK, GRES, U, GATHER>), dim3(apply_grid(M, C)), dim3(256), 0, s,
+                     (const bf16_t*)gy, (const bf16_t*)x, msk, (bf16_t*)gx, (bf16_t*)gres, M, C, coef, ps);
+}
+
+static bool al16(const void* p) { return ((uintptr_t)p & 15) == 0; }
+
+BIGDL_EXPORT int bigdl_bn_bwd_mask(const void* gy, const void* x, const void* mask, int mask_kind, void* gx, void* gres,
+                                   long long M, int C, const float* gamma, const float* mean, const float* invstd,
+                                   float* ggamma, float* gbeta, float gscale, float* cbias, float cbscale, float* ws,
+                                   float* coef, hipStream_t s) {
+  if (C % 8 || M <= 0 || !gy || !x || !mask || !mean || !invstd || !ws || !coef) return (int)hipErrorInvalidValue;
+  if ((mask_kind != kMaskCoef && mask_kind != kMaskBits) || (gres && !gx)) return (int)hipErrorInvalidValue;
+  if (!al16(gy) || !al16(x) || !al16(gx) || !al16(gres) || stats_smem(C) > 64 * 1024) return (int)hipErrorInvalidValue;
+  const BnPoolSrc ps = BnPoolSrc();
+#define BIGDL_BWD_SRC(MK, GR) \
+  launch_bwd_src<MK, false, GR>(gy, x, mask, gx, gres, M, C, gamma, mean, invstd, ggamma, gbeta, gscale, cbias, \
+                                cbscale, ws, coef, ps, s)
+  if (mask_kind == kMaskCoef) {
+    if (gres) BIGDL_BWD_SRC(kMaskCoef, true);
+    else BIGDL_BWD_SRC(kMaskCoef, false);
+  } else {
+    if (gres) BIGDL_BWD_SRC(kMaskBits, true);
+    else BIGDL_BWD_SRC(kMaskBits, false);
+  }
+#undef BIGDL_BWD_SRC
+  BIGDL_CHECK_LAUNCH();
+}
+
+BIGDL_EXPORT int bigdl_bn_bwd_pool(const void* gp, const void* idx, const void* x, const float* fcoef, void* gx, int N,
+                                   int H, int W, int C, int P, int Q, int ph, int pw, const float* gamma,
+                                   const float* mean, const float* invstd, float* ggamma, float* gbeta, float gscale,
+                                   float* cbias, float cbscale, float* ws, float* coef, hipStream_t s) {
+  if (C <= 0 || C % 8 || N <= 0 || H <= 0 || W <= 0 || P <= 0 || Q <= 0 || ph < 0 || ph > 1 || pw < 0 || pw > 1)
+    return (int)hipErrorInvalidValue;
+  if (!gp || !idx || !x || !mean || !invstd || !ws || !coef) return (int)hipErrorInvalidValue;
+  const long long M = (long long)N * H * W;
+  if (M >= 0x7fffffffLL || (long long)H * W >= 0x7fffffffLL) return (int)hipErrorInvalidValue;
+  if (!al16(gp) || !al16(x) || !al16(gx) || ((uintptr_t)idx & 7) || stats_smem(C) > 64 * 1024)
+    return (int)hipErrorInvalidValue;
+  BnPoolSrc ps;
+  ps.idx = (const int8_t*)idx;
+  ps.H = H; ps.W = W; ps.P = P; ps.Q = Q; ps.ph = ph; ps.pw = pw;
+  if (fcoef)
+    launch_bwd_src<kMaskCoef, true, false>(gp, x, fcoef, gx, nullptr, M, C, gamma, mean, invstd, ggamma, gbeta, gscale,
+                                           cbias, cbscale, ws, coef, ps, s);
+  else
+    launch_bwd_src<kMaskNone, true, false>(gp, x, nullptr, gx, nullptr, M, C, gamma, mean, invstd, ggamma, gbeta,
+                                           gscale, cbias, cbscale, ws, coef, ps, s);
   BIGDL_CHECK_LAUNCH();
 }
 
@@ -595,7 +747,7 @@
   if (gx) {
     int grid = apply_grid(M, C);
     hipLaunchKernelGGL((apply_unroll1() ? k_bn_bwd_apply<false, false, 1> : k_bn_bwd_apply<false, false, 4>), dim3(grid), dim3(256), 0, s, (const bf16_t*)gm,
-                       (const bf16_t*)x, (const bf16_t*)nullptr, (bf16_t*)gx, (bf16_t*)nullptr, M, C, coef);
+                       (const bf16_t*)x, (const bf16_t*)nullptr, (bf16_t*)gx, (bf16_t*)nullptr, M, C, coef, BnPoolSrc());
   }
   BIGDL_CHECK_LAUNCH();
 }
@@ -605,7 +757,7 @@
   if (C % 8 || M <= 0 || !gm || !x || !gx || !coef) return (int)hipErrorInvalidValue;
   hipLaunchKernelGGL((apply_unroll1() ? k_bn_bwd_apply<false, false, 1> : k_bn_bwd_apply<false, false, 4>),
                      dim3(apply_grid(M, C)), dim3(256), 0, s, (const bf16_t*)gm, (const bf16_t*)x,
-                     (const bf16_t*)nullptr, (bf16_t*)gx, (bf16_t*)nullptr, M, C, coef);
+                     (const bf16_t*)nullptr, (bf16_t*)gx, (bf16_t*)nullptr, M, C, coef, BnPoolSrc());
   BIGDL_CHECK_LAUNCH();
 }
 
@@ -1055,10 +1207,10 @@
     bf16_t* gx_ = (bf16_t*)gx;
     if (relu)
       hipLaunchKernelGGL((apply_unroll1() ? k_bn_bwd_apply<true, false, 1> : k_bn_bwd_apply<true, false, 4>), dim3(grid), dim3(256), 0, s, g_, x_, y_, gx_, (bf16_t*)nullptr, M, C,
-                         coef);
+                         coef, BnPoolSrc());
     else
       hipLaunchKernelGGL((apply_unroll1() ? k_bn_bwd_apply<false, false, 1> : k_bn_bwd_apply<false, false, 4>), dim3(grid), dim3(256), 0, s, g_, x_, y_, gx_, (bf16_t*)nullptr, M,
-                         C, coef);
+                         C, coef, BnPoolSrc());
   }
   BIGDL_CHECK_LAUNCH();
 }
diff --git a/bigdl-1_amd/bigdl/ops/csrc/pooling.hip b/bigdl-1_amd/bigdl/ops/csrc/pooling.hip
--- a/bigdl-1_amd/bigdl/ops/csrc/pooling.hip
+++ b/bigdl-1_amd/bigdl/ops/csrc/pooling.hip
@@ -100,6 +100,67 @@
         }
     const size_t o = (((size_t)n * g.P + p) * g.Q + q) * g.C + cg * 8;
     pst8(y + o, best);
+    if (!idx) continue;
+    uint32_t lo = 0, hi = 0;
+#pragma unroll
+    for (int e = 0; e < 4; ++e) lo |= (uint32_t)(arg[e] & 0xFF) << (8 * e);
+#pragma unroll
+    for (int e = 0; e < 4; ++e) hi |= (uint32_t)(arg[4 + e] & 0xFF) << (8 * e);
+    *reinterpret_cast<uint2*>(idx + o) = make_uint2(lo, hi);
+  }
+}
+
+template <typename IT, bool RELU>
+__global__ void __launch_bounds__(256) k_bn_maxpool_fwd_k3s2(const bf16_t* __restrict__ x,
+                                                             const float* __restrict__ coef,
+                                                             bf16_t* __restrict__ y, int8_t* __restrict__ idx,
+                                                             PoolGeom g) {
+  const int CG = g.C >> 3;
+  const IT total = (IT)g.N * g.P * g.Q * CG;
+  for (IT t = blockIdx.x * (IT)blockDim.x + threadIdx.x; t < total; t += (IT)gridDim.x * blockDim.x) {
+    const int cg = (int)(t % CG);
+    IT pix = t / CG;
+    const int q = (int)(pix % g.Q);
+    pix /= g.Q;
+    const int p = (int)(pix % g.P);
+    const int n = (int)(pix / g.P);
+    const int h0 = p * 2 - g.ph, w0 = q * 2 - g.pw;
+    const int hc = min(max(h0 + 1, 0), g.H - 1), wc = min(max(w0 + 1, 0), g.W - 1);
+    uint4 raw[9];
+    bool ok[9];
+#pragma unroll
+    for (int i = 0; i < 3; ++i)
+#pragma unroll
+      for (int j = 0; j < 3; ++j) {
+        const int h = h0 + i, w = w0 + j;
+        ok[3 * i + j] = (unsigned)h < (unsigned)g.H && (unsigned)w < (unsigned)g.W;
+        const int hh = ok[3 * i + j] ? h : hc, ww = ok[3 * i + j] ? w : wc;
+        raw[3 * i + j] = *reinterpret_cast<const uint4*>(x + (((size_t)n * g.H + hh) * g.W + ww) * g.C + cg * 8);
+      }
+    float sc[8], sh[8];
+    pld8(coef + cg * 8, sc);
+    pld8(coef + g.C + cg * 8, sh);
+    float best[8];
+    int arg[8];
+#pragma unroll
+    for (int e = 0; e < 8; ++e) { best[e] = -INFINITY; arg[e] = 0; }
+#pragma unroll
+    for (int k = 0; k < 9; ++k) {
+      float v[8];
+      unpack8(raw[k], v);
+#pragma unroll
+      for (int e = 0; e < 8; ++e) {
+        float o = fmaf(v[e], sc[e], sh[e]);
+        if (RELU) o = fmaxf(o, 0.f);
+        o = bf2f(f2bf(o));
+        if (ok[k] && (o > best[e] || o != o)) {
+          best[e] = o;
+          arg[e] = k;
+        }
+      }
+    }
+    const size_t o = (((size_t)n * g.P + p) * g.Q + q) * g.C + cg * 8;
+    store8(y + o, best);
     if (!idx) continue;
     uint32_t lo = 0, hi = 0;
 #pragma unroll
@@ -363,6 +424,28 @@
   BIGDL_CHECK_LAUNCH();
 }
 
+BIGDL_EXPORT int bigdl_bn_maxpool_fwd(const void* x, const float* coef, void* y, void* idx, int N, int H, int W, int C,
+                                      int P, int Q, int kh, int kw, int sh, int sw, int ph, int pw, int relu,
+                                      hipStream_t s) {
+  if (!x || !coef || !y || N <= 0 || H <= 0 || W <= 0 || P <= 0 || Q <= 0 || C <= 0 || C % 8)
+    return (int)hipErrorInvalidValue;
+  if (kh != 3 || kw != 3 || sh != 2 || sw != 2 || ph < 0 || pw < 0 || ph > 1 || pw > 1) return (int)hipErrorInvalidValue;
+  if (2 * (P - 1) - ph >= H || 2 * (Q - 1) - pw >= W) return (int)hipErrorInvalidValue;
+  if (((uintptr_t)x & 15) || ((uintptr_t)y & 15) || ((uintptr_t)coef & 15) || ((uintptr_t)idx & 7))
+    return (int)hipErrorInvalidValue;
+  const long long total = (long long)N * P * Q * (C / 8);
+  if (total >= 0x7fffffffLL || (long long)N * H * W * (C / 8) >= 0x7fffffffLL) return (int)hipErrorInvalidValue;
+  PoolGeom g = make_geom(N, H, W, C, P, Q, kh, kw, sh, sw, ph, pw);
+  const int grid = bigdl_grid(total, 256, 16384);
+  if (relu)
+    hipLaunchKernelGGL((k_bn_maxpool_fwd_k3s2<uint32_t, true>), dim3(grid), dim3(256), 0, s, (const bf16_t*)x, coef,
+                       (bf16_t*)y, (int8_t*)idx, g);
+  else
+    hipLaunchKernelGGL((k_bn_maxpool_fwd_k3s2<uint32_t, false>), dim3(grid), dim3(256), 0, s, (const bf16_t*)x, coef,
+                       (bf16_t*)y, (int8_t*)idx, g);
+  BIGDL_CHECK_LAUNCH();
+}
+
 BIGDL_EXPORT int bigdl_maxpool_bwd(const void* gy, const void* idx, void* gx, int N, int H, int W, int C, int P, int Q,
                                    int kh, int kw, int sh, int sw, int ph, int pw, hipStream_t s) {
   if (kh * kw > 127 || N <= 0 || C <= 0) return (int)hipErrorInvalidValue;
diff --git a/bigdl-1_amd/bigdl/ops/native_ops.py b/bigdl-1_amd/bigdl/ops/native_ops.py
--- a/bigdl-1_amd/bigdl/ops/native_ops.py
+++ b/bigdl-1_amd/bigdl/ops/native_ops.py
@@ -486,11 +486,35 @@
 
 @register("batchnorm_backward")
 def batchnorm_backward(gy, x, gamma, save_mean, save_invstd, y=None, relu=False, need_input=True, gg_acc=None,
-                       gb_acc=None, scale=1.0, cbias_acc=None, cbias_scale=1.0, want_gres=False):
+                       gb_acc=None, scale=1.0, cbias_acc=None, cbias_scale=1.0, want_gres=False, fcoef=None,
+                       mask_bits=None):
     rc = _rows_c(x)
     if rc is None:
         return NotImplemented
     M, C_ = rc
+    if relu and y is None and (fcoef is not None or mask_bits is not None):
+        if fcoef is not None:
+            kind, msk = 2, fcoef
+            ok = _f32vec(fcoef, 2 * C_)
+        else:
+            kind, msk = 3, mask_bits
+            ok = _bits_ok(mask_bits, M, C_, True) is not None
+        if not (ok and _bn_ok(x, C_) and gy.dtype == _bf16 and gy.shape == x.shape and gy.stride() == x.stride()
+                and _al16(gy) and all(_f32vec(t, C_) for t in (gamma, save_mean, save_invstd, gg_acc, gb_acc,
+                                                               cbias_acc))):
+            return NotImplemented
+        lib = _lib()
+        G = lib.bigdl_bn_num_partials(_ll(M), C.c_int(C_))
+        ws = torch.empty(2 * G * C_, dtype=_f32, device=x.device)
+        coef = torch.empty(3 * C_, dtype=_f32, device=x.device)
+        gx = torch.empty_like(x) if need_input else None
+        gres = torch.empty_like(x) if (want_gres and need_input) else None
+        check(lib.bigdl_bn_bwd_mask(ptr(gy), ptr(x), ptr(msk), C.c_int(kind), ptr(gx), ptr(gres), _ll(M), C.c_int(C_),
+                                    ptr(gamma), ptr(save_mean), ptr(save_invstd), ptr(gg_acc), ptr(gb_acc), _f(scale),
+                                    ptr(cbias_acc), _f(cbias_scale), ptr(ws), ptr(coef), _s()), "bn_bwd_mask")
+        if want_gres and gres is None:
+            gres = gy * R_.relu_mask(x, None, fcoef, mask_bits).to(gy.dtype)
+        return gx, gres
     mb = F3.producer_bits(y) if relu else None
     if (_bn32_ok(x, C_, gy, y if relu and mb is None else None) and (y is not None or not relu)
             and all(_f32vec(t, C_) for t in (gamma, save_mean, save_invstd, gg_acc, gb_acc, cbias_acc))):
@@ -1988,6 +2012,58 @@
     return y, (_Int8Idx(idx) if need_indices else None)
 
 
+def bn_maxpool_forward(bnout, k, s, p, ceil_mode=False, need_indices=True):
+    x, coef = bnout.x, bnout.coef
+    if (x.dim() != 4 or x.dtype != _bf16 or not x.is_cuda or not x.is_contiguous(memory_format=torch.channels_last)
+            or not _al16(x) or ceil_mode or tuple(k) != (3, 3) or tuple(s) != (2, 2) or p[0] not in (0, 1)
+            or p[1] not in (0, 1)):
+        return NotImplemented
+    N_, C_, H, W = x.shape
+    if C_ % 8 or not _f32vec(coef, 2 * C_) or not _al16(coef):
+        return NotImplemented
+    P = _pool_out(H, 3, 2, p[0], False)
+    Q = _pool_out(W, 3, 2, p[1], False)
+    if P <= 0 or Q <= 0 or N_ * H * W * (C_ // 8) >= 2 ** 31 - 1:
+        return NotImplemented
+    y = torch.empty((N_, C_, P, Q), dtype=_bf16, device=x.device, memory_format=torch.channels_last)
+    idx = torch.empty((N_, P, Q, C_), dtype=torch.int8, device=x.device) if need_indices else None
+    check(_lib().bigdl_bn_maxpool_fwd(ptr(x), ptr(coef), ptr(y), ptr(idx), N_, H, W, C_, P, Q, 3, 3, 2, 2, p[0], p[1],
+                                      1 if bnout.relu else 0, _s()), "bn_maxpool_fwd")
+    return y, (_Int8Idx(idx) if need_indices else None)
+
+
+def batchnorm_backward_pool(pg, x, gamma, save_mean, save_invstd, fcoef=None, need_input=True, gg_acc=None,
+                            gb_acc=None, scale=1.0, cbias_acc=None, cbias_scale=1.0):
+    rc = _rows_c(x)
+    if rc is None or x.dim() != 4 or not isinstance(pg.idx, _Int8Idx):
+        return NotImplemented
+    M, C_ = rc
+    N_, _, H, W = x.shape
+    g, idx = pg.g, pg.idx.t
+    if (not _bn_ok(x, C_) or tuple(pg.k) != (3, 3) or tuple(pg.s) != (2, 2) or pg.p[0] not in (0, 1)
+            or pg.p[1] not in (0, 1) or M >= 2 ** 31 - 1 or g.dim() != 4 or g.dtype != _bf16 or not g.is_cuda
+            or not g.is_contiguous(memory_format=torch.channels_last) or not _al16(g)):
+        return NotImplemented
+    P, Q = g.shape[2], g.shape[3]
+    if (tuple(g.shape) != (N_, C_, P, Q) or tuple(idx.shape) != (N_, P, Q, C_) or idx.dtype != torch.int8
+            or not idx.is_contiguous() or idx.data_ptr() % 8 or P != _pool_out(H, 3, 2, pg.p[0], False)
+            or Q != _pool_out(W, 3, 2, pg.p[1], False)):
+        return NotImplemented
+    if fcoef is not None and not _f32vec(fcoef, 2 * C_):
+        return NotImplemented
+    if not all(_f32vec(t, C_) for t in (gamma, save_mean, save_invstd, gg_acc, gb_acc, cbias_acc)):
+        return NotImplemented
+    lib = _lib()
+    G = lib.bigdl_bn_num_partials(_ll(M), C.c_int(C_))
+    ws = torch.empty(2 * G * C_, dtype=_f32, device=x.device)
+    coef = torch.empty(3 * C_, dtype=_f32, device=x.device)
+    gx = torch.empty_like(x) if need_input else None
+    check(lib.bigdl_bn_bwd_pool(ptr(g), ptr(idx), ptr(x), ptr(fcoef), ptr(gx), N_, H, W, C_, P, Q, pg.p[0], pg.p[1],
+                                ptr(gamma), ptr(save_mean), ptr(save_invstd), ptr(gg_acc), ptr(gb_acc), _f(scale),
+                                ptr(cbias_acc), _f(cbias_scale), ptr(ws), ptr(coef), _s()), "bn_bwd_pool")
+    return gx
+
+
 @register("maxpool2d_backward")
 def maxpool2d_backward(gy, x, idx, k, s, p, ceil_mode):
     if not isinstance(idx, _Int8Idx):
diff --git a/bigdl-1_amd/bigdl/ops/reference.py b/bigdl-1_amd/bigdl/ops/reference.py
--- a/bigdl-1_amd/bigdl/ops/reference.py
+++ b/bigdl-1_amd/bigdl/ops/reference.py
@@ -77,7 +77,7 @@
         return out
 
 
-class BNOut:
+class DeferredBN:
     __slots__ = ("x", "coef", "shape", "relu")
 
     def __init__(self, x, coef, relu=False):
@@ -107,6 +107,14 @@
             y = torch.relu(y)
         return y.to(self.x.dtype).contiguous(memory_format=torch.channels_last) if self.x.dim() == 4 \
             else y.to(self.x.dtype)
+
+
+class BNOut(DeferredBN):
+    __slots__ = ()
+
+
+class BNPoolOut(DeferredBN):
+    __slots__ = ()
 
 
 class BNGrad:
@@ -138,8 +146,33 @@
         return (a * self.g.float() + b * self.x.float() + c).to(self.g.dtype)
 
 
+class PoolGrad:
+    __slots__ = ("g", "idx", "k", "s", "p", "src", "shape")
+
+    def __init__(self, g, idx, k, s, p, src):
+        self.g, self.idx, self.k, self.s, self.p, self.src = g, idx, tuple(k), tuple(s), tuple(p), src
+        self.shape = tuple(src.shape)
+
+    @property
+    def dtype(self):
+        return self.g.dtype
+
+    @property
+    def is_cuda(self):
+        return self.g.is_cuda
+
+    def dim(self):
+        return len(self.shape)
+
+    def dense(self):
+        from . import dispatch, native as N
+        direct = isinstance(self.idx, torch.Tensor) or (self.g.is_cuda and N.has("maxpool2d_backward"))
+        return dispatch.maxpool2d_backward(self.g, self.src.x if direct else self.src.dense(), self.idx, self.k,
+                                           self.s, self.p, False)
+
+
 def as_dense(g):
-    return g.dense() if isinstance(g, (StridedGrad, BNGrad)) else g
+    return g.dense() if isinstance(g, (StridedGrad, BNGrad, PoolGrad)) else g
 
 
 def conv_transpose2d_forward(x, w4, b, stride, pad, adj, dilation=(1, 1), groups=1):
@@ -214,14 +247,26 @@
     return y.to(x.dtype)
 
 
+def relu_mask(x, y=None, fcoef=None, mask_bits=None):
+    if y is not None:
+        return y > 0
+    C = x.shape[1]
+    if fcoef is not None:
+        return DeferredBN(x, fcoef, relu=False).dense() > 0
+    w = (2 ** torch.arange(8, device=x.device, dtype=torch.int32)).view(1, 8)
+    pos = (mask_bits.view(-1, 1).to(torch.int32) & w) != 0
+    return pos.view(x.shape[0], *x.shape[2:], C).permute(0, 3, 1, 2)
+
+
 def batchnorm_backward(gy, x, gamma, save_mean, save_invstd, y=None, relu=False, need_input=True, gg_acc=None,
-                       gb_acc=None, scale=1.0, cbias_acc=None, cbias_scale=1.0, want_gres=False):
+                       gb_acc=None, scale=1.0, cbias_acc=None, cbias_scale=1.0, want_gres=False, fcoef=None,
+                       mask_bits=None):
     C = x.shape[1]
     dims = [d for d in range(x.dim()) if d != 1]
     shape = [1, C] + [1] * (x.dim() - 2)
     g = acc_float(gy)
     if relu:
-        g = g * (y > 0).float()
+        g = g * relu_mask(x, y, fcoef, mask_bits).to(g.dtype)
     xhat = (acc_float(x) - save_mean.view(shape)) * save_invstd.view(shape)
     dbeta = g.sum(dim=dims)
     dgamma = (g * xhat).sum(dim=dims)
@@ -351,6 +396,18 @@
     return aten.max_pool2d_with_indices_backward(gy, x, list(k), list(s), list(p), [1, 1], ceil_mode, idx)
 
 
+def bn_maxpool_forward(bnout, k, s, p, ceil_mode=False, need_indices=True):
+    return maxpool2d_forward(bnout.dense(), k, s, p, ceil_mode, need_indices)
+
+
+def batchnorm_backward_pool(pg, x, gamma, save_mean, save_invstd, fcoef=None, need_input=True, gg_acc=None,
+                            gb_acc=None, scale=1.0, cbias_acc=None, cbias_scale=1.0):
+    gy = pg.dense()
+    return batchnorm_backward(gy, x, gamma, save_mean, save_invstd, relu=fcoef is not None, need_input=need_input,
+                              gg_acc=gg_acc, gb_acc=gb_acc, scale=scale, cbias_acc=cbias_acc,
+                              cbias_scale=cbias_scale, fcoef=fcoef)[0]
+
+
 def avgpool2d_forward(x, k, s, p, ceil_mode, count_include_pad, divisor=None):
     return F.avg_pool2d(x, k, s, p, ceil_mode, count_include_pad, divisor)
 
diff --git a/bigdl-1_amd/bigdl/utils/config.py b/bigdl-1_amd/bigdl/utils/config.py
--- a/bigdl-1_amd/bigdl/utils/config.py
+++ b/bigdl-1_amd/bigdl/utils/config.py
@@ -79,6 +79,7 @@
     "bigdl.fusion.convstats": (bool, True, "conv epilogue emits the following training BN's statistics"),
     "bigdl.fusion.shortcutbn": (bool, True, "a ResNet block's conv->BN shortcut hands its BN output to the fused tail deferred (input + coefficients), applied inside the tail's pass"),
     "bigdl.fusion.bnbwd": (bool, True, "dgrad epilogue applies the producing BN's ReLU mask and its backward reductions"),
+    "bigdl.fusion.bnpool": (bool, True, "a training BN + ReLU whose only consumer is a 3x3 stride-2 max-pool (the ResNet stem) hands its output over deferred (bf16 on a GPU): the pool applies BN + ReLU to its window taps on load and the BN backward gathers the pool gradient through the argmax on load - the BN output and the dense pool gradient are never written"),
     "bigdl.fusion.bnprologue": (int, 0, "a BN whose producer is a 1x1 stride-1 conv hands it the input gradient "
                                          "deferred (A*g + B*x + C applied in the conv's dgrad / wgrad operand loads): "
                                          "0 off, 1 when the BN is narrower than the conv input, 2 always "
```

Result: faster. 12560 images/sec, median of 6 (+1.7%).
